# aerius-labs/paillier-halo2

Hardware: AMD Instinct MI355X
Metric: Paillier-encrypt proofs/s (2048-bit n, k=17); MSM achieved HBM GB/s vs peak (higher is better)
Workload: dtype u32 limbs (29-bit reduced radix, 254-bit modular integers), u64 limbs (4096-bit integers)

## Files before the change

include/pz.h:

```cpp
#ifndef PZ_H
#define PZ_H

#include <stddef.h>
#include <stdint.h>

#ifdef __cplusplus
extern "C" {
#endif

typedef struct pz_ctx pz_ctx;
typedef struct pz_bases pz_bases;

enum pz_status {
    PZ_OK = 0,
    PZ_ERR_INVALID = -1,
    PZ_ERR_HIP = -2,
    PZ_ERR_NO_DEVICE = -3,
    PZ_ERR_OOM = -4,
    PZ_ERR_ZERO_MODULUS = -5,
    PZ_ERR_RANGE = -6,
    PZ_ERR_UNSUPPORTED = -7,
    PZ_ERR_CAPACITY = -8,
    PZ_ERR_MESSAGE_RANGE = -9,
    PZ_ERR_ASYNC = -10
    ,
    PZ_ERR_INTERNAL = -11
};

int pz_init(int n_devices, const int* device_ids, pz_ctx** out);
int pz_free(pz_ctx* ctx);
const char* pz_strerror(int status);
const char* pz_last_hip_error(const pz_ctx* ctx);
int pz_set_stream(pz_ctx* ctx, void* hip_stream);
int pz_sync(pz_ctx* ctx);
#define PZ_ABI_VERSION 7
int pz_abi_version(void);

int pz_dev_alloc(pz_ctx* ctx, size_t bytes, void** d_out);
int pz_dev_cache_limit(pz_ctx* ctx, size_t max_bytes);
int pz_dev_arena(pz_ctx* ctx, size_t bytes);
int pz_dev_arena_info(pz_ctx* ctx, uint64_t out[6]);
int pz_dev_mem_info(pz_ctx* ctx, size_t* free_bytes, size_t* total_bytes);
int pz_dev_free(pz_ctx* ctx, void* d);
int pz_upload(pz_ctx* ctx, void* d_dst, const void* src, size_t bytes);
int pz_download(pz_ctx* ctx, void* dst, const void* d_src, size_t bytes);
int pz_dev_memset(pz_ctx* ctx, void* d_dst, int byte_value, size_t bytes);
int pz_dev_copy(pz_ctx* ctx, void* d_dst, const void* d_src, size_t bytes);
int pz_dev_copy_2d(pz_ctx* ctx, void* d_dst, size_t dst_pitch, const void* d_src, size_t src_pitch, size_t width, size_t rows);
int pz_ctx_wait(pz_ctx* waiter, pz_ctx* producer);

int pz_srs_load_g1(pz_ctx* ctx, uint32_t k, const uint64_t* bases_affine, int lagrange, pz_bases** out);
int pz_bases_load_g1(pz_ctx* ctx, const uint64_t* bases_affine, size_t n_points, int on_device,
                     uint32_t window_bits, pz_bases** out);
int pz_bases_free(pz_ctx* ctx, pz_bases* bases);
int pz_bases_info(const pz_bases* bases, size_t* n_points, uint32_t* window_bits, uint32_t* n_windows);

int pz_msm_g1(pz_ctx* ctx, const pz_bases* bases, const uint64_t* scalars, size_t n, uint64_t out_jac[12]);
int pz_msm_g1_batch(pz_ctx* ctx, const pz_bases* bases, const uint64_t* const* scalar_cols, size_t n_cols,
                    size_t n, uint64_t* out_jac );
int pz_msm_g1_dev(pz_ctx* ctx, const pz_bases* bases, const uint64_t* d_scalars, size_t n_cols, size_t n,
                  size_t col_stride, uint32_t win_lo, uint32_t win_hi, uint64_t* d_out_jac);
int pz_g1_sum(pz_ctx* ctx, const uint64_t* jac , size_t n, uint64_t out_jac[12]);
int pz_g1_sum_dev(pz_ctx* ctx, const uint64_t* d_jac, size_t n, uint64_t* d_out_jac);
int pz_msm_g1_multi(pz_ctx* const* ctxs, const pz_bases* const* bases, const uint64_t* const* d_scalars, const size_t* n_per_ctx,
                    size_t n_ctx, int split_points, uint64_t out_jac[12]);
int pz_g1_normalize(pz_ctx* ctx, const uint64_t* jac , size_t n, uint64_t* aff );
int pz_g1_fixed_base_mul(pz_ctx* ctx, const uint64_t* scalars, size_t n, uint64_t* out_affine );
int pz_g1_fixed_base_mul_dev(pz_ctx* ctx, const uint64_t* d_scalars, size_t n, uint64_t* d_out_affine);

int pz_g1_commit_mask_dev(pz_ctx* ctx, const pz_bases* bases, const uint8_t* d_mask, size_t n_cols, size_t n, size_t mask_stride,
                          uint64_t* d_out_jac);

int pz_ntt_fr(pz_ctx* ctx, uint64_t* a , const uint64_t omega[4], uint32_t log_n);
int pz_ntt_fr_batch(pz_ctx* ctx, uint64_t* const* cols, size_t n_cols, const uint64_t omega[4], uint32_t log_n);
int pz_ntt_fr_dev(pz_ctx* ctx, uint64_t* d_a, size_t n_cols, size_t col_stride, const uint64_t omega[4],
                  uint32_t log_n, const uint64_t* pre_coset_g, const uint64_t* post_scale);
int pz_ntt_fr_to_dev(pz_ctx* ctx, const uint64_t* d_in, size_t in_stride, uint64_t* d_out, size_t out_stride, size_t n_cols,
                     const uint64_t omega[4], uint32_t log_n, const uint64_t* pre_coset_g, const uint64_t* post_scale);

int pz_ntt_fr_extend_dev(pz_ctx* ctx, const uint64_t* d_coeff, size_t n_cols, size_t in_stride, uint64_t* d_ext,
                         size_t out_stride, uint32_t log_n, uint32_t log_e, const uint64_t omega_n[4],
                         const uint64_t* coset_gens, const uint64_t* scale);
int pz_ntt_fr_coeff_extend_dev(pz_ctx* ctx, uint64_t* d_values, size_t n_cols, size_t col_stride, uint64_t* d_ext,
                               size_t out_stride, uint32_t log_n, uint32_t log_e, const uint64_t omega_n[4],
                               const uint64_t omega_n_inv[4], const uint64_t n_inv[4], const uint64_t* coset_gens);
int pz_fr_convert_dev(pz_ctx* ctx, uint64_t* d_a, size_t n, int to_mont);
int pz_fr_from_mask_dev(pz_ctx* ctx, const uint8_t* d_mask, size_t n, uint64_t* d_out);

int pz_mul_mod(pz_ctx* ctx, uint32_t limbs, const uint64_t* a, const uint64_t* b, const uint64_t* modulus,
               uint64_t* q, uint64_t* r);
int pz_paillier_trace(pz_ctx* ctx, uint32_t limbs_n2, const uint64_t* n2, const uint64_t* base, const uint64_t* exp,
                      uint32_t exp_limbs, uint64_t* steps_out, size_t* n_steps, uint64_t* result);
int pz_paillier_encrypt(pz_ctx* ctx, uint32_t limbs_n, size_t batch, const uint64_t* n, const uint64_t* g,
                        const uint64_t* m, const uint64_t* r, uint64_t* steps_out, size_t steps_cap,
                        uint32_t* n_steps_g, uint32_t* n_steps_r, uint64_t* c_out);
int pz_paillier_encrypt_dev(pz_ctx* ctx, uint32_t limbs_n, size_t batch, const uint64_t* n, const uint64_t* g,
                            const uint64_t* m, const uint64_t* r, uint64_t* d_steps_out, size_t steps_cap,
                            uint32_t* n_steps_g, uint32_t* n_steps_r, uint64_t* c_out);

int pz_paillier_encrypt_uniform(pz_ctx* ctx, uint32_t limbs_n, size_t batch, uint32_t m_bits, const uint64_t* n, const uint64_t* g,
                                const uint64_t* m, const uint64_t* r, uint64_t* steps_out, size_t steps_cap, uint32_t* n_steps_g,
                                uint32_t* n_steps_r, uint64_t* c_out);
int pz_paillier_encrypt_uniform_dev(pz_ctx* ctx, uint32_t limbs_n, size_t batch, uint32_t m_bits, const uint64_t* n,
                                    const uint64_t* g, const uint64_t* m, const uint64_t* r, uint64_t* d_steps_out, size_t steps_cap,
                                    uint32_t* n_steps_g, uint32_t* n_steps_r, uint64_t* c_out);

int pz_paillier_tally(pz_ctx* ctx, uint32_t limbs_n, size_t count, const uint64_t* n, const uint64_t* cts, uint64_t* steps_out,
                      size_t steps_cap, uint64_t* c_out);
int pz_paillier_tally_dev(pz_ctx* ctx, uint32_t limbs_n, size_t count, const uint64_t* n, const uint64_t* cts, uint64_t* d_steps_out,
                          size_t steps_cap, uint64_t* c_out);

int pz_witness_cells_per_step(uint32_t limbs, uint32_t limb_bits, uint32_t lookup_bits, size_t* advice_cells,
                              size_t* lookup_cells);
int pz_witness_expand_dev(pz_ctx* ctx, uint32_t limbs, uint32_t limb_bits, uint32_t lookup_bits,
                          const uint64_t* d_steps, size_t n_steps, const uint64_t* d_modulus, uint64_t* d_advice,
                          uint64_t* d_lookup);

int pz_circuit_cells(int kind, uint32_t limbs_n, uint32_t limb_bits, uint32_t lookup_bits, size_t n_steps_g,
                     size_t n_steps_r, size_t* advice_cells, size_t* lookup_cells);
int pz_circuit_expand_dev(pz_ctx* ctx, int kind, uint32_t limbs_n, uint32_t limb_bits, uint32_t lookup_bits,
                          const uint64_t* inputs, const uint64_t* d_steps, size_t n_steps_g, size_t n_steps_r,
                          const uint64_t* d_modulus, uint64_t* d_advice, uint64_t* d_lookup, size_t rows, size_t col_stride);

int pz_circuit_break_points(const uint8_t* gate_mask, size_t n_cells, size_t max_rows, uint64_t* starts_out, size_t capacity,
// ... 121 lines not shown
                           const uint64_t* d_l_active, const uint64_t beta[4], const uint64_t gamma[4], const uint64_t y[4],
                           uint64_t* d_h);
int pz_quotient_permutation_split_dev(pz_ctx* ctx, const uint64_t* d_cols_ext, size_t col_stride, const uint64_t* d_sigma_ext,
                                      size_t sigma_stride, const uint64_t* d_z_ext, size_t z_stride, uint32_t n_sets_total,
                                      uint32_t set_lo, uint32_t n_sets, uint32_t chunk_len, uint32_t m_cols, int head, uint32_t log_ext,
                                      uint32_t rot_step, uint32_t last_rotation, const uint64_t* d_l0, const uint64_t* d_l_last,
                                      const uint64_t beta[4], const uint64_t gamma[4], const uint64_t delta[4],
                                      const uint64_t coset_g[4], const uint64_t omega_ext[4], const uint64_t y[4], uint64_t* d_h_low,
                                      uint64_t* d_h_d);
int pz_quotient_lookup_split_dev(pz_ctx* ctx, const uint64_t* d_input_ext, size_t input_stride, const uint64_t* d_table_ext,
                                 const uint64_t* d_perm_input_ext, size_t perm_input_stride, const uint64_t* d_perm_table_ext,
                                 size_t perm_table_stride, const uint64_t* d_z_ext, size_t z_stride, uint32_t n_lookups,
                                 uint32_t log_ext, uint32_t rot_step, const uint64_t* d_l0, const uint64_t* d_l_last,
                                 const uint64_t* d_l_active, const uint64_t beta[4], const uint64_t gamma[4], const uint64_t y[4],
                                 uint64_t* d_h_low, uint64_t* d_h_d);
int pz_quotient_d_rows_dev(pz_ctx* ctx, const uint64_t* d_cols, size_t col_stride, const uint64_t* d_sigma, size_t sigma_stride,
                           const uint64_t* d_z, size_t z_stride, uint32_t m, uint32_t chunk_len, const uint64_t* d_input,
                           size_t input_stride, const uint64_t* d_table, const uint64_t* d_perm_input, size_t perm_input_stride,
                           const uint64_t* d_perm_table, size_t perm_table_stride, const uint64_t* d_zl, size_t zl_stride,
                           uint32_t n_lookups, uint32_t log_n, size_t row_lo, const uint64_t omega[4], const uint64_t beta[4],
                           const uint64_t gamma[4], const uint64_t delta[4], const uint64_t y[4], uint64_t* d_out);
int pz_fr_mul_row_dev(pz_ctx* ctx, const uint64_t* d_a, size_t n_cols, size_t col_stride, size_t n, const uint64_t* d_row,
                      uint64_t* d_out, size_t out_stride);
int pz_quotient_finish_dev(pz_ctx* ctx, uint64_t* d_h, uint32_t log_n, uint32_t log_e, const uint64_t coset_g[4],
                           const uint64_t omega_ext[4]);
int pz_fr_distribute_powers_dev(pz_ctx* ctx, uint64_t* d_a, size_t n_cols, size_t col_stride, size_t n,
                                const uint64_t g[4], const uint64_t c[4]);
int pz_fr_lincomb_dev(pz_ctx* ctx, const uint64_t* d_polys, size_t n_cols, size_t col_stride, size_t n,
                      const uint64_t v[4], uint64_t* d_out, int accumulate);
int pz_poly_div_linear_dev(pz_ctx* ctx, const uint64_t* d_coeffs, size_t n_cols, size_t col_stride, size_t n,
                           const uint64_t x[4], uint64_t* d_q, size_t q_stride);

typedef struct pz_shplonk pz_shplonk;
int pz_shplonk_begin_dev(pz_ctx* ctx, size_t n, uint32_t n_sets, const uint32_t* set_n_polys, const uint64_t* const* d_polys,
                         const uint32_t* set_n_points, const uint32_t* point_idx, uint32_t n_points_total, const uint64_t* points,
                         const uint64_t* evals, const uint64_t y[4], const uint64_t v[4], uint64_t* d_h, pz_shplonk** state);
int pz_shplonk_finish_dev(pz_ctx* ctx, pz_shplonk* state, const uint64_t u[4], const uint64_t* d_h, uint64_t* d_h2);
int pz_shplonk_free(pz_ctx* ctx, pz_shplonk* state);

typedef struct pz_structure pz_structure;
int pz_circuit_structure_dev(pz_ctx* ctx, int kind, uint32_t limbs_n, uint32_t limb_bits, uint32_t lookup_bits, uint32_t k,
                             const uint64_t* exp_g, const uint64_t* exp_r, size_t minimum_rows, uint32_t blinding_factors,
                             pz_structure** out);
int pz_circuit_structure_tally_dev(pz_ctx* ctx, uint32_t limbs_n, uint32_t limb_bits, uint32_t lookup_bits, uint32_t k, size_t count,
                                   size_t minimum_rows, uint32_t blinding_factors, pz_structure** out);
int pz_structure_info(const pz_structure* st, size_t* n_adv, size_t* n_adv_filled, size_t* n_lk, size_t* max_rows, size_t* n_constants,
                      size_t* n_cells, size_t* n_lookups, size_t* n_steps_g, size_t* n_steps_r);
int pz_structure_arrays(const pz_structure* st, const uint8_t** d_selectors, const uint32_t** d_map_col, const uint32_t** d_map_row,
                        const uint64_t** d_col_starts, const uint64_t** constants, const uint64_t** col_starts_host);
int pz_structure_free(pz_structure* st);

typedef struct pz_pk pz_pk;
typedef struct pz_proof pz_proof;
#define PZ_BLINDING_SEEDED_TEST_STREAM (~(size_t)0)
#define PZ_PK_EXT_ALL (~(size_t)0)
int pz_pk_create(pz_ctx* ctx, const pz_bases* bases_lagrange, const pz_bases* bases_monomial, uint32_t k, uint32_t lookup_bits,
                 uint32_t blinding_factors, size_t max_rows, size_t n_adv, size_t n_lk, const uint8_t* selectors,
                 const uint64_t* constants, size_t n_constants, const uint32_t* map_col, const uint32_t* map_row, size_t tile,
                 size_t ext_resident_cols, pz_pk** out);
int pz_pk_create_dev(pz_ctx* ctx, const pz_bases* bases_lagrange, const pz_bases* bases_monomial, uint32_t k, uint32_t lookup_bits,
                     uint32_t blinding_factors, size_t max_rows, size_t n_adv, size_t n_lk, const uint8_t* d_selectors,
                     const uint64_t* constants, size_t n_constants, const uint32_t* d_map_col, const uint32_t* d_map_row, size_t tile,
                     size_t ext_resident_cols, pz_pk** out);
int pz_pk_info(const pz_pk* pk, size_t* n_fixed, size_t* n_perm_cols, size_t* n_sets, size_t* blinding_words, size_t* evals_words);
int pz_pk_commitments(const pz_pk* pk, uint64_t* fixed_affine, uint64_t* sigma_affine);
int pz_pk_free(pz_pk* pk);
int pz_proof_begin(pz_pk* pk, uint64_t* d_cols, uint64_t seed, const uint64_t* blinding, size_t n_blinding, pz_proof** out,
                   uint64_t* advice_affine);
int pz_proof_lookups(pz_proof* proof, const uint64_t theta[4], uint64_t* perm_inputs_affine, uint64_t* perm_tables_affine);
int pz_proof_products(pz_proof* proof, const uint64_t beta[4], const uint64_t gamma[4], uint64_t* perm_z_affine,
                      uint64_t* lookup_z_affine, uint64_t* random_affine);
int pz_proof_quotient(pz_proof* proof, const uint64_t y[4], uint64_t* h_affine);
int pz_proof_evaluate(pz_proof* proof, const uint64_t x[4], uint64_t* evals);
int pz_proof_open_begin(pz_proof* proof, const uint64_t y[4], const uint64_t v[4], uint64_t* w1_affine);
int pz_proof_open_finish(pz_proof* proof, const uint64_t u[4], uint64_t* w2_affine, int* quotient_degree_ok);
int pz_proof_free(pz_proof* proof);

int pz_circuit_public_cells(int kind, uint32_t limbs_n, uint32_t limb_bits, uint32_t lookup_bits, size_t n_steps_g, size_t n_steps_r,
                            uint64_t* cells_out, size_t capacity, size_t* n_public);
int pz_structure_expose(pz_structure* st);
int pz_structure_public(const pz_structure* st, size_t* n_instance, size_t* n_public, const uint32_t** d_cell_col, const uint32_t** d_cell_row);
int pz_public_gather_dev(pz_ctx* ctx, const uint64_t* d_cols, size_t col_stride, const uint32_t* d_cell_col, const uint32_t* d_cell_row,
                         size_t n_public, uint64_t* out_words);
int pz_instance_eval_dev(pz_ctx* ctx, uint32_t k, const uint64_t omega[4], const uint64_t n_inv[4], const uint64_t* d_instances,
                         size_t n_public, size_t n_proofs, const uint64_t* d_x, uint64_t* d_out, int32_t* d_flags);
int pz_pk_create_pub(pz_ctx* ctx, const pz_bases* bases_lagrange, const pz_bases* bases_monomial, uint32_t k, uint32_t lookup_bits,
                     uint32_t blinding_factors, size_t max_rows, size_t n_adv, size_t n_lk, size_t n_instance, size_t n_public,
                     const uint8_t* selectors, const uint64_t* constants, size_t n_constants, const uint32_t* map_col, const uint32_t* map_row,
                     size_t tile, size_t ext_resident_cols, pz_pk** out);
int pz_pk_create_pub_dev(pz_ctx* ctx, const pz_bases* bases_lagrange, const pz_bases* bases_monomial, uint32_t k, uint32_t lookup_bits,
                         uint32_t blinding_factors, size_t max_rows, size_t n_adv, size_t n_lk, size_t n_instance, size_t n_public,
                         const uint8_t* d_selectors, const uint64_t* constants, size_t n_constants, const uint32_t* d_map_col,
                         const uint32_t* d_map_row, size_t tile, size_t ext_resident_cols, pz_pk** out);
int pz_vk_keygen_pub_dev(pz_ctx* ctx, const pz_bases* bases_lagrange, uint32_t k, uint32_t lookup_bits, size_t n_adv, size_t n_lk,
                         size_t n_instance, size_t n_public, const uint8_t* d_selectors, const uint64_t* constants, size_t n_constants,
                         const uint32_t* d_map_col, const uint32_t* d_map_row, size_t tile, uint64_t* fixed_affine, uint64_t* sigma_affine);
int pz_vk_keygen_pub(pz_ctx* ctx, const pz_bases* bases_lagrange, uint32_t k, uint32_t lookup_bits, size_t n_adv, size_t n_lk,
                     size_t n_instance, size_t n_public, const uint8_t* selectors, const uint64_t* constants, size_t n_constants,
                     const uint32_t* map_col, const uint32_t* map_row, size_t tile, uint64_t* fixed_affine, uint64_t* sigma_affine);
int pz_vk_create_pub(pz_ctx* ctx, uint32_t k, uint32_t blinding_factors, size_t n_adv, size_t n_lk, size_t n_instance, size_t n_public,
                     const uint64_t* fixed_affine, const uint64_t* sigma_affine, const uint64_t g0_affine[8], const uint64_t g2[16],
                     const uint64_t s_g2[16], pz_vk** out);
int pz_proof_begin_pub(pz_pk* pk, uint64_t* d_cols, uint64_t seed, const uint64_t* blinding, size_t n_blinding, const uint64_t* instances,
                       size_t n_public, pz_proof** out, uint64_t* advice_affine);
int pz_verify_batch_pub(pz_vk* vk, const uint64_t* instances, size_t n_public, const uint64_t* proofs, size_t n_proofs, const uint8_t* seeds,
                        const size_t* seed_offsets, int32_t* verdicts, uint64_t* h_evals, uint64_t* ab_affine, int* all_ok);
// ... 19 lines not shown
```

paillier_halo2_amd/_lib.py:

```python
from __future__ import annotations

import ctypes as C
import os
import subprocess

_HERE = os.path.dirname(os.path.abspath(__file__))
CSRC = os.path.join(_HERE, "csrc")
SO_PATH = os.path.join(CSRC, "libpz_hip.so")
PROBE_SO_PATH = os.path.join(CSRC, "libpz_probe.so")

U64P = C.POINTER(C.c_uint64)
U32P = C.POINTER(C.c_uint32)
VP = C.c_void_p

SIGNATURES = {
    "pz_init": (C.c_int, [C.c_int, C.POINTER(C.c_int), C.POINTER(VP)]),
    "pz_free": (C.c_int, [VP]),
    "pz_strerror": (C.c_char_p, [C.c_int]),
    "pz_last_hip_error": (C.c_char_p, [VP]),
    "pz_set_stream": (C.c_int, [VP, VP]),
    "pz_sync": (C.c_int, [VP]),
    "pz_abi_version": (C.c_int, []),
    "pz_dev_alloc": (C.c_int, [VP, C.c_size_t, C.POINTER(VP)]),
    "pz_dev_cache_limit": (C.c_int, [VP, C.c_size_t]),
    "pz_dev_arena": (C.c_int, [VP, C.c_size_t]),
    "pz_dev_arena_info": (C.c_int, [VP, C.POINTER(C.c_uint64)]),
    "pz_dev_mem_info": (C.c_int, [VP, C.POINTER(C.c_size_t), C.POINTER(C.c_size_t)]),
    "pz_dev_free": (C.c_int, [VP, VP]),
    "pz_upload": (C.c_int, [VP, VP, VP, C.c_size_t]),
    "pz_download": (C.c_int, [VP, VP, VP, C.c_size_t]),
    "pz_dev_memset": (C.c_int, [VP, VP, C.c_int, C.c_size_t]),
    "pz_dev_copy": (C.c_int, [VP, VP, VP, C.c_size_t]),
    "pz_dev_copy_2d": (C.c_int, [VP, VP, C.c_size_t, VP, C.c_size_t, C.c_size_t, C.c_size_t]),
    "pz_ctx_wait": (C.c_int, [VP, VP]),
    "pz_srs_load_g1": (C.c_int, [VP, C.c_uint32, VP, C.c_int, C.POINTER(VP)]),
    "pz_bases_load_g1": (C.c_int, [VP, VP, C.c_size_t, C.c_int, C.c_uint32, C.POINTER(VP)]),
    "pz_bases_free": (C.c_int, [VP, VP]),
    "pz_bases_info": (C.c_int, [VP, C.POINTER(C.c_size_t), U32P, U32P]),
    "pz_msm_g1": (C.c_int, [VP, VP, VP, C.c_size_t, VP]),
    "pz_msm_g1_batch": (C.c_int, [VP, VP, C.POINTER(VP), C.c_size_t, C.c_size_t, VP]),
    "pz_msm_g1_dev": (C.c_int, [VP, VP, VP, C.c_size_t, C.c_size_t, C.c_size_t, C.c_uint32, C.c_uint32, VP]),
    "pz_g1_commit_mask_dev": (C.c_int, [VP, VP, VP, C.c_size_t, C.c_size_t, C.c_size_t, VP]),
    "pz_g1_sum": (C.c_int, [VP, VP, C.c_size_t, VP]),
    "pz_g1_sum_dev": (C.c_int, [VP, VP, C.c_size_t, VP]),
    "pz_msm_g1_multi": (C.c_int, [VP, VP, VP, VP, C.c_size_t, C.c_int, VP]),
    "pz_g1_normalize": (C.c_int, [VP, VP, C.c_size_t, VP]),
    "pz_g1_fixed_base_mul": (C.c_int, [VP, VP, C.c_size_t, VP]),
    "pz_g1_fixed_base_mul_dev": (C.c_int, [VP, VP, C.c_size_t, VP]),
    "pz_ntt_fr": (C.c_int, [VP, VP, VP, C.c_uint32]),
    "pz_ntt_fr_batch": (C.c_int, [VP, C.POINTER(VP), C.c_size_t, VP, C.c_uint32]),
    "pz_ntt_fr_dev": (C.c_int, [VP, VP, C.c_size_t, C.c_size_t, VP, C.c_uint32, VP, VP]),
    "pz_ntt_fr_to_dev": (C.c_int, [VP, VP, C.c_size_t, VP, C.c_size_t, C.c_size_t, VP, C.c_uint32, VP, VP]),
    "pz_ntt_fr_extend_dev": (C.c_int, [VP, VP, C.c_size_t, C.c_size_t, VP, C.c_size_t, C.c_uint32, C.c_uint32, VP, VP, VP]),
    "pz_ntt_fr_coeff_extend_dev": (C.c_int, [VP, VP, C.c_size_t, C.c_size_t, VP, C.c_size_t, C.c_uint32, C.c_uint32, VP, VP, VP,
                                             VP]),
    "pz_fr_convert_dev": (C.c_int, [VP, VP, C.c_size_t, C.c_int]),
    "pz_fr_from_mask_dev": (C.c_int, [VP, VP, C.c_size_t, VP]),
    "pz_mul_mod": (C.c_int, [VP, C.c_uint32, VP, VP, VP, VP, VP]),
    "pz_paillier_trace": (C.c_int, [VP, C.c_uint32, VP, VP, VP, C.c_uint32, VP, C.POINTER(C.c_size_t), VP]),
    "pz_paillier_encrypt": (C.c_int, [VP, C.c_uint32, C.c_size_t, VP, VP, VP, VP, VP, C.c_size_t, VP, VP, VP]),
    "pz_paillier_encrypt_dev": (C.c_int, [VP, C.c_uint32, C.c_size_t, VP, VP, VP, VP, VP, C.c_size_t, VP, VP, VP]),
    "pz_paillier_tally": (C.c_int, [VP, C.c_uint32, C.c_size_t, VP, VP, VP, C.c_size_t, VP]),
    "pz_paillier_tally_dev": (C.c_int, [VP, C.c_uint32, C.c_size_t, VP, VP, VP, C.c_size_t, VP]),
    "pz_paillier_encrypt_uniform": (C.c_int, [VP, C.c_uint32, C.c_size_t, C.c_uint32, VP, VP, VP, VP, VP, C.c_size_t, VP, VP, VP]),
    "pz_paillier_encrypt_uniform_dev": (C.c_int, [VP, C.c_uint32, C.c_size_t, C.c_uint32, VP, VP, VP, VP, VP, C.c_size_t, VP, VP, VP]),
    "pz_witness_cells_per_step": (C.c_int, [C.c_uint32, C.c_uint32, C.c_uint32, C.POINTER(C.c_size_t),
                                            C.POINTER(C.c_size_t)]),
    "pz_witness_expand": (C.c_int, [VP, C.c_uint32, C.c_uint32, C.c_uint32, VP, C.c_size_t, VP, VP, VP]),
    "pz_witness_expand_dev": (C.c_int, [VP, C.c_uint32, C.c_uint32, C.c_uint32, VP, C.c_size_t, VP, VP, VP]),
    "pz_refresh_aux": (C.c_int, [C.c_uint32, C.c_uint32, C.c_uint32, VP, C.c_uint32, U32P]),
    "pz_op_cells": (C.c_int, [C.c_int, C.c_uint32, C.c_uint32, C.c_uint32, C.POINTER(C.c_size_t), C.POINTER(C.c_size_t)]),
    "pz_circuit_cells": (C.c_int, [C.c_int, C.c_uint32, C.c_uint32, C.c_uint32, C.c_size_t, C.c_size_t, C.POINTER(C.c_size_t),
                                   C.POINTER(C.c_size_t)]),
    "pz_circuit_expand_dev": (C.c_int, [VP, C.c_int, C.c_uint32, C.c_uint32, C.c_uint32, VP, VP, C.c_size_t, C.c_size_t, VP, VP, VP,
                                        C.c_size_t, C.c_size_t]),
    "pz_circuit_break_points": (C.c_int, [VP, C.c_size_t, C.c_size_t, VP, C.c_size_t, C.POINTER(C.c_size_t)]),
    "pz_circuit_expand_cols_dev": (C.c_int, [VP, C.c_int, C.c_uint32, C.c_uint32, C.c_uint32, VP, VP, C.c_size_t, C.c_size_t, VP, VP, VP,
                                             VP, C.c_size_t, C.c_size_t, C.c_size_t, C.c_size_t]),
    "pz_srs_setup_g1_dev": (C.c_int, [VP, C.c_uint32, VP, VP, VP, VP]),
    "pz_srs_lagrange_from_monomial_dev": (C.c_int, [VP, C.c_uint32, VP, VP, VP, VP]),
    "pz_permutation_sigma_dev": (C.c_int, [VP, VP, VP, C.c_size_t, C.c_uint32, VP, VP, VP, C.c_size_t]),
    "pz_permutation_sigma_part_dev": (C.c_int, [VP, VP, VP, C.c_size_t, C.c_size_t, C.c_size_t, C.c_uint32, VP, VP, VP, C.c_size_t]),
    "pz_keygen_columns_dev": (C.c_int, [VP, VP, VP, C.c_size_t, C.c_size_t, C.c_uint32, C.c_uint32, VP, VP, VP, VP, VP, VP, C.c_size_t]),
    "pz_poly_eval_dev": (C.c_int, [VP, VP, C.c_size_t, C.c_size_t, C.c_size_t, VP, VP]),
    "pz_poly_eval_multi_dev": (C.c_int, [VP, VP, C.c_size_t, C.c_size_t, C.c_size_t, VP, C.c_uint32, VP]),
    "pz_g1_check_dev": (C.c_int, [VP, VP, C.c_size_t, C.POINTER(C.c_uint64)]),
    "pz_g2_generator": (C.c_int, [VP]),
    "pz_g2_mul_dev": (C.c_int, [VP, VP, VP, C.c_size_t, VP]),
    "pz_pairing_dev": (C.c_int, [VP, VP, VP, C.c_size_t, VP]),
    "pz_pairing_check_dev": (C.c_int, [VP, VP, VP, C.c_size_t, C.c_uint32, VP]),
    "pz_vk_create": (C.c_int, [VP, C.c_uint32, C.c_uint32, C.c_size_t, C.c_size_t, VP, VP, VP, VP, VP, C.POINTER(VP)]),
    "pz_vk_info": (C.c_int, [VP, C.POINTER(C.c_size_t), C.POINTER(C.c_size_t)]),
    "pz_verify_batch": (C.c_int, [VP, VP, C.c_size_t, VP, VP, VP, VP, VP, C.POINTER(C.c_int)]),
    "pz_vk_free": (C.c_int, [VP]),
    "pz_vk_keygen_dev": (C.c_int, [VP, VP, C.c_uint32, C.c_uint32, C.c_size_t, C.c_size_t, VP, VP, C.c_size_t, VP, VP, C.c_size_t, VP, VP]),
# ... 171 lines not shown
```

paillier_halo2_amd/csrc/pz_internal.h:

```cpp
#pragma once
#include <hip/hip_runtime.h>
#include <stdint.h>
#include <stdio.h>
#include <string.h>

#include <map>
#include <mutex>
#include <vector>

#include "../../include/pz.h"

enum { PZ_T_MSM_ACC = 0, PZ_T_NTT = 1, PZ_T_TRACE = 2, PZ_T_EXPAND = 3, PZ_T_MSM_ALL = 4, PZ_T_MSM_SORT = 5, PZ_T_MSM_TREE = 6, PZ_T_COUNT = 7 };

struct pz_pow_table {
    uint64_t base[4];
    uint64_t init[4];
    size_t n;
    size_t cap;
    void* d;
    void* d_raw = nullptr;
    bool raw_valid = false;
    uint64_t stamp;
};

// ... 7 lines not shown
    size_t cap = 0;
};

enum { WS_HIST = 0, WS_OFFS, WS_CURSOR, WS_ITEMS, WS_ENTRIES, WS_PARTIALS, WS_NODES_A, WS_NODES_B, WS_NTT_TMP,
       WS_IO_A, WS_IO_B, WS_IO_C, WS_BIG_A, WS_BIG_B, WS_BIG_C, WS_MISC, WS_TOTALS, WS_ORDER, WS_SH_C, WS_SH_SMALL, WS_ROWC, WS_SEL, WS_K3, WS_MULTI, WS_PAIR, WS_COUNT };

struct pz_event_pair {
    hipEvent_t a, b;
};

#define PZ_IO_EVENTS 10
struct pz_arena;
struct pz_ctx {
    int device = 0;
    hipStream_t own_stream = nullptr;
    hipStream_t stream = nullptr;
    char hip_err[256] = {0};
    pz_wsbuf ws[WS_COUNT];
    std::vector<pz_pow_table> pow_tables;
    uint64_t pow_clock = 0;
    std::vector<pz_ext_table> ext_tables;
    bool timing = false;
    std::vector<pz_event_pair> ev[PZ_T_COUNT];
    size_t ev_used[PZ_T_COUNT] = {0};
    double ev_ms[PZ_T_COUNT] = {0};
    uint64_t ev_n[PZ_T_COUNT] = {0};
    int cu_count = 256;
    size_t mem_avail = 0;
    unsigned mem_avail_age = 0;
    hipStream_t io_h2d = nullptr, io_d2h = nullptr;
    hipEvent_t io_ev[PZ_IO_EVENTS] = {};
    void* stage_h[4] = {nullptr, nullptr, nullptr, nullptr};
    size_t stage_cap[4] = {0, 0, 0, 0};
    hipEvent_t stage_ev[4] = {nullptr, nullptr, nullptr, nullptr};
    unsigned stage_next = 0;
    volatile unsigned* async_err_h = nullptr;
    volatile unsigned* async_err_d = nullptr;
    size_t dev_cache_limit = 0, dev_cache_bytes = 0;
    std::vector<std::pair<void*, size_t>> dev_cache;
    std::map<void*, size_t> dev_live;
    struct pz_arena* arena = nullptr;
    std::recursive_mutex mu;
};

struct pz_bases {
    size_t n = 0;
    uint32_t c = 0;
    uint32_t nwin = 0;
    void* d_table = nullptr;
    int lagrange = 0;
    int device = 0;
};

static inline int pz_hip_fail(pz_ctx* ctx, hipError_t e, const char* what) {
    if (ctx) snprintf(ctx->hip_err, sizeof ctx->hip_err, "%s: %s", what, hipGetErrorString(e));
    return e == hipErrorOutOfMemory ? PZ_ERR_OOM : PZ_ERR_HIP;
}
#define HIPCHK(ctx, x)                                              \
    do {                                                            \
        hipError_t e_ = (x);                                        \
        if (e_ != hipSuccess) return pz_hip_fail((ctx), e_, #x);    \
    } while (0)
#define PZCHK(x)                    \
    do {                            \
        int rc_ = (x);              \
        if (rc_ != PZ_OK) return rc_; \
    } while (0)

#define PZ_ENTER(ctx)                                           \
    std::lock_guard<std::recursive_mutex> pz_lock_((ctx)->mu);  \
    HIPCHK((ctx), hipSetDevice((ctx)->device))

int pz_ws_get(pz_ctx* ctx, int slot, size_t bytes, void** out);
hipError_t pz_hip_malloc(pz_ctx* ctx, void** d, size_t bytes);
hipError_t pz_hip_free(void* d);
size_t pz_mem_free_bytes(pz_ctx* ctx);
void pz_dev_cache_trim(pz_ctx* ctx, size_t keep_bytes);
int pz_get_pow_table(pz_ctx* ctx, const uint64_t base[4], size_t n, void** d_out, const uint64_t* init = nullptr);
int pz_get_pow_table_raw(pz_ctx* ctx, const uint64_t base[4], size_t n, void** d_raw_out, const uint64_t* init = nullptr);
int pz_raw29_convert(pz_ctx* ctx, const void* d_src_fr, void* d_dst_u32, size_t count);

struct pz_timer {
    pz_ctx* ctx;
    int cls;
    bool on;
    size_t idx;
    pz_timer(pz_ctx* c, int cls_);
    ~pz_timer();
};

int pz_async_err_init(pz_ctx* ctx);
int pz_check_async(pz_ctx* ctx);
const uint64_t* pz_fr_one261();
int pz_io_init(pz_ctx* ctx);
int pz_upload_small_async(pz_ctx* ctx, void* d_dst, const void* src, size_t bytes);

int pz_permutation_sigma_tile(pz_ctx* ctx, const uint32_t* d_mc, const uint32_t* d_mr, size_t m_total, size_t n_cols, uint32_t k,
                              const uint64_t omega[4], const uint64_t delta[4], uint64_t* d_sigma, size_t sigma_stride);

struct pz_dev_bufs {
    pz_ctx* c;
    std::vector<void*> bufs;
    explicit pz_dev_bufs(pz_ctx* c_) : c(c_) {}
    int get(size_t bytes, void** out) {
        *out = nullptr;
        const int rc = pz_dev_alloc(c, bytes ? bytes : 1, out);
// ... 59 lines not shown
```

paillier_halo2_amd/csrc/pz_msm.hip:

```cpp
#include "ec.cuh"
#include "ec29.cuh"
#include "ec29_quad.cuh"
#include <math.h>
#include <stdlib.h>

#include "pz_internal.h"

#define MSM_CHUNK_MIN 16u
#define MSM_CHUNK_MAX 256u
#define MSM_HEAVY 24u
#define MSM_MEDIUM 1024u
#define MSM_SLICE_MAX_COLS 8u

struct MsmP {
    size_t n;
    size_t n_table;
    unsigned c;
    unsigned nwin;
    unsigned win_lo, win_hi;
    unsigned B;
    size_t cap;
    size_t max_items;
    unsigned chunk;
    unsigned spt;
};

struct ScatterSel {
    const unsigned long long* total;
    unsigned long long thr;
    volatile unsigned* err;
};
__device__ __noinline__ void scatter_bad(const ScatterSel& s) { *s.err = 1u; }
__device__ __forceinline__ bool scatter_dense(const ScatterSel& s) { return *s.total >= s.thr; }

__device__ __forceinline__ u32 sel8(const u32 s[8], unsigned i) {
    u32 r = s[0];
#pragma unroll
    for (int k = 1; k < 8; ++k) r = (i == (unsigned)k) ? s[k] : r;
    return r;
}

__device__ __forceinline__ bool scalar_prepare(const Fr& mont, u32 s[8]) {
    Fr k = fp_from_mont(mont);
    Fr t;
    u64 br = 0;
#pragma unroll
    for (int i = 0; i < 8; ++i) {
        u64 d = (u64)FieldParams<FrTag>::P(i) - k.v[i] - br;
        t.v[i] = (u32)d;
        br = (d >> 32) & 1;
    }
    bool lt = false, decided = false;
#pragma unroll
    for (int i = 7; i >= 0; --i) {
        if (!decided && t.v[i] != k.v[i]) {
            lt = t.v[i] < k.v[i];
            decided = true;
        }
    }
#pragma unroll
    for (int i = 0; i < 8; ++i) s[i] = lt ? t.v[i] : k.v[i];
    return lt;
}

__device__ __forceinline__ int next_digit(const u32 s[8], unsigned w, unsigned c, unsigned& carry) {
    unsigned off = w * c;
    unsigned wi = off >> 5, sh = off & 31;
    u32 lo = wi < 8 ? sel8(s, wi) : 0;
    u32 hi = wi + 1 < 8 ? sel8(s, wi + 1) : 0;
    u64 both = ((u64)hi << 32) | lo;
    unsigned raw = (unsigned)(both >> sh) & ((1u << c) - 1);
    unsigned d = raw + carry;
    if (d > (1u << (c - 1))) {
        carry = 1;
        return (int)d - (int)(1u << c);
    }
    carry = 0;
    return (int)d;
}

__global__ __launch_bounds__(128) void k_build_table(const G1Aff64* __restrict__ bases, G1Aff64* __restrict__ table,
                                                     size_t n, unsigned c, unsigned nwin) {
    size_t i = (size_t)blockIdx.x * blockDim.x + threadIdx.x;
    if (i >= n) return;
    G1A29 p = a29_load64(bases + i);
    if (!a29_is_inf(p)) {
        p.x = f29_to_261(p.x);
        p.y = f29_to_261(p.y);
        p = a29_canon(p);
    }
    a29_store64(table + i, p);
    G1X29 x = x29_from_affine(p);
    for (unsigned w = 1; w < nwin; ++w) {
        for (unsigned k = 0; k < c; ++k) x = x29_dbl(x);
        const G1A29 a = a29_canon(x29_to_affine(x));
        a29_store64(table + (size_t)w * n + i, a);
        x = x29_from_affine(a);
    }
}

#define SORT_THREADS 1024u
#ifndef SORT_PER_THREAD
#define SORT_PER_THREAD 8u
#endif
#define SORT_SLICE (SORT_THREADS * SORT_PER_THREAD)
#define SORT_MAXB 32768u

#ifndef PZ_SORT_XCD
#define PZ_SORT_XCD 1
#endif
__device__ __forceinline__ bool sort_block_coords(unsigned n_slices, size_t n_cols, unsigned& slice, size_t& col) {
    if (PZ_SORT_XCD && n_cols >= 8) {
        const unsigned w = blockIdx.x >> 3;
        slice = w % n_slices;
        col = (size_t)(w / n_slices) * 8 + (blockIdx.x & 7u);
    } else {
        slice = blockIdx.x % n_slices;
        col = blockIdx.x / n_slices;
    }
    return col < n_cols;
}
static unsigned sort_grid(unsigned n_slices, size_t n_cols) {
    if (PZ_SORT_XCD && n_cols >= 8) return n_slices * (unsigned)((n_cols + 7) / 8 * 8);
    return n_slices * (unsigned)n_cols;
}

__global__ __launch_bounds__(SORT_THREADS) void k_msm_hist(const Fr* __restrict__ scalars, size_t col_stride, MsmP p,
                                                           u32* __restrict__ slice_hist, unsigned n_slices, size_t n_cols) {
    __shared__ u32 h[SORT_MAXB];
    size_t col;
    unsigned slice;
    if (!sort_block_coords(n_slices, n_cols, slice, col)) return;
    for (unsigned b = threadIdx.x; b < p.B; b += SORT_THREADS) h[b] = 0;
    __syncthreads();
    const size_t base = (size_t)slice * SORT_THREADS * p.spt;
    for (unsigned t = 0; t < p.spt; ++t) {
        const size_t i = base + (size_t)t * SORT_THREADS + threadIdx.x;
        if (i >= p.n) break;
        u32 s[8];
        (void)scalar_prepare(fp_load<FrTag>(scalars + col * col_stride + i), s);
        u32 any = 0;
#pragma unroll
        for (int k = 0; k < 8; ++k) any |= s[k];
        if (!any) continue;
        unsigned carry = 0;
        if (p.c == 16) {
#pragma unroll
            for (unsigned w = 0; w < 16; ++w) {
                if (w < p.win_hi) {
                    const unsigned d0 = ((s[w >> 1] >> (16 * (w & 1))) & 0xffffu) + carry;
                    carry = d0 > 0x8000u ? 1u : 0u;
                    const unsigned mag = carry ? 0x10000u - d0 : d0;
                    if (w >= p.win_lo && mag != 0) atomicAdd(&h[mag - 1], 1u);
                }
            }
        } else {
            for (unsigned w = 0; w < p.win_hi; ++w) {
                int d = next_digit(s, w, p.c, carry);
                if (w >= p.win_lo && d != 0) atomicAdd(&h[(d < 0 ? -d : d) - 1], 1u);
            }
        }
    }
    __syncthreads();
    u32* out = slice_hist + (col * n_slices + slice) * (size_t)p.B;
    for (unsigned b = threadIdx.x; b < p.B; b += SORT_THREADS) out[b] = h[b];
}

__global__ __launch_bounds__(256) void k_msm_totals(u32* __restrict__ slice_hist, unsigned n_slices, MsmP p,
                                                    u32* __restrict__ totals) {
    const size_t col = blockIdx.y;
    const unsigned b = blockIdx.x * blockDim.x + threadIdx.x;
    if (b >= p.B) return;
    u32* sh = slice_hist + col * n_slices * (size_t)p.B + b;
    u32 run = 0;
    unsigned sl = 0;
    for (; sl + 8 <= n_slices; sl += 8) {
        u32 v[8];
#pragma unroll
        for (unsigned k = 0; k < 8; ++k) v[k] = sh[(size_t)(sl + k) * p.B];
#pragma unroll
        for (unsigned k = 0; k < 8; ++k) {
            sh[(size_t)(sl + k) * p.B] = run;
            run += v[k];
        }
    }
    for (; sl < n_slices; ++sl) {
        const u32 v = sh[(size_t)sl * p.B];
        sh[(size_t)sl * p.B] = run;
        run += v;
    }
    totals[col * p.B + b] = run;
// ... 73 lines not shown
            run += s_bin[m2];
            s_bin[m2] = 0;
        }
        fold_cnt[col] = run;
        run = 0;
        for (int sz = (int)p.chunk; sz >= 1; --sz) {
            s_obase[sz] = run;
            run += s_obin[sz];
            s_obin[sz] = 0;
        }
    }
    __syncthreads();
    c = s_cnt[threadIdx.x];
    m = s_itm[threadIdx.x];
#pragma unroll
    for (unsigned k = 0; k < 32; ++k) {
        const unsigned b = lo + k;
        if (k < per && b < p.B) {
            const u32 v = hv[k];
            o[b] = c;
            it[b] = m;
            c += v;
            const u32 ch = (v + p.chunk - 1) / p.chunk;
            m += ch;
            if (ch > 1 && ch <= MSM_HEAVY) fold_order[col * p.B + s_base[ch] + atomicAdd(&s_bin[ch], 1u)] = b;
            if (ch) {
                const u32 q = v / ch, rem = v % ch;
                const u32 ph = rem ? s_obase[q + 1] + atomicAdd(&s_obin[q + 1], rem) : 0u;
                const u32 pl = s_obase[q] + atomicAdd(&s_obin[q], ch - rem);
                {
                    const u32 item0 = m - ch;
                    u32* ord = item_order + col * p.max_items;
                    u32* obk = item_bucket + col * p.max_items;
                    for (u32 j = 0; j < ch; ++j) {
                        const u32 pos = j < rem ? ph + j : pl + j - rem;
                        ord[pos] = item0 + j;
                        obk[pos] = b;
                    }
                }
            }
        }
    }
}

#define SORT_FINE_LOG 7u
#define SORT_FINE (1u << SORT_FINE_LOG)
#define SORT_COARSE_MAX (SORT_MAXB >> SORT_FINE_LOG)
#define COARSE_THREADS 256u
#define COARSE_ROUND (COARSE_THREADS * 16u)
static_assert(COARSE_ROUND <= 65536u && SORT_COARSE_MAX <= 256u && SORT_COARSE_MAX == COARSE_THREADS, "k_msm_scatter_coarse packing");
__global__ __launch_bounds__(COARSE_THREADS) void k_msm_scatter_coarse(const Fr* __restrict__ scalars, size_t col_stride, MsmP p,
                                                                       const u32* __restrict__ slice_hist, unsigned n_slices,
                                                                       const u32* __restrict__ offs, u32* __restrict__ staged,
                                                                       size_t n_cols, ScatterSel sel) {
    if (!scatter_dense(sel)) return;
    __shared__ u32 cb[SORT_COARSE_MAX];
    __shared__ u32 cnt[SORT_COARSE_MAX];
    __shared__ u32 lbase[SORT_COARSE_MAX];
    __shared__ u32 gb[SORT_COARSE_MAX];
    __shared__ u32 stage[COARSE_ROUND];
    __shared__ unsigned char sbin[COARSE_ROUND];
    __shared__ u32 s_total;
    size_t col;
    unsigned slice;
    if (!sort_block_coords(n_slices, n_cols, slice, col)) return;
    const u32* in = slice_hist + (col * n_slices + slice) * (size_t)p.B;
    const u32* o = offs + col * (p.B + 1);
    const unsigned n_coarse = p.B >> SORT_FINE_LOG;
    if (threadIdx.x < SORT_COARSE_MAX) {
        cb[threadIdx.x] = threadIdx.x < n_coarse ? o[threadIdx.x << SORT_FINE_LOG] : 0u;
        cnt[threadIdx.x] = 0;
    }
    __syncthreads();
    for (unsigned b0 = (threadIdx.x & ~63u); b0 < p.B; b0 += 4 * COARSE_THREADS) {
        u32 v[4];
#pragma unroll
        for (unsigned k = 0; k < 4; ++k) {
            const unsigned b = b0 + k * COARSE_THREADS + (threadIdx.x & 63u);
            v[k] = b < p.B ? in[b] : 0u;
        }
#pragma unroll
        for (unsigned k = 0; k < 4; ++k) {
            u32 t = v[k];
#pragma unroll
            for (int off = 32; off > 0; off >>= 1) t += __shfl_xor(t, off, 64);
            const unsigned b = b0 + k * COARSE_THREADS;
            if ((threadIdx.x & 63u) == 0 && b < p.B && t) atomicAdd(&cb[b >> SORT_FINE_LOG], t);
        }
    }
    __syncthreads();
    u32* e = staged + col * p.cap;
    const size_t base = (size_t)slice * SORT_THREADS * p.spt;
    const unsigned rounds = SORT_THREADS * p.spt / COARSE_THREADS;
    Fr nxt = fp_zero<FrTag>();
    if (base + threadIdx.x < p.n) nxt = fp_load<FrTag>(scalars + col * col_stride + base + threadIdx.x);
    for (unsigned rd = 0; rd < rounds; ++rd) {
        const size_t i = base + (size_t)rd * COARSE_THREADS + threadIdx.x;
        if (base + (size_t)rd * COARSE_THREADS >= p.n) break;
        const Fr cur_scalar = nxt;
        u32 ev[16], rb[16];
#pragma unroll
        for (unsigned w = 0; w < 16; ++w) rb[w] = 0xffffffffu;
        if (i < p.n) {
            u32 s[8];
            const bool neg = scalar_prepare(cur_scalar, s);
            unsigned carry = 0;
#pragma unroll
            for (unsigned w = 0; w < 16; ++w) {
                if (w < p.win_hi) {
                    const unsigned d0 = ((s[w >> 1] >> (16 * (w & 1))) & 0xffffu) + carry;
                    carry = d0 > 0x8000u ? 1u : 0u;
                    const unsigned mag = carry ? 0x10000u - d0 : d0;
                    if (w >= p.win_lo && mag != 0) {
                        const unsigned bkt = mag - 1, grp = bkt >> SORT_FINE_LOG;
                        const bool sgn = neg != (carry != 0);
                        ev[w] = (u32)((size_t)w * p.n_table + i) | (sgn ? 0x01000000u : 0u) | ((bkt & (SORT_FINE - 1)) << 25);
                        rb[w] = atomicAdd(&cnt[grp], 1u) | (grp << 16);
                    }
                }
            }
        }
        __syncthreads();
        if (threadIdx.x < 64) {
            const unsigned c0 = cnt[4 * threadIdx.x], c1 = cnt[4 * threadIdx.x + 1], c2 = cnt[4 * threadIdx.x + 2], c3 = cnt[4 * threadIdx.x + 3];
            const unsigned sum = c0 + c1 + c2 + c3;
            unsigned incl = sum;
#pragma unroll
            for (int off = 1; off < 64; off <<= 1) {
                const unsigned t = __shfl_up(incl, off, 64);
                if ((int)threadIdx.x >= off) incl += t;
            }
            const unsigned excl = incl - sum;
            lbase[4 * threadIdx.x] = excl;
            lbase[4 * threadIdx.x + 1] = excl + c0;
            lbase[4 * threadIdx.x + 2] = excl + c0 + c1;
            lbase[4 * threadIdx.x + 3] = excl + c0 + c1 + c2;
            if (threadIdx.x == 63) s_total = incl;
        }
        __syncthreads();
        {
            const unsigned g = cb[threadIdx.x], c = cnt[threadIdx.x];
            gb[threadIdx.x] = g - lbase[threadIdx.x];
            cb[threadIdx.x] = g + c;
            cnt[threadIdx.x] = 0;
        }
#pragma unroll
        for (unsigned w = 0; w < 16; ++w) {
            if (rb[w] != 0xffffffffu) {
                const unsigned grp = rb[w] >> 16, slot = lbase[grp] + (rb[w] & 0xffffu);
                stage[slot] = ev[w];
                sbin[slot] = (unsigned char)grp;
            }
        }
        __syncthreads();
        {
            const size_t in_ = i + COARSE_THREADS;
            if (rd + 1 < rounds && in_ < p.n) nxt = fp_load<FrTag>(scalars + col * col_stride + in_);
        }
        const unsigned total = s_total;
        for (unsigned sl = threadIdx.x; sl < total; sl += COARSE_THREADS) {
            const u32 pos = gb[sbin[sl]] + sl;
            if (pos < p.cap) e[pos] = stage[sl];
            else scatter_bad(sel);
        }
    }
}

#define FINE_LDS_ENTRIES 12288u
#define FINE_THREADS 512u
__global__ __launch_bounds__(FINE_THREADS) void k_msm_scatter_fine(MsmP p, const u32* __restrict__ offs, const u32* __restrict__ staged,
                                                          u32* __restrict__ entries, ScatterSel sel) {
    if (!scatter_dense(sel)) return;
    __shared__ u32 cur[SORT_FINE + 1];
    __shared__ u32 buf[FINE_LDS_ENTRIES];
    const size_t col = blockIdx.y;
    const u32* o = offs + col * (p.B + 1) + ((size_t)blockIdx.x << SORT_FINE_LOG);
    if (threadIdx.x <= SORT_FINE) cur[threadIdx.x] = o[threadIdx.x];
    __syncthreads();
    const u32 lo = cur[0], hi = cur[SORT_FINE];
    __syncthreads();
    const u32* src = staged + col * p.cap;
    u32* dst = entries + col * p.cap;
    const bool in_lds = hi - lo <= FINE_LDS_ENTRIES;
    for (u32 j0 = lo + threadIdx.x; j0 < hi; j0 += 8 * FINE_THREADS) {
        u32 v[8];
#pragma unroll
        for (unsigned k = 0; k < 8; ++k) {
            const u32 j = j0 + k * FINE_THREADS;
            v[k] = j < hi ? src[j] : 0xffffffffu;
        }
#pragma unroll
        for (unsigned k = 0; k < 8; ++k) {
            if (j0 + k * FINE_THREADS < hi) {
                const u32 pos = atomicAdd(&cur[v[k] >> 25], 1u);
                const u32 e = (v[k] & 0x00ffffffu) | ((v[k] & 0x01000000u) << 7);
                if (pos >= hi) scatter_bad(sel);
                else if (in_lds) buf[pos - lo] = e;
                else dst[pos] = e;
            }
        }
    }
    if (!in_lds) return;
    __syncthreads();
    for (u32 j = threadIdx.x; j < hi - lo; j += FINE_THREADS) dst[lo + j] = buf[j];
}

#define FEW_BINS (MSM_CHUNK_MAX + 1u)
__device__ __forceinline__ u32 block_sum_256(u32 v, u32* s_tmp) {
#pragma unroll
    for (int off = 32; off > 0; off >>= 1) v += __shfl_xor(v, off, 64);
// ... 114 lines not shown
    if (lane == 63) { s_wc[wv] = ic; s_wm[wv] = im; }
    __syncthreads();
    u32 bc = 0, bm = 0;
    for (unsigned k = 0; k < wv; ++k) { bc += s_wc[k]; bm += s_wm[k]; }
    const u32 o_b = pc + bc + ic - v, it_b = pm + bm + im - ch;
    u32* o = offs + col * (p.B + 1);
    u32* it = items + col * (p.B + 1);
    if (b < p.B) {
        o[b] = o_b;
        it[b] = it_b;
        if (b == p.B - 1) {
            o[p.B] = o_b + v;
            it[p.B] = it_b + ch;
            atomicAdd(digits_total, (unsigned long long)(o_b + v));
        }
    }
    u32* ord = item_order + col * p.max_items;
    u32* obk = item_bucket + col * p.max_items;
    u32 ph = 0, pl = 0, rem = 0;
    if (ch) {
        const u32 q = v / ch;
        rem = v % ch;
        if (rem) ph = s_pos[q + 1] + atomicAdd(&s_rank[q + 1], rem);
        pl = s_pos[q] + atomicAdd(&s_rank[q], ch - rem);
        if (ch > ITEMS_SOLO) {
            s_big[atomicAdd(&s_nbig, 1u)] = threadIdx.x;
        } else {
            for (u32 j = 0; j < ch; ++j) {
                const u32 pos = j < rem ? ph + j : pl + j - rem;
                ord[pos] = it_b + j;
                obk[pos] = b;
            }
        }
    }
    __shared__ u32 s_par[256][5];
    if (ch > ITEMS_SOLO) {
        s_par[threadIdx.x][0] = ch; s_par[threadIdx.x][1] = rem; s_par[threadIdx.x][2] = ph; s_par[threadIdx.x][3] = pl; s_par[threadIdx.x][4] = it_b;
    }
    __syncthreads();
    for (unsigned k = 0; k < s_nbig; ++k) {
        const unsigned tt = s_big[k];
        const u32 ch2 = s_par[tt][0], rem2 = s_par[tt][1], ph2 = s_par[tt][2], pl2 = s_par[tt][3], it2 = s_par[tt][4];
        for (u32 j = threadIdx.x; j < ch2; j += blockDim.x) {
            const u32 pos = j < rem2 ? ph2 + j : pl2 + j - rem2;
            ord[pos] = it2 + j;
            obk[pos] = blk * blockDim.x + tt;
        }
    }
}

__global__ __launch_bounds__(SORT_THREADS) void k_msm_scatter(const Fr* __restrict__ scalars, size_t col_stride, MsmP p,
                                                              const u32* __restrict__ slice_hist, unsigned n_slices,
                                                              const u32* __restrict__ offs, u32* __restrict__ entries, size_t n_cols,
                                                              ScatterSel sel) {
    if (scatter_dense(sel)) return;
    __shared__ u32 h[SORT_MAXB];
    size_t col;
    unsigned slice;
    if (!sort_block_coords(n_slices, n_cols, slice, col)) return;
    const u32* in = slice_hist + (col * n_slices + slice) * (size_t)p.B;
    const u32* o = offs + col * (p.B + 1);
    for (unsigned b0 = threadIdx.x; b0 < p.B; b0 += 8 * SORT_THREADS) {
        u32 va[8], vb[8];
#pragma unroll
        for (unsigned k = 0; k < 8; ++k) {
            const unsigned b = b0 + k * SORT_THREADS, bc = b < p.B ? b : p.B - 1;
            va[k] = o[bc];
            vb[k] = in[bc];
        }
#pragma unroll
        for (unsigned k = 0; k < 8; ++k) {
            const unsigned b = b0 + k * SORT_THREADS;
            if (b < p.B) h[b] = va[k] + vb[k];
        }
    }
    __syncthreads();
    u32* e = entries + col * p.cap;
    const size_t base = (size_t)slice * SORT_THREADS * p.spt;
    for (unsigned t = 0; t < p.spt; ++t) {
        const size_t i = base + (size_t)t * SORT_THREADS + threadIdx.x;
        if (i >= p.n) break;
        u32 s[8];
        const bool neg = scalar_prepare(fp_load<FrTag>(scalars + col * col_stride + i), s);
        u32 any = 0;
#pragma unroll
        for (int k = 0; k < 8; ++k) any |= s[k];
        if (!any) continue;
        unsigned carry = 0;
        if (p.c == 16) {
#pragma unroll
            for (unsigned w = 0; w < 16; ++w) {
                if (w < p.win_hi) {
                    const unsigned d0 = ((s[w >> 1] >> (16 * (w & 1))) & 0xffffu) + carry;
                    carry = d0 > 0x8000u ? 1u : 0u;
                    const unsigned mag = carry ? 0x10000u - d0 : d0;
                    if (w >= p.win_lo && mag != 0) {
                        const u32 pos = atomicAdd(&h[mag - 1], 1u);
                        const bool sgn = neg != (carry != 0);
                        if (pos < p.cap) e[pos] = (u32)((size_t)w * p.n_table + i) | (sgn ? 0x80000000u : 0u);
                        else scatter_bad(sel);
                    }
                }
            }
        } else {
            for (unsigned w = 0; w < p.win_hi; ++w) {
                int d = next_digit(s, w, p.c, carry);
                if (w >= p.win_lo && d != 0) {
                    const unsigned b = (d < 0 ? -d : d) - 1;
                    const u32 pos = atomicAdd(&h[b], 1u);
                    const bool sgn = neg != (d < 0);
                    if (pos < p.cap) e[pos] = (u32)((size_t)w * p.n_table + i) | (sgn ? 0x80000000u : 0u);
                    else scatter_bad(sel);
                }
            }
        }
    }
}

__global__ __launch_bounds__(256) void k_msm_accumulate(const G1Aff64* __restrict__ table, MsmP p,
                                                        const u32* __restrict__ offs, const u32* __restrict__ items,
                                                        const u32* __restrict__ item_order,
                                                        const u32* __restrict__ item_bucket,
                                                        const u32* __restrict__ entries, G1X29Raw* __restrict__ partials) {
    const size_t col = blockIdx.x;
    const u32* it = items + col * (p.B + 1);
    const u32 total = it[p.B];
    const u32 rank = blockIdx.y * blockDim.x + threadIdx.x;
    if (rank >= total) return;
    const u32 item = item_order[col * p.max_items + rank];
    const unsigned b = item_bucket[col * p.max_items + rank];
    const u32* o = offs + col * (p.B + 1);
    const u32 cnt = o[b + 1] - o[b], nch = it[b + 1] - it[b], j = item - it[b];
    const u32 q = cnt / nch, rem = cnt % nch;
    const u32 start = o[b] + j * q + (j < rem ? j : rem);
// ... 455 lines not shown
    int rc = pz_bases_load_g1(ctx, bases_affine, (size_t)1 << k, 0, 0, out);
    if (rc == PZ_OK) (*out)->lagrange = lagrange;
    return rc;
}

extern "C" int pz_bases_free(pz_ctx* ctx, pz_bases* b) {
    if (!b) return PZ_OK;
    if (ctx) {
        std::lock_guard<std::recursive_mutex> lk(ctx->mu);
        (void)hipSetDevice(ctx->device);
        (void)hipStreamSynchronize(ctx->stream);
    }
    if (b->d_table) (void)pz_hip_free(b->d_table);
    delete b;
    return PZ_OK;
}

extern "C" int pz_bases_info(const pz_bases* b, size_t* n_points, uint32_t* window_bits, uint32_t* n_windows) {
    if (!b) return PZ_ERR_INVALID;
    if (n_points) *n_points = b->n;
    if (window_bits) *window_bits = b->c;
    if (n_windows) *n_windows = b->nwin;
    return PZ_OK;
}

static unsigned msm_chunk_for(size_t n_cols, size_t digits_per_col, unsigned window_bits) {
    static int env = -1;
    if (env < 0) {
        const char* e = getenv("PZ_MSM_CHUNK");
        env = e ? atoi(e) : 0;
    }
    if (env >= (int)MSM_CHUNK_MIN && env <= (int)MSM_CHUNK_MAX) return (unsigned)env;
    if (n_cols <= MSM_SLICE_MAX_COLS) {
        const double per_bucket = (double)digits_per_col / (double)((size_t)1 << (window_bits - 1));
        double ch = 0.79 * pow(per_bucket, 0.63);
        unsigned c32 = ch < 24.0 ? MSM_CHUNK_MIN : 32u * (unsigned)((ch + 16.0) / 32.0);
        if (c32 > MSM_CHUNK_MAX) c32 = MSM_CHUNK_MAX;
        return c32;
    }
    const size_t want = (n_cols * digits_per_col) >> 18;
    unsigned chunk = MSM_CHUNK_MIN;
    while (chunk < MSM_CHUNK_MAX && chunk * 2 <= want) chunk *= 2;
    return chunk;
}

static unsigned msm_spt_for(size_t n_cols, size_t n) {
    const size_t min_wg = n_cols <= MSM_SLICE_MAX_COLS ? 128 : 512;
    unsigned spt = SORT_PER_THREAD;
    while (spt > 1 && n_cols * pz_div_up(n, (size_t)SORT_THREADS * spt) < min_wg) spt >>= 1;
    return spt;
}

static int msm_group(pz_ctx* ctx, const pz_bases* bases, const Fr* d_scalars, size_t nc, size_t n, size_t cs,
                     unsigned win_lo, unsigned win_hi, unsigned chunk, G1Jac* d_out) {
    MsmP p;
    p.n = n;
    p.n_table = bases->n;
    p.c = bases->c;
    p.nwin = bases->nwin;
    p.win_lo = win_lo;
    p.win_hi = win_hi;
    p.B = 1u << (bases->c - 1);
    p.cap = n * (size_t)(win_hi - win_lo);
    p.chunk = chunk;
    if (p.B + n * (size_t)(win_hi - win_lo) / chunk > 65535u * 256u) return PZ_ERR_CAPACITY;
    p.max_items = p.B + p.cap / chunk;
    void *hist, *offs, *heavy, *items, *entries, *partials, *na, *nb, *totals, *fold, *iord;
    p.spt = msm_spt_for(nc, n);
    const unsigned n_slices = pz_div_up(n, (size_t)SORT_THREADS * p.spt);
    PZCHK(pz_ws_get(ctx, WS_HIST, nc * (size_t)n_slices * p.B * 4, &hist));
    PZCHK(pz_ws_get(ctx, WS_CURSOR, nc * (size_t)(p.B + 1) * 4, &heavy));
    const bool split_items = nc <= MSM_SLICE_MAX_COLS;
    const unsigned nblk_few = pz_div_up(p.B, 256);
    PZCHK(pz_ws_get(ctx, WS_TOTALS, nc * ((size_t)p.B + (split_items ? (size_t)nblk_few * (2 + FEW_BINS) : 0)) * 4, &totals));
    u32* blk_cnt = (u32*)totals + nc * (size_t)p.B;
    u32* blk_itm = blk_cnt + nc * (size_t)nblk_few;
    u32* blk_bins = blk_itm + nc * (size_t)nblk_few;
    u32* heavy_cnt = (u32*)heavy + nc * (size_t)p.B;
    PZCHK(pz_ws_get(ctx, WS_MISC, nc * (size_t)(p.B + 1) * 4, &fold));
    u32* fold_cnt = (u32*)fold + nc * (size_t)p.B;
    PZCHK(pz_ws_get(ctx, WS_ORDER, nc * p.max_items * 8, &iord));
    u32* item_order = (u32*)iord;
    u32* item_bucket = (u32*)iord + nc * p.max_items;
    PZCHK(pz_ws_get(ctx, WS_OFFS, nc * (p.B + 1) * 4, &offs));
    PZCHK(pz_ws_get(ctx, WS_ITEMS, nc * (p.B + 1) * 4, &items));
    PZCHK(pz_ws_get(ctx, WS_ENTRIES, nc * p.cap * 4 + 16, &entries));
    static int scatter_mode = -1;
    if (scatter_mode < 0) {
        const char* e = getenv("PZ_MSM_SCATTER");
        scatter_mode = (e && !strcmp(e, "one")) ? 1 : (e && !strcmp(e, "two")) ? 2 : 0;
    }
    const bool two_pass = scatter_mode != 1 && p.c == 16 && (size_t)p.nwin * p.n_table <= ((size_t)1 << 24) &&
                          (nc > MSM_SLICE_MAX_COLS || scatter_mode == 2);
    {
        const size_t part_bytes = nc * p.max_items * sizeof(G1X29Raw), stage_bytes = two_pass ? nc * p.cap * 4 + 16 : 0;
        PZCHK(pz_ws_get(ctx, WS_PARTIALS, part_bytes > stage_bytes ? part_bytes : stage_bytes, &partials));
    }
    const unsigned m1 = p.B >= 16 ? 16 : p.B;
    unsigned n_nodes = p.B / m1;
    PZCHK(pz_ws_get(ctx, WS_NODES_A, nc * (size_t)n_nodes * sizeof(MsmNode), &na));
    PZCHK(pz_ws_get(ctx, WS_NODES_B, nc * (size_t)(n_nodes / 2 + 1) * sizeof(MsmNode), &nb));
    hipStream_t st = ctx->stream;
    pz_timer tall(ctx, PZ_T_MSM_ALL);
    dim3 gs(sort_grid(n_slices, nc));
    void* dsel;
    PZCHK(pz_ws_get(ctx, WS_SEL, 8, &dsel));
    HIPCHK(ctx, hipMemsetAsync(dsel, 0, 8, st));
    PZCHK(pz_async_err_init(ctx));
    {
        pz_timer tsort(ctx, PZ_T_MSM_SORT);
        hipLaunchKernelGGL(k_msm_hist, gs, dim3(SORT_THREADS), 0, st, d_scalars, cs, p, (u32*)hist, n_slices, nc);
        if (split_items) {
            hipLaunchKernelGGL(k_msm_totals_few, dim3(nblk_few, (unsigned)nc), dim3(256), 0, st, (u32*)hist, n_slices, p, (u32*)totals,
                               blk_cnt, blk_itm, blk_bins);
            hipLaunchKernelGGL(k_msm_items_few, dim3(nblk_few, (unsigned)nc), dim3(256), 0, st, p, (const u32*)totals, (const u32*)blk_cnt,
                               (const u32*)blk_itm, (const u32*)blk_bins, (u32*)offs, (u32*)items, item_order, item_bucket,
                               (unsigned long long*)dsel);
        } else {
            hipLaunchKernelGGL(k_msm_totals, dim3(pz_div_up(p.B, 256), (unsigned)nc), dim3(256), 0, st, (u32*)hist, n_slices, p,
                               (u32*)totals);
            hipLaunchKernelGGL(k_msm_scan, dim3((unsigned)nc), dim3(SCAN_THREADS), 0, st, (const u32*)totals, p, (u32*)offs, (u32*)items,
                               (u32*)heavy, heavy_cnt, (u32*)fold, fold_cnt, item_order, item_bucket, (unsigned long long*)dsel);
        }
        ScatterSel sel;
        sel.total = (const unsigned long long*)dsel;
        sel.thr = !two_pass ? ~0ull : scatter_mode == 2 ? 0ull : (unsigned long long)(0.4 * (double)nc * (double)p.cap);
        sel.err = ctx->async_err_d;
        if (two_pass) {
            hipLaunchKernelGGL(k_msm_scatter_coarse, gs, dim3(COARSE_THREADS), 0, st, d_scalars, cs, p, (const u32*)hist, n_slices,
                               (const u32*)offs, (u32*)partials, nc, sel);
            hipLaunchKernelGGL(k_msm_scatter_fine, dim3(p.B >> SORT_FINE_LOG, (unsigned)nc), dim3(FINE_THREADS), 0, st, p, (const u32*)offs,
                               (const u32*)partials, (u32*)entries, sel);
        }
        if (scatter_mode != 2 || !two_pass)
            hipLaunchKernelGGL(k_msm_scatter, gs, dim3(SORT_THREADS), 0, st, d_scalars, cs, p, (const u32*)hist, n_slices,
                               (const u32*)offs, (u32*)entries, nc, sel);
    }
    {
        pz_timer tacc(ctx, PZ_T_MSM_ACC);
        hipLaunchKernelGGL(k_msm_accumulate, dim3((unsigned)nc, pz_div_up(p.max_items, 256)), dim3(256), 0, st,
                           (const G1Aff64*)bases->d_table, p, (const u32*)offs, (const u32*)items,
                           (const u32*)item_order, (const u32*)item_bucket, (const u32*)entries, (G1X29Raw*)partials);
    }
    pz_timer ttree(ctx, PZ_T_MSM_TREE);
    if (split_items) {
        const unsigned gx4 = pz_div_up(p.B, 64), gx32 = p.B / 8 < 2048u ? (p.B / 8 ? p.B / 8 : 1u) : 2048u;
        hipLaunchKernelGGL(k_msm_fold_few, dim3(gx4, (unsigned)nc), dim3(256), 0, st, p, (const u32*)items, (G1X29Raw*)partials, 2u, 1u, MSM_FEW_SMALL);
        hipLaunchKernelGGL(k_msm_fold_few, dim3(gx32, (unsigned)nc), dim3(256), 0, st, p, (const u32*)items, (G1X29Raw*)partials, 5u, MSM_FEW_SMALL,
                           MSM_MEDIUM);
        hipLaunchKernelGGL(k_msm_heavy_few, dim3(p.B / 256 < 64u ? (p.B / 256 ? p.B / 256 : 1u) : 64u, (unsigned)nc), dim3(256), 0, st, p,
                           (const u32*)items, (G1X29Raw*)partials);
    } else {
    hipLaunchKernelGGL(k_msm_bucket_sum, dim3((unsigned)nc, pz_div_up(p.B, 256)), dim3(256), 0, st, p, (const u32*)items,
                       (const u32*)fold, (const u32*)fold_cnt, (G1X29Raw*)partials);
    unsigned hx = (unsigned)(8192 / nc);
    if (hx < 4) hx = 4;
    if (hx > p.B) hx = p.B;
    hipLaunchKernelGGL(k_msm_heavy_sum, dim3(hx, (unsigned)nc), dim3(256), 0, st, p, (const u32*)items, (const u32*)heavy,
                       (const u32*)heavy_cnt, (G1X29Raw*)partials);
    hipLaunchKernelGGL(k_msm_medium_sum, dim3(hx, (unsigned)nc), dim3(256), 0, st, p, (const u32*)items, (const u32*)heavy,
                       (const u32*)heavy_cnt, (G1X29Raw*)partials);
    }
    if (nc <= MSM_SLICE_MAX_COLS) {
        const unsigned nblk = (p.B >> 8) + 1;
        void *sp, *sl;
        PZCHK(pz_ws_get(ctx, WS_NODES_A, nc * (size_t)SLICE_SLOTS * nblk * sizeof(G1X29Raw), &sp));
        PZCHK(pz_ws_get(ctx, WS_NODES_B, nc * 16 * sizeof(G1X29Raw), &sl));
        hipLaunchKernelGGL(k_msm_slice_partial, dim3(nblk, SLICE_SLOTS, (unsigned)nc), dim3(256), 0, st, p, (const u32*)items,
                           (const G1X29Raw*)partials, nblk, (G1X29Raw*)sp);
        hipLaunchKernelGGL(k_msm_slice_reduce, dim3(p.c, (unsigned)nc), dim3(256), 0, st, p, nblk, (const G1X29Raw*)sp, (G1X29Raw*)sl);
        hipLaunchKernelGGL(k_msm_slice_horner, dim3((unsigned)nc), dim3(64), 0, st, p, (const G1X29Raw*)sl, d_out);
        HIPCHK(ctx, hipGetLastError());
        return PZ_OK;
    }
    hipLaunchKernelGGL(k_msm_reduce_l1, dim3(pz_div_up(n_nodes, 128), (unsigned)nc), dim3(128), 0, st, p, m1,
                       (const u32*)items, (const G1X29Raw*)partials, (MsmNode*)na);
    const unsigned m1_used = m1;
    MsmNode* cur = (MsmNode*)na;
    MsmNode* nxt = (MsmNode*)nb;
    unsigned log_w = 0;
    for (unsigned t = m1_used; t > 1; t >>= 1) ++log_w;
    while (n_nodes > 1) {
        unsigned m = n_nodes >= 16 ? 16 : n_nodes;
        hipLaunchKernelGGL(k_msm_combine_quad, dim3(pz_div_up((size_t)(n_nodes / m) * 4, 256), (unsigned)nc), dim3(256), 0, st, n_nodes, m,
                           log_w, (const MsmNode*)cur, nxt);
        n_nodes /= m;
        for (unsigned t = m; t > 1; t >>= 1) ++log_w;
        MsmNode* tmp = cur;
        cur = nxt;
        nxt = tmp;
    }
    hipLaunchKernelGGL(k_msm_emit, dim3(pz_div_up(nc, 64)), dim3(64), 0, st, (const MsmNode*)cur, nc, d_out);
    HIPCHK(ctx, hipGetLastError());
    return PZ_OK;
}

extern "C" int pz_msm_g1_dev(pz_ctx* ctx, const pz_bases* bases, const uint64_t* d_scalars, size_t n_cols, size_t n,
                             size_t col_stride, uint32_t win_lo, uint32_t win_hi, uint64_t* d_out_jac) {
    if (!ctx || !bases || (n_cols && (!d_scalars || !d_out_jac))) return PZ_ERR_INVALID;
    if (n > bases->n || win_lo > win_hi || win_hi > bases->nwin) return PZ_ERR_INVALID;
    if (col_stride % 4 || (n_cols > 1 && col_stride < 4 * n)) return PZ_ERR_INVALID;
    if (n_cols == 0) return PZ_OK;
    PZ_ENTER(ctx);
    if (n == 0 || win_lo == win_hi) {
        size_t nn = n_cols;
        void* z;
        PZCHK(pz_ws_get(ctx, WS_NODES_A, nn * sizeof(MsmNode), &z));
        HIPCHK(ctx, hipMemsetAsync(z, 0, nn * sizeof(MsmNode), ctx->stream));
        hipLaunchKernelGGL(k_msm_emit, dim3(pz_div_up(nn, 64)), dim3(64), 0, ctx->stream, (const MsmNode*)z, nn,
                           (G1Jac*)d_out_jac);
        HIPCHK(ctx, hipGetLastError());
        return PZ_OK;
    }
    const size_t cs = col_stride / 4;
    const size_t digits = n * (size_t)(win_hi - win_lo);
    const unsigned chunk = msm_chunk_for(n_cols, digits, bases->c);
    const size_t part_col = (digits / chunk) * sizeof(G1X29Raw);
    const size_t per_col = digits * 4 + (part_col > digits * 4 ? part_col : digits * 4) + (digits / chunk) * 8 +
                           (size_t)(1u << (bases->c - 1)) * (180 + 4 * (size_t)pz_div_up(n, (size_t)SORT_THREADS * msm_spt_for(1, n)));
    size_t ws_budget = pz_msm_ws_gib() << 30;
    {
        if (ctx->mem_avail == 0 || ++ctx->mem_avail_age >= 64) {
            const size_t free_b = pz_mem_free_bytes(ctx);
            if (free_b) {
                size_t held = 0;
                for (int i = 0; i < WS_COUNT; ++i) held += ctx->ws[i].cap;
                ctx->mem_avail = (free_b + held) / 2;
                ctx->mem_avail_age = 0;
            }
        }
        if (ctx->mem_avail && ws_budget > ctx->mem_avail) ws_budget = ctx->mem_avail;
    }
    size_t group = ws_budget / per_col;
    if (group == 0) group = 1;
    if (group > n_cols) group = n_cols;
    if (group > 4096) group = 4096;
    for (size_t c0 = 0; c0 < n_cols;) {
        const size_t nc = n_cols - c0 < group ? n_cols - c0 : group;
        const int rc = msm_group(ctx, bases, (const Fr*)d_scalars + c0 * cs, nc, n, cs, win_lo, win_hi, chunk, (G1Jac*)d_out_jac + c0);
        if (rc == PZ_ERR_OOM && group > 1) {
            ctx->mem_avail = 0;
            (void)hipGetLastError();
            group = (group + 1) / 2;
            continue;
        }
        PZCHK(rc);
        c0 += nc;
    }
    return PZ_OK;
}

extern "C" int pz_msm_g1_batch(pz_ctx* ctx, const pz_bases* bases, const uint64_t* const* scalar_cols, size_t n_cols,
                               size_t n, uint64_t* out_jac) {
    if (!ctx || !bases || (n_cols && (!scalar_cols || !out_jac))) return PZ_ERR_INVALID;
    if (n > bases->n) return PZ_ERR_INVALID;
    if (n_cols == 0) return PZ_OK;
    PZ_ENTER(ctx);
    const size_t bytes = n * 32;
    for (size_t j = 0; j < n_cols; ++j)
        if (!scalar_cols[j] && n) return PZ_ERR_INVALID;
    const size_t g_min = bytes ? (((size_t)1 << 27) / bytes ? ((size_t)1 << 27) / bytes : 1) : n_cols;
    size_t g_max = bytes ? (((size_t)1 << 30) / bytes ? ((size_t)1 << 30) / bytes : 1) : n_cols;
    if (g_max > n_cols) g_max = n_cols;
    void *d_s, *d_o;
    PZCHK(pz_ws_get(ctx, WS_IO_B, 2 * g_max * bytes + 32, &d_s));
    PZCHK(pz_ws_get(ctx, WS_IO_C, n_cols * 96, &d_o));
    PZCHK(pz_io_init(ctx));
    hipEvent_t* ev_in = ctx->io_ev;
    hipEvent_t* ev_done = ctx->io_ev + 2;
    int rc = PZ_OK;
    size_t g = 0, group = g_min < g_max ? g_min : g_max;
    for (size_t c0 = 0; c0 < n_cols && rc == PZ_OK; ++g) {
        const size_t nc = n_cols - c0 < group ? n_cols - c0 : group;
        const unsigned b = (unsigned)(g & 1);
        char* buf = (char*)d_s + b * g_max * bytes;
        hipError_t e = hipSuccess;
        if (g >= 2) e = hipStreamWaitEvent(ctx->io_h2d, ev_done[b], 0);
        for (size_t j = 0; j < nc && e == hipSuccess && bytes; ++j)
            e = hipMemcpyAsync(buf + j * bytes, scalar_cols[c0 + j], bytes, hipMemcpyHostToDevice, ctx->io_h2d);
        if (e == hipSuccess) e = hipEventRecord(ev_in[b], ctx->io_h2d);
        if (e == hipSuccess) e = hipStreamWaitEvent(ctx->stream, ev_in[b], 0);
        if (e != hipSuccess) { rc = pz_hip_fail(ctx, e, "pz_msm_g1_batch: upload"); break; }
        rc = pz_msm_g1_dev(ctx, bases, (const uint64_t*)buf, nc, n, 4 * n, 0, bases->nwin, (uint64_t*)d_o + c0 * 12);
        if (rc == PZ_OK && (e = hipEventRecord(ev_done[b], ctx->stream)) != hipSuccess) rc = pz_hip_fail(ctx, e, "pz_msm_g1_batch: event");
        c0 += nc;
        group = group * 2 < g_max ? group * 2 : g_max;
    }
    if (rc == PZ_OK) {
        hipError_t e = hipMemcpyAsync(out_jac, d_o, n_cols * 96, hipMemcpyDeviceToHost, ctx->stream);
        if (e != hipSuccess) rc = pz_hip_fail(ctx, e, "pz_msm_g1_batch: download");
    }
    hipError_t e1 = hipStreamSynchronize(ctx->io_h2d), e2 = hipStreamSynchronize(ctx->stream);
    if (rc == PZ_OK && (e1 != hipSuccess || e2 != hipSuccess)) rc = pz_hip_fail(ctx, e1 != hipSuccess ? e1 : e2, "pz_msm_g1_batch: synchronize");
    if (rc == PZ_OK) rc = pz_check_async(ctx);
    return rc;
}

extern "C" int pz_msm_g1(pz_ctx* ctx, const pz_bases* bases, const uint64_t* scalars, size_t n, uint64_t out_jac[12]) {
    if (n && !scalars) return PZ_ERR_INVALID;
    const uint64_t* cols[1] = {scalars};
    return pz_msm_g1_batch(ctx, bases, cols, 1, n, out_jac);
// ... 222 lines not shown
```

paillier_halo2_amd/csrc/pz_prover.cpp:

```cpp
#define PZP_THROW
#include "../host/create_proof.hpp"

#include <atomic>
#include <memory>
#include <mutex>
#include <new>

struct pz_pk {
    pzp::Ctx mem;
    pzp::ProvingKey* key = nullptr;
    pzp::Workspace ws;
    std::atomic<bool> busy{false};
    mutable std::mutex digest_mu;
    mutable bool have_digest = false;
    mutable uint8_t digest[pzh::KEY_DIGEST_BYTES] = {};
};
struct pz_proof {
    pz_pk* pk;
    pzp::Session* se;
    bool failed = false;
};

namespace {
bool fr_canonical(const uint64_t c[4]) {
    for (int i = 3; i >= 0; --i)
        if (c[i] != pzh::FR_MOD[i]) return c[i] < pzh::FR_MOD[i];
    return false;
}
pzh::Fr fr_of(const uint64_t c[4]) {
    pzh::Fr r;
    memcpy(r.v, c, 32);
    return r;
}
template <class F> int guarded_raw(F&& f) {
    try {
        f();
        return PZ_OK;
    } catch (const pzp::PzpError& e) {
        return e.rc;
    } catch (const std::bad_alloc&) {
        return PZ_ERR_OOM;
    } catch (...) {
        return PZ_ERR_INTERNAL;
    }
}
template <class F> int phase(pz_proof* pr, F&& f) {
    if (pr->failed) return PZ_ERR_INVALID;
    const int rc = guarded_raw(f);
    if (rc != PZ_OK) pr->failed = true;
    return rc;
}
size_t evals_words(const pzp::ProvingKey& pk) {
    const size_t A = pk.st.n_adv, Lk = pk.st.n_lk, m = pk.st.m(), S = pk.n_sets;
    return 4 * (4 * A + (Lk + 1) + pk.F + m + 3 * S + 2 * Lk + 2 * Lk + Lk + 1 + 1);
}
}

namespace {
int pk_create(pz_ctx* ctx, const pz_bases* bases_lagrange, const pz_bases* bases_monomial, uint32_t k, uint32_t lookup_bits,
              uint32_t blinding_factors, size_t max_rows, size_t n_adv, size_t n_lk, const uint8_t* selectors, const uint64_t* constants,
              size_t n_constants, const uint32_t* map_col, const uint32_t* map_row, size_t tile, size_t ext_resident_cols, bool on_device,
              size_t n_instance, size_t n_public, pz_pk** out) {
    if (!ctx || !bases_lagrange || !bases_monomial || !selectors || !map_col || !map_row || !out || (n_constants && !constants)) return PZ_ERR_INVALID;
    if (k < 4 || k > 24 || !n_adv || !n_lk || lookup_bits >= k || tile == 0 || tile % pzp::CHUNK) return PZ_ERR_INVALID;
    const size_t n = (size_t)1 << k;
    if (max_rows + blinding_factors + 1 > n || n_constants > max_rows) return PZ_ERR_INVALID;
    if (n_instance > 1 || (n_instance ? n_public == 0 || n_public > max_rows : n_public != 0)) return PZ_ERR_INVALID;
    if ((n_adv + n_lk + 1 + n_instance) > ((size_t)1 << 32) / n) return PZ_ERR_UNSUPPORTED;
    size_t np_l = 0, np_m = 0;
    if (pz_bases_info(bases_lagrange, &np_l, nullptr, nullptr) != PZ_OK || pz_bases_info(bases_monomial, &np_m, nullptr, nullptr) != PZ_OK) return PZ_ERR_INVALID;
    if (np_l < n || np_m < n) return PZ_ERR_INVALID;
    *out = nullptr;
    pz_pk* pk = new (std::nothrow) pz_pk;
    if (!pk) return PZ_ERR_OOM;
    pk->mem.c = ctx;
    pk->mem.round_cols = true;
    const int rc = guarded_raw([&] {
        pzp::Structure st;
        st.k = k; st.lookup_bits = lookup_bits; st.blinding_factors = blinding_factors; st.max_rows = max_rows; st.n_adv = n_adv; st.n_lk = n_lk;
        st.n_instance = n_instance; st.n_public = n_public;
        const size_t m = st.m();
        st.constants.assign(constants, constants + 4 * n_constants);
        if (on_device) {
            st.d_selectors = selectors; st.d_map_col = map_col; st.d_map_row = map_row;
        } else {
            st.selectors.assign(selectors, selectors + n_adv * n);
            st.map_col.assign(map_col, map_col + m * n);
            st.map_row.assign(map_row, map_row + m * n);
        }
        pk->key = pzp::keygen(pk->mem, std::move(st), bases_lagrange, bases_monomial, ext_resident_cols);
        pk->key->st.d_selectors = nullptr; pk->key->st.d_map_col = pk->key->st.d_map_row = nullptr;
        pk->ws = pzp::make_workspace(pk->mem, *pk->key, tile);
        PZP_CK(pz_sync(ctx));
    });
    if (rc != PZ_OK) {
        (void)pz_sync(ctx);
        pk->mem.release();
        delete pk->key;
        delete pk;
        return rc;
    }
    *out = pk;
    return PZ_OK;
}
}

extern "C" int pz_pk_create(pz_ctx* ctx, const pz_bases* bases_lagrange, const pz_bases* bases_monomial, uint32_t k, uint32_t lookup_bits,
                            uint32_t blinding_factors, size_t max_rows, size_t n_adv, size_t n_lk, const uint8_t* selectors,
                            const uint64_t* constants, size_t n_constants, const uint32_t* map_col, const uint32_t* map_row, size_t tile,
                            size_t ext_resident_cols, pz_pk** out) {
    return pk_create(ctx, bases_lagrange, bases_monomial, k, lookup_bits, blinding_factors, max_rows, n_adv, n_lk, selectors, constants, n_constants,
                     map_col, map_row, tile, ext_resident_cols, false, 0, 0, out);
}
extern "C" int pz_pk_create_dev(pz_ctx* ctx, const pz_bases* bases_lagrange, const pz_bases* bases_monomial, uint32_t k, uint32_t lookup_bits,
                                uint32_t blinding_factors, size_t max_rows, size_t n_adv, size_t n_lk, const uint8_t* d_selectors,
                                const uint64_t* constants, size_t n_constants, const uint32_t* d_map_col, const uint32_t* d_map_row, size_t tile,
                                size_t ext_resident_cols, pz_pk** out) {
    return pk_create(ctx, bases_lagrange, bases_monomial, k, lookup_bits, blinding_factors, max_rows, n_adv, n_lk, d_selectors, constants,
                     n_constants, d_map_col, d_map_row, tile, ext_resident_cols, true, 0, 0, out);
}
extern "C" int pz_pk_create_pub(pz_ctx* ctx, const pz_bases* bases_lagrange, const pz_bases* bases_monomial, uint32_t k, uint32_t lookup_bits,
                                uint32_t blinding_factors, size_t max_rows, size_t n_adv, size_t n_lk, size_t n_instance, size_t n_public,
                                const uint8_t* selectors, const uint64_t* constants, size_t n_constants, const uint32_t* map_col,
                                const uint32_t* map_row, size_t tile, size_t ext_resident_cols, pz_pk** out) {
    return pk_create(ctx, bases_lagrange, bases_monomial, k, lookup_bits, blinding_factors, max_rows, n_adv, n_lk, selectors, constants, n_constants,
                     map_col, map_row, tile, ext_resident_cols, false, n_instance, n_public, out);
}
extern "C" int pz_pk_create_pub_dev(pz_ctx* ctx, const pz_bases* bases_lagrange, const pz_bases* bases_monomial, uint32_t k, uint32_t lookup_bits,
                                    uint32_t blinding_factors, size_t max_rows, size_t n_adv, size_t n_lk, size_t n_instance, size_t n_public,
                                    const uint8_t* d_selectors, const uint64_t* constants, size_t n_constants, const uint32_t* d_map_col,
                                    const uint32_t* d_map_row, size_t tile, size_t ext_resident_cols, pz_pk** out) {
    return pk_create(ctx, bases_lagrange, bases_monomial, k, lookup_bits, blinding_factors, max_rows, n_adv, n_lk, d_selectors, constants,
                     n_constants, d_map_col, d_map_row, tile, ext_resident_cols, true, n_instance, n_public, out);
}

extern "C" int pz_pk_info(const pz_pk* pk, size_t* n_fixed, size_t* n_perm_cols, size_t* n_sets, size_t* blinding_words, size_t* evals_words_out) {
    if (!pk || !pk->key) return PZ_ERR_INVALID;
    if (n_fixed) *n_fixed = pk->key->F;
    if (n_perm_cols) *n_perm_cols = pk->key->st.m();
    if (n_sets) *n_sets = pk->key->n_sets;
    if (blinding_words) *blinding_words = pzp::blinding_words(*pk->key);
    if (evals_words_out) *evals_words_out = evals_words(*pk->key);
    return PZ_OK;
}

extern "C" int pz_pk_commitments(const pz_pk* pk, uint64_t* fixed_affine, uint64_t* sigma_affine) {
    if (!pk || !pk->key || !fixed_affine || !sigma_affine) return PZ_ERR_INVALID;
    memcpy(fixed_affine, pk->key->fixed_commit.data(), pk->key->fixed_commit.size() * 8);
    memcpy(sigma_affine, pk->key->sigma_commit.data(), pk->key->sigma_commit.size() * 8);
    return PZ_OK;
}

extern "C" int pz_pk_digest(const pz_pk* pk, uint8_t out[64]) {
    if (!pk || !pk->key || !out) return PZ_ERR_INVALID;
    std::lock_guard<std::mutex> g(pk->digest_mu);
    if (!pk->have_digest) {
        pzp::key_digest(*pk->key, pk->digest);
        pk->have_digest = true;
    }
    memcpy(out, pk->digest, pzh::KEY_DIGEST_BYTES);
    return PZ_OK;
}

extern "C" int pz_pk_free(pz_pk* pk) {
    if (!pk) return PZ_OK;
    if (pk->busy.load()) return PZ_ERR_INVALID;
    if (pk->mem.c) (void)pz_sync(pk->mem.c);
    pk->mem.release();
    delete pk->key;
    delete pk;
    return PZ_OK;
}

namespace {
int proof_begin(pz_pk* pk, uint64_t* d_cols, uint64_t seed, const uint64_t* blinding, size_t n_blinding, const uint64_t* instances, size_t n_public,
                pz_proof** out, uint64_t* advice_affine) {
    if (!pk || !pk->key || !d_cols || !out || !advice_affine) return PZ_ERR_INVALID;
    if (blinding ? n_blinding < pzp::blinding_words(*pk->key) : n_blinding != PZ_BLINDING_SEEDED_TEST_STREAM) return PZ_ERR_INVALID;
    if (n_public != pk->key->st.n_public || (n_public && !instances)) return PZ_ERR_INVALID;
    for (size_t i = 0; i < n_public; ++i)
        if (pzh::ge_mod(instances + 4 * i)) return PZ_ERR_INVALID;
    *out = nullptr;
    bool idle = false;
    if (!pk->busy.compare_exchange_strong(idle, true)) return PZ_ERR_INVALID;
    pz_proof* pr = new (std::nothrow) pz_proof{pk, nullptr};
    if (!pr) {
// ... 79 lines not shown
```

paillier_halo2_amd/engine.py:

```python
from __future__ import annotations

import ctypes as C
from typing import Optional, Sequence, Tuple

import numpy as np

from . import _lib
from ._lib import PzError, VP


def _np(a, shape_last: Optional[int] = None) -> np.ndarray:
    arr = np.ascontiguousarray(a, dtype=np.uint64)
    if shape_last is not None and (arr.ndim == 0 or arr.shape[-1] != shape_last):
        arr = arr.reshape(-1, shape_last)
    return arr


def _ptr(a: np.ndarray) -> VP:
    return VP(a.ctypes.data)


class Bases:

    def __init__(self, engine: "Engine", handle: VP):
        self.engine = engine
        self.handle = handle
        n = C.c_size_t()
        c = C.c_uint32()
        w = C.c_uint32()
        engine._chk(_lib.lib().pz_bases_info(handle, C.byref(n), C.byref(c), C.byref(w)), "pz_bases_info")
        self.n_points = n.value
        self.window_bits = c.value
        self.n_windows = w.value

    def free(self):
        if self.handle is not None:
            _lib.lib().pz_bases_free(self.engine.ctx, self.handle)
            self.handle = None


class VkHandle:

    def __init__(self, engine: "Engine", handle: VP):
        self.engine = engine
        self.handle = handle
        cw, ew = C.c_size_t(), C.c_size_t()
        engine._chk(_lib.lib().pz_vk_info(handle, C.byref(cw), C.byref(ew)), "pz_vk_info")
        self.commitment_words, self.evals_words = cw.value, ew.value

    @property
    def proof_words(self) -> int:
        return self.commitment_words + self.evals_words

    @property
    def wire_bytes(self) -> int:
        n = C.c_size_t()
        self.engine._chk(_lib.lib().pz_proof_wire_bytes(self.handle, C.byref(n)), "pz_proof_wire_bytes")
        return n.value

    def digest(self) -> bytes:
        out = (C.c_uint8 * 64)()
        self.engine._chk(_lib.lib().pz_vk_digest(self.handle, out), "pz_vk_digest")
        return bytes(out)

    def bind(self, on: bool = True):
        self.engine._chk(_lib.lib().pz_vk_bind(self.handle, 1 if on else 0), "pz_vk_bind")

    @property
    def bound(self) -> bool:
        on = C.c_int()
        self.engine._chk(_lib.lib().pz_vk_is_bound(self.handle, C.byref(on)), "pz_vk_is_bound")
        return bool(on.value)

    def free(self):
        if self.handle is not None:
            _lib.lib().pz_vk_free(self.handle)
            self.handle = None

    def __del__(self):
        try:
            self.free()
        except Exception:
            pass


class _BorrowedBases(Bases):

    def __init__(self, engine: "Engine", handle: VP, owner):
        super().__init__(engine, handle)
        self.owner = owner

    def free(self):
        self.handle = None
# ... 95 lines not shown
        if stream is None:
            stream = torch.cuda.Stream(device=self.device)
        assert stream.cuda_stream != 0
        torch.cuda.set_stream(stream)
        self.set_stream(stream.cuda_stream)
        self._torch_stream = stream
        return stream

    def sync(self):
        self._chk(self.L.pz_sync(self.ctx), "pz_sync")

    def load_bases(self, bases_affine, window_bits: int = 0) -> Bases:
        b = _np(bases_affine, 8)
        h = VP()
        self._chk(self.L.pz_bases_load_g1(self.ctx, _ptr(b), b.shape[0], 0, window_bits, C.byref(h)),
                  "pz_bases_load_g1")
        return Bases(self, h)

    def load_bases_dev(self, d_ptr: int, n_points: int, window_bits: int = 0) -> Bases:
        h = VP()
        self._chk(self.L.pz_bases_load_g1(self.ctx, VP(d_ptr), n_points, 1, window_bits, C.byref(h)),
                  "pz_bases_load_g1(dev)")
        return Bases(self, h)

    def srs_load_g1(self, k: int, bases_affine, lagrange: bool = False) -> Bases:
        b = _np(bases_affine, 8)
        assert b.shape[0] == 1 << k
        h = VP()
        self._chk(self.L.pz_srs_load_g1(self.ctx, k, _ptr(b), int(lagrange), C.byref(h)), "pz_srs_load_g1")
        return Bases(self, h)

    def msm(self, bases: Bases, scalars) -> np.ndarray:
        s = _np(scalars, 4)
        out = np.zeros(12, dtype=np.uint64)
        self._chk(self.L.pz_msm_g1(self.ctx, bases.handle, _ptr(s) if s.size else VP(), s.shape[0] if s.size else 0,
                                   _ptr(out)), "pz_msm_g1")
        return out

    def msm_batch(self, bases: Bases, cols: Sequence[np.ndarray]) -> np.ndarray:
        cols = [_np(c, 4) for c in cols]
        n = cols[0].shape[0] if cols else 0
        assert all(c.shape[0] == n for c in cols)
        arr = (VP * len(cols))(*[_ptr(c) for c in cols])
        out = np.zeros((len(cols), 12), dtype=np.uint64)
        self._chk(self.L.pz_msm_g1_batch(self.ctx, bases.handle, arr, len(cols), n, _ptr(out)), "pz_msm_g1_batch")
        return out

    def msm_dev(self, bases: Bases, d_scalars: int, n_cols: int, n: int, col_stride_u64: int, d_out: int,
                win_lo: int = 0, win_hi: Optional[int] = None):
        if win_hi is None:
            win_hi = bases.n_windows
        self._chk(self.L.pz_msm_g1_dev(self.ctx, bases.handle, VP(d_scalars), n_cols, n, col_stride_u64, win_lo,
                                       win_hi, VP(d_out)), "pz_msm_g1_dev")

    @staticmethod
    def msm_multi(engines: Sequence["Engine"], bases: Sequence[Bases], d_scalars: Sequence[int], n_per_ctx: Sequence[int],
                  split_points: bool) -> np.ndarray:
        k = len(engines)
        assert len(bases) == len(d_scalars) == len(n_per_ctx) == k and k > 0
        ctxs = (VP * k)(*[e.ctx for e in engines])
        bs = (VP * k)(*[(b.handle if b is not None else VP()) for b in bases])
        sc = (VP * k)(*[VP(p) for p in d_scalars])
        ns = (C.c_size_t * k)(*n_per_ctx)
        out = np.zeros(12, dtype=np.uint64)
        engines[0]._chk(engines[0].L.pz_msm_g1_multi(ctxs, bs, sc, ns, k, int(split_points), _ptr(out)), "pz_msm_g1_multi")
        return out

    def g1_sum(self, jac) -> np.ndarray:
        j = _np(jac, 12)
        out = np.zeros(12, dtype=np.uint64)
        self._chk(self.L.pz_g1_sum(self.ctx, _ptr(j), j.shape[0], _ptr(out)), "pz_g1_sum")
        return out

    def g1_sum_dev(self, d_jac: int, n: int, d_out: int):
        self._chk(self.L.pz_g1_sum_dev(self.ctx, VP(d_jac), n, VP(d_out)), "pz_g1_sum_dev")

    def g1_normalize(self, jac) -> np.ndarray:
        j = _np(jac, 12)
        out = np.zeros((j.shape[0], 8), dtype=np.uint64)
        self._chk(self.L.pz_g1_normalize(self.ctx, _ptr(j), j.shape[0], _ptr(out)), "pz_g1_normalize")
        return out

    def g1_fixed_base_mul(self, scalars) -> np.ndarray:
        s = _np(scalars, 4)
        out = np.zeros((s.shape[0], 8), dtype=np.uint64)
        self._chk(self.L.pz_g1_fixed_base_mul(self.ctx, _ptr(s), s.shape[0], _ptr(out)), "pz_g1_fixed_base_mul")
        return out

    def g1_fixed_base_mul_dev(self, d_scalars: int, n: int, d_out: int):
        self._chk(self.L.pz_g1_fixed_base_mul_dev(self.ctx, VP(d_scalars), n, VP(d_out)), "pz_g1_fixed_base_mul_dev")

    def ntt(self, a, omega, log_n: int) -> np.ndarray:
        x = _np(a, 4).copy()
        assert x.shape[0] == 1 << log_n
        w = _np(omega).reshape(4)
        self._chk(self.L.pz_ntt_fr(self.ctx, _ptr(x), _ptr(w), log_n), "pz_ntt_fr")
        return x

    def ntt_batch(self, cols: Sequence[np.ndarray], omega, log_n: int):
        cols = [_np(c, 4).copy() for c in cols]
        arr = (VP * len(cols))(*[_ptr(c) for c in cols])
        w = _np(omega).reshape(4)
        self._chk(self.L.pz_ntt_fr_batch(self.ctx, arr, len(cols), _ptr(w), log_n), "pz_ntt_fr_batch")
        return cols

    def ntt_batch_inplace(self, cols: Sequence[np.ndarray], omega, log_n: int):
# ... 649 lines not shown
```

paillier_halo2_amd/host/create_proof.hpp:

```cpp
#pragma once
#include <cstdint>
#include <cstdio>
#include <cstdlib>
#include <cstring>
#include <functional>
#include <memory>
#include <string>
#include <vector>

#include "../../include/pz.h"
#include "fr_host.hpp"
#include "key_digest.hpp"
#include "transcript.hpp"

namespace pzp {
using pzh::Fr;

struct PzpError {
    int rc;
};
#ifdef PZP_THROW
#define PZP_FAIL(rc_, what_) throw ::pzp::PzpError{rc_}
#else
#define PZP_FAIL(rc_, what_)                                                                               \
// ... 48 lines not shown
        n_inv = pzh::inv(pzh::from_u64(n));
        omega4 = pzh::omega(k + 2);
        coset_g = pzh::zeta();
        auto mk = [&](unsigned log_e, const Fr& cg, const Fr& om) {
            Part p;
            p.log_e = log_e;
            p.size = n << log_e;
            p.coset_g = cg;
            p.omega = om;
            p.omega_inv = pzh::inv(om);
            p.size_inv = pzh::inv(pzh::from_u64(p.size));
            Fr x = cg;
            for (unsigned r = 0; r < (1u << log_e); ++r) {
                p.gens.insert(p.gens.end(), x.v, x.v + 4);
                x = pzh::mul(x, om);
            }
            return p;
        };
        parts.push_back(mk(1, coset_g, pzh::mul(omega4, omega4)));
        parts.push_back(mk(0, pzh::mul(coset_g, omega4), omega));
    }
};

class Ctx {
  public:
    pz_ctx* c = nullptr;
    std::vector<void*> owned;
    bool round_cols = false;
    size_t cols(size_t x) const { return round_cols ? (x + 63) / 64 * 64 : x; }
    uint64_t* alloc(size_t words) {
        void* d = nullptr;
        PZP_CK(pz_dev_alloc(c, words * 8, &d));
        owned.push_back(d);
        PZP_CK(pz_dev_memset(c, d, 0, words * 8));
        return (uint64_t*)d;
    }
    void release() {
        for (void* d : owned) pz_dev_free(c, d);
        owned.clear();
    }
};

struct ProvingKey {
    Structure st;
    Domain dom;
    size_t n_sets = 0, F = 0;
    const pz_bases *bl = nullptr, *bm = nullptr;
    uint64_t *fixed_coeff = nullptr, *sigma_coeff = nullptr, *sigma_lagrange = nullptr, *const_lagrange = nullptr, *table_lagrange = nullptr;
    uint64_t *fixed_ext[2] = {nullptr, nullptr}, *sigma_ext[2] = {nullptr, nullptr}, *l_ext[2] = {nullptr, nullptr};
    uint64_t* table_ext[2] = {nullptr, nullptr};
    size_t res_fixed = 0, res_sigma = 0;
    bool streamed = false;
    std::vector<uint64_t> fixed_commit, sigma_commit;
    explicit ProvingKey(Structure&& s) : st(std::move(s)), dom(st.k, st.blinding_factors) {}
};

inline void key_digest(const ProvingKey& pk, uint8_t out[pzh::KEY_DIGEST_BYTES]) {
    pzh::key_digest(pk.st.k, pk.st.blinding_factors, pk.st.n_adv, pk.st.n_lk, pk.st.n_instance, pk.st.n_public, pk.fixed_commit.data(),
                    pk.sigma_commit.data(), out);
}

inline void upload_mont(Ctx& cx, uint64_t* d, const std::vector<Fr>& v) {
    PZP_CK(pz_upload(cx.c, d, v.data(), v.size() * 32));
}

static const size_t EXT_ALL = ~(size_t)0;

struct Scratch {
    pz_ctx* c;
    std::vector<void*> bufs;
    explicit Scratch(pz_ctx* c_) : c(c_) {}
    void* get(size_t bytes) {
        void* d = nullptr;
        PZP_CK(pz_dev_alloc(c, bytes, &d));
        bufs.push_back(d);
        return d;
    }
    ~Scratch() {
        for (void* d : bufs) pz_dev_free(c, d);
    }
};

inline ProvingKey* keygen(Ctx& cx, Structure&& st_in, const pz_bases* bl, const pz_bases* bm, size_t ext_resident_cols = EXT_ALL) {
    std::unique_ptr<ProvingKey> pk(new ProvingKey(std::move(st_in)));
    const Structure& st = pk->st;
    Domain& d = pk->dom;
    const size_t n = d.n, A = st.n_adv, m = st.m(), F = A + 2;
    pk->bl = bl; pk->bm = bm; pk->F = F;
    pk->n_sets = (m + CHUNK - 1) / CHUNK;
    pk->streamed = ext_resident_cols < m;
    pk->res_sigma = pk->streamed ? ext_resident_cols : m;
    pk->res_fixed = pk->res_sigma < A ? pk->res_sigma : A;
    uint64_t* fixed = cx.alloc(cx.cols(F) * n * 4);
    {
        Scratch tmp(cx.c);
        const uint8_t* d_sel = st.d_selectors;
        if (!d_sel) {
            void* up = tmp.get(A * n);
            PZP_CK(pz_upload(cx.c, up, st.selectors.data(), A * n));
            d_sel = (const uint8_t*)up;
        }
        PZP_CK(pz_fr_from_mask_dev(cx.c, d_sel, A * n, fixed));
        PZP_CK(pz_sync(cx.c));
    }
    {
        std::vector<Fr> col(n);
        const Fr zero = {{0, 0, 0, 0}};
        for (size_t i = 0; i < n; ++i) col[i] = i < st.constants.size() / 4 ? pzh::from_raw(&st.constants[4 * i]) : zero;
        upload_mont(cx, fixed + A * n * 4, col);
        for (size_t i = 0; i < n; ++i) col[i] = i < ((size_t)1 << st.lookup_bits) ? pzh::from_u64(i) : zero;
        upload_mont(cx, fixed + (A + 1) * n * 4, col);
    }
    pk->const_lagrange = cx.alloc(n * 4);
    pk->table_lagrange = cx.alloc(n * 4);
    PZP_CK(pz_dev_copy(cx.c, pk->const_lagrange, fixed + A * n * 4, n * 32));
    PZP_CK(pz_dev_copy(cx.c, pk->table_lagrange, fixed + (A + 1) * n * 4, n * 32));
    uint64_t* sigma = cx.alloc(cx.cols(m) * n * 4);
    {
        Scratch tmp(cx.c);
        const uint32_t *dmc = st.d_map_col, *dmr = st.d_map_row;
        if (!dmc || !dmr) {
            void *mc = tmp.get(m * n * 4), *mr = tmp.get(m * n * 4);
            PZP_CK(pz_upload(cx.c, mc, st.map_col.data(), m * n * 4));
            PZP_CK(pz_upload(cx.c, mr, st.map_row.data(), m * n * 4));
            dmc = (const uint32_t*)mc;
            dmr = (const uint32_t*)mr;
        }
        const Fr delta = pzh::delta();
        PZP_CK(pz_permutation_sigma_dev(cx.c, dmc, dmr, m, st.k, d.omega.v, delta.v, sigma, 4 * n));
        PZP_CK(pz_sync(cx.c));
    }
    {
        Structure& s_ = pk->st;
        std::vector<uint8_t>().swap(s_.selectors);
        std::vector<uint32_t>().swap(s_.map_col);
        std::vector<uint32_t>().swap(s_.map_row);
    }
    pk->sigma_lagrange = cx.alloc(cx.cols(m) * n * 4);
    PZP_CK(pz_dev_copy(cx.c, pk->sigma_lagrange, sigma, m * n * 32));
    uint64_t* com_f = cx.alloc(cx.cols(F) * 12);
    uint64_t* com_s = cx.alloc(cx.cols(m) * 12);
    for (int pi = 0; pi < 2; ++pi) {
        pk->fixed_ext[pi] = cx.alloc((pk->res_fixed ? cx.cols(pk->res_fixed) : 1) * d.parts[pi].size * 4);
        pk->sigma_ext[pi] = cx.alloc((pk->res_sigma ? cx.cols(pk->res_sigma) : 1) * d.parts[pi].size * 4);
        pk->l_ext[pi] = cx.alloc(3 * d.parts[pi].size * 4);
        pk->table_ext[pi] = cx.alloc(d.parts[pi].size * 4);
    }
    struct Job { uint64_t* cols; size_t cnt; uint64_t* com; uint64_t** ext; size_t res; };
    Job jobs[2] = {{fixed, F, com_f, pk->fixed_ext, pk->res_fixed}, {sigma, m, com_s, pk->sigma_ext, pk->res_sigma}};
    for (auto& jb : jobs) {
        for (size_t c0 = 0; c0 < jb.cnt; c0 += 256) {
            const size_t cnt = jb.cnt - c0 < 256 ? jb.cnt - c0 : 256;
            const size_t r_here = jb.res <= c0 ? 0 : (jb.res - c0 < cnt ? jb.res - c0 : cnt);
            const size_t lo[2] = {c0, c0 + r_here}, bc[2] = {r_here, cnt - r_here};
            for (int keep = 1; keep >= 0; --keep) {
                const size_t b0 = lo[1 - keep], bn = bc[1 - keep];
                if (!bn) continue;
                const Part& A_ = d.parts[0];
                PZP_CK(pz_keygen_columns_dev(cx.c, bl, jb.cols + b0 * n * 4, bn, 4 * n, st.k, A_.log_e, d.omega.v, d.omega_inv.v, d.n_inv.v,
                                             A_.gens.data(), jb.com + b0 * 12, keep ? jb.ext[0] + b0 * A_.size * 4 : nullptr, 4 * A_.size));
                if (!keep) continue;
                const Part& B_ = d.parts[1];
                PZP_CK(pz_ntt_fr_extend_dev(cx.c, jb.cols + b0 * n * 4, bn, 4 * n, jb.ext[1] + b0 * B_.size * 4, 4 * B_.size, st.k, B_.log_e, d.omega.v,
                                            B_.gens.data(), nullptr));
            }
        }
    }
    pk->fixed_coeff = fixed;
    pk->sigma_coeff = sigma;
    for (int pi = 0; pi < 2; ++pi)
        PZP_CK(pz_ntt_fr_extend_dev(cx.c, fixed + (A + 1) * n * 4, 1, 4 * n, pk->table_ext[pi], 4 * d.parts[pi].size, st.k, d.parts[pi].log_e,
                                    d.omega.v, d.parts[pi].gens.data(), nullptr));
    {
        uint64_t* lrows = cx.alloc(3 * n * 4);
        std::vector<Fr> col(n);
        const Fr zero = {{0, 0, 0, 0}};
        for (int w = 0; w < 3; ++w) {
            for (size_t i = 0; i < n; ++i) col[i] = (w == 0 ? i == 0 : w == 1 ? i == d.usable : i < d.usable) ? pzh::FR_ONE : zero;
            upload_mont(cx, lrows + (size_t)w * n * 4, col);
        }
        PZP_CK(pz_ntt_fr_dev(cx.c, lrows, 3, 4 * n, d.omega_inv.v, st.k, nullptr, d.n_inv.v));
        for (int pi = 0; pi < 2; ++pi)
            PZP_CK(pz_ntt_fr_extend_dev(cx.c, lrows, 3, 4 * n, pk->l_ext[pi], 4 * d.parts[pi].size, st.k, d.parts[pi].log_e, d.omega.v,
// ... 109 lines not shown
struct Fam {
    const char* name;
    const uint64_t* polys;
    size_t count;
    std::vector<int> idx;
};

struct Session {
    Ctx& cx;
    ProvingKey& pk;
    Workspace& w;
    uint64_t* d_cols;
    Rng rng;
    Fr beta, gamma, y, x, xs[6];
    uint64_t* pieces = nullptr;
    std::vector<Fam> fams;
    std::vector<std::vector<uint64_t>> ev;
    pz_shplonk* state = nullptr;
    int phase = 0;
    std::vector<uint64_t> instances;

    Session(Ctx& cx_, ProvingKey& pk_, Workspace& w_, uint64_t* d_cols_, Rng rng_) : cx(cx_), pk(pk_), w(w_), d_cols(d_cols_), rng(rng_) {}
    ~Session() {
        if (state) pz_shplonk_free(cx.c, state);
    }
    void expect(int p) {
        if (phase != p) PZP_FAIL(PZ_ERR_INVALID, "proof phases out of order");
        phase = -1;
    }
    void done(int p) { phase = p + 1; }
    void commit(const pz_bases* b, const uint64_t* t, size_t count, uint64_t* out) {
        uint32_t nw = 0, cb = 0;
        size_t np = 0;
        PZP_CK(pz_bases_info(b, &np, &cb, &nw));
        PZP_CK(pz_msm_g1_dev(cx.c, b, t, count, pk.dom.n, 4 * pk.dom.n, 0, nw, out));
    }
    void affine(const uint64_t* d_jac, size_t count, uint64_t* out) {
        std::vector<uint64_t> jac(12 * count);
        PZP_CK(pz_download(cx.c, jac.data(), d_jac, count * 96));
        PZP_CK(pz_g1_normalize(cx.c, jac.data(), count, out));
    }

    void advice(uint64_t* out_affine, const std::function<void()>& after_launch = nullptr) {
        expect(0);
        const Domain& d = pk.dom;
        const size_t n = d.n, W = pk.st.n_adv + pk.st.n_lk;
        blind_rows(cx, w, rng, d_cols, W, n, d.usable);
        PZP_CK(pz_dev_copy(cx.c, d_cols + W * n * 4, pk.const_lagrange, n * 32));
        if (pk.st.n_instance) {
            if (instances.size() != 4 * pk.st.n_public) PZP_FAIL(PZ_ERR_INVALID, "instances do not match the key's n_public");
            PZP_CK(pz_dev_memset(cx.c, d_cols + (W + 1) * n * 4, 0, n * 32));
            PZP_CK(pz_upload(cx.c, d_cols + (W + 1) * n * 4, instances.data(), instances.size() * 8));
        }
        commit(pk.bl, d_cols, W, w.out12);
        if (after_launch) after_launch();
        affine(w.out12, W, out_affine);
        done(0);
    }
    void lookups(uint64_t* out_inputs, uint64_t* out_tables) {
        expect(1);
        const Domain& d = pk.dom;
        const size_t n = d.n, Lk = pk.st.n_lk;
        uint64_t* lk_in = d_cols + pk.st.n_adv * n * 4;
        PZP_CK(pz_lookup_permute_dev(cx.c, lk_in, Lk, 4 * n, pk.table_lagrange, d.usable, pk.st.lookup_bits, w.Ap, w.Sp, 4 * n));
        blind_rows(cx, w, rng, w.Ap, Lk, n, d.usable);
        blind_rows(cx, w, rng, w.Sp, Lk, n, d.usable);
        commit(pk.bl, w.Ap, Lk, w.out12);
        commit(pk.bl, w.Sp, Lk, w.out12 + Lk * 12);
        affine(w.out12, Lk, out_inputs);
        affine(w.out12 + Lk * 12, Lk, out_tables);
        done(1);
    }
    void products(const Fr& beta_, const Fr& gamma_, uint64_t* out_z, uint64_t* out_zl, uint64_t* out_random) {
        expect(2);
        beta = beta_; gamma = gamma_;
        const Domain& d = pk.dom;
        const size_t n = d.n, u = d.usable, Lk = pk.st.n_lk, S = pk.n_sets;
        const Fr delta = pzh::delta();
        uint64_t* lk_in = d_cols + pk.st.n_adv * n * 4;
        PZP_CK(pz_permutation_product_sets_dev(cx.c, d_cols, 4 * n, pk.sigma_lagrange, 4 * n, pk.st.m(), CHUNK, d.k, u, d.omega.v, beta.v, gamma.v,
                                               delta.v, w.Z, 4 * n));
        blind_rows(cx, w, rng, w.Z, S, n, u + 1);
        PZP_CK(pz_lookup_product_dev(cx.c, lk_in, 4 * n, pk.table_lagrange, w.Ap, 4 * n, w.Sp, 4 * n, Lk, n, beta.v, gamma.v, pzh::FR_ONE.v, w.Zl,
                                     4 * n));
        blind_rows(cx, w, rng, w.Zl, Lk, n, u + 1);
        blind_rows(cx, w, rng, w.rnd, 1, n, 0);
        commit(pk.bl, w.Z, S, w.out12);
        commit(pk.bl, w.Zl, Lk, w.out12 + S * 12);
        commit(pk.bm, w.rnd, 1, w.out12 + (S + Lk) * 12);
        affine(w.out12, S, out_z);
        affine(w.out12 + S * 12, Lk, out_zl);
        affine(w.out12 + (S + Lk) * 12, 1, out_random);
        done(2);
    }
    void quotient(const Fr& y_, uint64_t* out_h) {
        expect(3);
        y = y_;
        const Structure& st = pk.st;
        const Domain& d = pk.dom;
        const size_t n = d.n, A = st.n_adv, Lk = st.n_lk, m = st.m(), S = pk.n_sets, tile = w.tile;
        const unsigned k = d.k, bf = d.bf;
        const Fr delta = pzh::delta();
        auto to_coeff = [&](uint64_t* t, size_t cnt) {
            for (size_t c0 = 0; c0 < cnt; c0 += tile)
                PZP_CK(pz_ntt_fr_dev(cx.c, t + c0 * n * 4, cnt - c0 < tile ? cnt - c0 : tile, 4 * n, d.omega_inv.v, k, nullptr, d.n_inv.v));
        };
        PZP_CK(pz_quotient_d_rows_dev(cx.c, d_cols, 4 * n, pk.sigma_lagrange, 4 * n, w.Z, 4 * n, (uint32_t)m, CHUNK, d_cols + A * n * 4, 4 * n,
// ... 248 lines not shown
```

paillier_halo2_amd/prover.py:

```python
from __future__ import annotations

from dataclasses import dataclass, field
from typing import Dict, List, Optional, Sequence, Tuple

import numpy as np

from . import consts
from .engine import Bases, Engine

FR = consts.FR_R
M = consts.fr_mont_limbs

LOG_E = 2
CHUNK = 2
ZETA = pow(consts.FR_GENERATOR, (FR - 1) // 3, FR)
DELTA = pow(consts.FR_GENERATOR, 1 << consts.FR_S, FR)


@dataclass
class CircuitStructure:
    k: int
    lookup_bits: int
    max_rows: int
    blinding_factors: int
    selectors: np.ndarray
    n_lk: int
    constants: Sequence[int]
    map_col: np.ndarray
    map_row: np.ndarray
    table: Optional[Sequence[int]] = None
    minimum_rows: Optional[int] = None
    n_adv_used: Optional[int] = None
    n_instance: int = 0
    public_cells: Optional[Sequence[Tuple[int, int]]] = None

    @property
    def n_adv(self) -> int:
        return int(self.selectors.shape[0])

    @property
    def n_public(self) -> int:
        return len(self.public_cells) if self.n_instance and self.public_cells is not None else 0

    @property
    def m(self) -> int:
        return self.n_adv + self.n_lk + 1 + self.n_instance


def _torch():
    import torch

    return torch


# ... 18 lines not shown
    t = torch.from_numpy(raw.view(np.int64)).cuda()
    eng.fr_convert_dev(t.data_ptr(), n, True)
    return t


_R3 = FR >> 192


def _random_fr(gen, *shape):
    torch = _torch()
    K = 8
    c = torch.randint(-(1 << 63), (1 << 63) - 1, (*shape, K, 4), dtype=torch.int64, device="cuda", generator=gen)
    c[..., 3] &= 0x3FFFFFFFFFFFFFFF
    ok = c[..., 3] < _R3
    first = ok.to(torch.int8).argmax(dim=-1, keepdim=True)
    t = torch.gather(c, -2, first.unsqueeze(-1).expand(*shape, 1, 4)).squeeze(-2)
    none = ~ok.any(dim=-1)
    t[..., 3] = torch.where(none, t[..., 3] & 0x0FFFFFFFFFFFFFFF, t[..., 3])
    return t


@dataclass
class Domain:
    k: int
    bf: int
    cosets: int = 3

    def __post_init__(self):
        self.n = 1 << self.k
        self.N = self.n << LOG_E
        self.E = 1 << LOG_E
        self.usable = self.n - (self.bf + 1)
        self.omega = consts.fr_omega(self.k)
        self.omega_inv = pow(self.omega, -1, FR)
        self.n_inv = pow(self.n, -1, FR)
        self.omega_ext = consts.fr_omega(self.k + LOG_E)
        self.omega_ext_inv = pow(self.omega_ext, -1, FR)
        self.N_inv = pow(self.N, -1, FR)
        self.coset_g = ZETA
        self.gens = np.stack([M(self.coset_g * pow(self.omega_ext, r, FR) % FR) for r in range(self.E)])
        self.parts = self._parts(self.cosets)

    def _parts(self, cosets: int):
        w4, g = self.omega_ext, self.coset_g
        mk = lambda log_e, cg, om: dict(log_e=log_e, E=1 << log_e, size=self.n << log_e, coset_g=cg, omega=om, omega_inv=pow(om, -1, FR),
                                        size_inv=pow(self.n << log_e, -1, FR),
                                        gens=np.stack([M(cg * pow(om, r, FR) % FR) for r in range(1 << log_e)]))
        if cosets == 4:
            return [mk(2, g, w4)]
        assert cosets == 3
        return [mk(1, g, w4 * w4 % FR), mk(0, g * w4 % FR, pow(w4, 4, FR))]


class ProvingKey:

    def __init__(self, eng: Engine, st: CircuitStructure, bases_lagrange: Bases, bases_monomial: Bases, cosets: int = 3,
                 ext_resident_cols: Optional[int] = None):
        torch = _torch()
        self.eng, self.st = eng, st
        self.dom = d = Domain(st.k, st.blinding_factors, cosets)
        self.bases_lagrange, self.bases_monomial = bases_lagrange, bases_monomial
        n, N, A, m = d.n, d.N, st.n_adv, st.m
        assert st.max_rows <= d.usable and tuple(st.map_col.shape) == (m, n) and tuple(st.selectors.shape) == (A, n)
        self.n_sets = -(-m // CHUNK)
        one = torch.from_numpy(M(1).view(np.int64)).cuda()
        zero4 = torch.zeros_like(one)
        GB = 256
        F = A + 2
        fixed = _zeros_cap(F, n, 4)
        for a0 in range(0, A, GB):
            sel = st.selectors[a0:a0 + GB]
            sel = sel.cuda() if isinstance(sel, torch.Tensor) else torch.from_numpy(np.ascontiguousarray(sel)).cuda()
            fixed[a0:a0 + sel.shape[0]] = torch.where(sel.bool().unsqueeze(-1), one, zero4)
            del sel
        consts_col = list(st.constants) + [0] * (n - len(st.constants))
        fixed[A] = _ints_to_dev_mont(eng, consts_col)
        table = list(st.table) if st.table is not None else [i if i < (1 << st.lookup_bits) else 0 for i in range(n)]
        fixed[A + 1] = _ints_to_dev_mont(eng, table)
        self.const_lagrange = fixed[A].clone()
        self.table_lagrange = fixed[A + 1].clone()
        sigma = _zeros_cap(m, n, 4)
        as_dev = lambda a: a.to(torch.int32).cuda().contiguous() if isinstance(a, torch.Tensor) else torch.from_numpy(a.view(np.int32)).cuda()
        d_mc, d_mr = as_dev(st.map_col), as_dev(st.map_row)
        eng.permutation_sigma_dev(d_mc.data_ptr(), d_mr.data_ptr(), m, st.k, M(d.omega), M(DELTA), sigma.data_ptr(), 4 * n)
        eng.sync()
        del d_mc, d_mr
        self.sigma_lagrange = _zeros_cap(m, n, 4).copy_(sigma)
        self.fixed_commit = _zeros(F, 12)
        self.sigma_commit = _zeros(m, 12)
        P0 = d.parts[0]
        self.streamed = ext_resident_cols is not None and ext_resident_cols < m
        R = m if not self.streamed else max(0, int(ext_resident_cols))
        self.ext_resident = (min(R, A), R)
        Rf, Rs = self.ext_resident
        if not self.streamed:
            Rf = F
        self.fixed_ext = [_zeros_cap(Rf, pt["size"], 4) for pt in d.parts]
        self.sigma_ext = [_zeros_cap(Rs, pt["size"], 4) for pt in d.parts]
        for t_, cnt_all, com, ext, Rx in ((fixed, F, self.fixed_commit, self.fixed_ext, Rf), (sigma, m, self.sigma_commit, self.sigma_ext, Rs)):
            for c0 in range(0, cnt_all, GB):
                cnt = min(GB, cnt_all - c0)
                r_here = max(0, min(cnt, Rx - c0))
                for b0, bc, keep in ((c0, r_here, True), (c0 + r_here, cnt - r_here, False)):
                    if not bc:
                        continue
                    eng.keygen_columns_dev(bases_lagrange, t_[b0].data_ptr(), bc, 4 * n, st.k, P0["log_e"], M(d.omega), M(d.omega_inv), M(d.n_inv),
                                           P0["gens"], com[b0].data_ptr(), ext[0][b0].data_ptr() if keep else None, 4 * P0["size"])
                    for pi in range(1, len(d.parts) if keep else 0):
                        pt = d.parts[pi]
                        eng.ntt_extend_dev(t_[b0].data_ptr(), bc, 4 * n, ext[pi][b0].data_ptr(), 4 * pt["size"], st.k, pt["log_e"], M(d.omega),
                                           pt["gens"], None)
        self.fixed_coeff = fixed
        self.sigma_coeff = sigma
        self.table_ext = [_zeros(1, pt["size"], 4) for pt in d.parts]
        for pi, pt in enumerate(d.parts):
            eng.ntt_extend_dev(fixed[A + 1].data_ptr(), 1, 4 * n, self.table_ext[pi].data_ptr(), 4 * pt["size"], st.k, pt["log_e"], M(d.omega), pt["gens"], None)
        u = d.usable
        lrows = _zeros(3, n, 4)
        lrows[0, 0] = one
        lrows[1, u] = one
        lrows[2, :u] = one
        eng.ntt_dev(lrows.data_ptr(), 3, 4 * n, M(d.omega_inv), st.k, None, M(d.n_inv))
        self.l_ext = [_zeros(3, pt["size"], 4) for pt in d.parts]
        for pi, pt in enumerate(d.parts):
            eng.ntt_extend_dev(lrows.data_ptr(), 3, 4 * n, self.l_ext[pi].data_ptr(), 4 * pt["size"], st.k, pt["log_e"], M(d.omega), pt["gens"], None)
        eng.sync()

    def vk_commitments(self) -> Dict[str, np.ndarray]:
        e = self.eng
        e.sync()
        jac = lambda t: e.g1_normalize(t.cpu().numpy().view(np.uint64))
        return {"fixed": jac(self.fixed_commit), "sigma": jac(self.sigma_commit)}

    def digest(self) -> bytes:
        if getattr(self, "_digest", None) is None:
            vk, st = self.vk_commitments(), self.st
            self._digest = key_digest(st.k, st.blinding_factors, st.n_adv, st.n_lk, vk["fixed"], vk["sigma"], getattr(st, "n_instance", 0),
                                      getattr(st, "n_public", 0))
        return self._digest


KEY_DIGEST_PERSONAL = b"PZ-Key-Digest-v1"


def key_digest(k: int, bf: int, n_adv: int, n_lk: int, fixed, sigma, n_instance: int = 0, n_public: int = 0) -> bytes:
    import hashlib
    import struct

    f = np.ascontiguousarray(fixed, dtype="<u8").reshape(-1)
    s = np.ascontiguousarray(sigma, dtype="<u8").reshape(-1)
    if f.size != 8 * (n_adv + 2) or s.size != 8 * (n_adv + n_lk + 1 + n_instance):
        raise ValueError("fixed must hold n_adv + 2 points and sigma n_adv + n_lk + 1 (+ 1 with an instance column)")
    if not n_instance and n_public:
        raise ValueError("public values need the instance column")
    h = hashlib.blake2b(struct.pack("<6Q", k, bf, n_adv, n_lk, n_instance, n_public), digest_size=64, person=KEY_DIGEST_PERSONAL)
    h.update(f.tobytes())
    h.update(s.tobytes())
    return h.digest()


def keygen(eng: Engine, st: CircuitStructure, bases_lagrange: Bases, bases_monomial: Bases, cosets: int = 3,
           ext_resident_cols: Optional[int] = None) -> ProvingKey:
    return ProvingKey(eng, st, bases_lagrange, bases_monomial, cosets, ext_resident_cols)


@dataclass
class Challenges:
    theta: int
    beta: int
    gamma: int
    y: int
    x: int
    sh_y: int
    sh_v: int
    sh_u: int
    transcript_seed: Optional[bytes] = None


class Transcript:

    def __init__(self, ch: Challenges):
        self.ch = ch

    def absorb_points(self, eng: Engine, *jac_tensors):
        return [eng.g1_normalize(t.cpu().numpy().view(np.uint64)) for t in jac_tensors]

    def absorb_affine(self, *host_arrays):
        pass

    def absorb_scalars(self, *host_arrays):
        pass

    def squeeze(self, name: str) -> int:
        return getattr(self.ch, name)


class HashTranscript(Transcript):

    PERSONAL = b"Halo2-Transcript"

    def __init__(self, seed: bytes = b"pz", key_digest: Optional[bytes] = None):
        import hashlib

        self.seed = bytes(seed)
        self.key_digest = None if key_digest is None else bytes(key_digest)
        if self.key_digest is not None and len(self.key_digest) != 64:
            raise ValueError("a key digest is 64 bytes")
        self.h = hashlib.blake2b((self.key_digest or b"") + self.seed, digest_size=64, person=self.PERSONAL)
        self.drawn: Dict[str, int] = {}

    def _items(self, tag: int, a: np.ndarray, words: int):
        a = np.ascontiguousarray(a, dtype=np.uint64).reshape(-1, words)
        buf = np.empty((a.shape[0], 1 + 8 * words), dtype=np.uint8)
        buf[:, 0] = tag
        buf[:, 1:] = a.view(np.uint8).reshape(a.shape[0], 8 * words)
        self.h.update(buf.tobytes())
# ... 100 lines not shown

        seed = int.from_bytes(os.urandom(8), "little") >> 1
    gen.manual_seed(seed)
    pr = Proof()
    bl, bm = pk.bases_lagrange, pk.bases_monomial
    t_last = [time.perf_counter()]

    def phase(name):
        if "on_phase" in hooks:
            hooks["on_phase"](name)
        if timings is not None:
            eng.sync()
            now = time.perf_counter()
            timings[name] = timings.get(name, 0.0) + (now - t_last[0]) * 1e3
            t_last[0] = now

    eng2, split_cols = hooks.get("commit_engine"), int(hooks.get("commit_split", 512))

    def commit(bases, t, count, stride_u64):
        out = _zeros(count, 12)
        if eng2 is None or count < 2 * split_cols:
            eng.msm_dev(bases, t.data_ptr(), count, n, stride_u64, out.data_ptr())
            return out
        eng2.wait_for(eng)
        for i, c0 in enumerate(range(0, count, split_cols)):
            (eng if i % 2 == 0 else eng2).msm_dev(bases, t[c0].data_ptr(), min(split_cols, count - c0), n, stride_u64, out[c0].data_ptr())
        eng.wait_for(eng2)
        return out

    def to_coeff(t, cnt):
        for c0 in range(0, cnt, tile):
            eng.ntt_dev(t[c0].data_ptr(), min(tile, cnt - c0), 4 * n, M(d.omega_inv), k, None, M(d.n_inv))

    def extend(src, cnt, dst, pt):
        eng.ntt_extend_dev(src.data_ptr(), cnt, 4 * n, dst.data_ptr(), 4 * pt["size"], k, pt["log_e"], M(d.omega), pt["gens"], None)

    if st.n_instance and not st.n_public:
        raise ValueError("a structure with the instance column names its public cells (at least one)")
    n_pub = st.n_public if st.n_instance else 0
    if (len(instances) if instances is not None else 0) != n_pub:
        raise ValueError("this key's statement has %d public values" % n_pub)
    if n_pub:
        if any(not 0 <= int(v) < FR for v in instances):
            raise ValueError("a public value must be a field element")
        inst_m = np.stack([M(int(v)) for v in instances]).astype(np.uint64)
        tr.absorb_scalars(inst_m.reshape(n_pub, 1, 4))
    cols[:W, u:] = _random_fr(gen, W, n - u)
    cols[W] = pk.const_lagrange
    if st.n_instance:
        cols[W + 1] = 0
        cols[W + 1, :n_pub] = torch.from_numpy(inst_m.view(np.int64)).to(cols.device)
    if "advice" in hooks:
        hooks["advice"](cols)
    c_adv = commit(bl, cols, W, 4 * n)
    if "after_advice_launch" in hooks:
        hooks["after_advice_launch"]()
    (a_adv,) = tr.absorb_points(eng, c_adv)
    tr.squeeze("theta")
    phase("advice_commit")
    Ap, Sp, Zl, Z = ws.Ap, ws.Sp, ws.Zl, ws.Z
    lk_in = cols[A:W]
    eng.lookup_permute_dev(lk_in.data_ptr(), Lk, 4 * n, pk.table_lagrange.data_ptr(), u, st.lookup_bits, Ap.data_ptr(), Sp.data_ptr(), 4 * n)
    if "permuted" in hooks:
        hooks["permuted"](Ap, Sp)
    Ap[:, u:] = _random_fr(gen, Lk, n - u)
    Sp[:, u:] = _random_fr(gen, Lk, n - u)
    c_ap, c_sp = commit(bl, Ap, Lk, 4 * n), commit(bl, Sp, Lk, 4 * n)
    a_ap, a_sp = tr.absorb_points(eng, c_ap, c_sp)
    beta_i, gamma_i = tr.squeeze("beta"), tr.squeeze("gamma")
    beta, gamma = M(beta_i), M(gamma_i)
    phase("lookup_permute_commit")
    eng.permutation_product_sets_dev(cols.data_ptr(), 4 * n, pk.sigma_lagrange.data_ptr(), 4 * n, m, CHUNK, k, u, M(d.omega), beta, gamma,
                                     M(DELTA), Z.data_ptr(), 4 * n)
    Z[:, u + 1:] = _random_fr(gen, S, n - u - 1)
    eng.lookup_product_dev(lk_in.data_ptr(), 4 * n, pk.table_lagrange.data_ptr(), Ap.data_ptr(), 4 * n, Sp.data_ptr(), 4 * n, Lk, n, beta,
                           gamma, M(1), Zl.data_ptr(), 4 * n)
    Zl[:, u + 1:] = _random_fr(gen, Lk, n - u - 1)
    if "products" in hooks:
        hooks["products"](Z, Zl)
    c_z, c_zl = commit(bl, Z, S, 4 * n), commit(bl, Zl, Lk, 4 * n)
    rnd = ws.rnd
    rnd.copy_(_random_fr(gen, 1, n))
    c_rnd = commit(bm, rnd, 1, 4 * n)
    a_z, a_zl, a_rnd = tr.absorb_points(eng, c_z, c_zl, c_rnd)
    y_i = tr.squeeze("y")
    y = M(y_i)
    phase("products_commit")
    if len(d.parts) == 2:
        dvec = ws.dvec
        eng.quotient_d_rows_dev(cols.data_ptr(), 4 * n, pk.sigma_lagrange.data_ptr(), 4 * n, Z.data_ptr(), 4 * n, m, CHUNK, lk_in.data_ptr(), 4 * n,
                                pk.table_lagrange.data_ptr(), Ap.data_ptr(), 4 * n, Sp.data_ptr(), 4 * n, Zl.data_ptr(), 4 * n, Lk, k, u, M(d.omega),
                                beta, gamma, M(DELTA), y, dvec.data_ptr())
    for t, cnt in ((cols, m), (Ap, Lk), (Sp, Lk), (Z, S), (Zl, Lk)):
        to_coeff(t, cnt)
    n_perm_lines = 2 + (S - 1) + S
    lt = ws.lk_ext[0][0].shape[0]
    Rf, Rs = pk.ext_resident
    h = ws.h
    pieces = h.view(d.E, n, 4)

    def key_tile(pi, coeff, resident, R_, which, c0, cnt):
        if not pk.streamed or c0 + cnt <= R_:
            return resident[pi][c0].data_ptr()
        buf = ws.key_ext[pi][which]
        extend(coeff[c0:c0 + cnt], cnt, buf, d.parts[pi])
        return buf.data_ptr()

# ... 175 lines not shown
```

paillier_halo2_amd/prover_native.py:

```python
from __future__ import annotations

import ctypes as C
from typing import Dict, Optional

import numpy as np

from . import consts
from ._lib import VP
from .engine import Bases, Engine
from .prover import CHUNK, Challenges, CircuitStructure, Proof, Transcript

M = consts.fr_mont_limbs


def _host(a):
    return a.cpu().numpy() if hasattr(a, "cpu") else a


def _p(a: np.ndarray):
    return VP(a.ctypes.data)


class NativeKey:

    def __init__(self, eng: Engine, st: CircuitStructure, bases_lagrange: Bases, bases_monomial: Bases, tile: int = 64,
                 ext_resident_cols: Optional[int] = None):
        self.eng, self.st = eng, st
        n = 1 << st.k
        consts_w = np.zeros((len(st.constants), 4), dtype=np.uint64)
        for i, v in enumerate(st.constants):
            consts_w[i] = consts.int_to_limbs(int(v) % consts.FR_R, 4)
        h = VP()
        R = (1 << 64) - 1 if ext_resident_cols is None else int(ext_resident_cols)
        on_dev = hasattr(st.selectors, "is_cuda") and st.selectors.is_cuda
        if on_dev:
            import torch

            sel = st.selectors.to(torch.uint8).contiguous()
            mc, mr = st.map_col.to(torch.int32).contiguous(), st.map_row.to(torch.int32).contiguous()
            assert tuple(sel.shape) == (st.n_adv, n) and tuple(mc.shape) == (st.m, n) == tuple(mr.shape)
            eng._chk(eng.L.pz_pk_create_pub_dev(eng.ctx, bases_lagrange.handle, bases_monomial.handle, st.k, st.lookup_bits, st.blinding_factors,
                                                st.max_rows, st.n_adv, st.n_lk, st.n_instance, st.n_public, VP(sel.data_ptr()), _p(consts_w),
                                                len(st.constants), VP(mc.data_ptr()), VP(mr.data_ptr()), tile, R, C.byref(h)), "pz_pk_create_pub_dev")
        else:
            sel = np.ascontiguousarray(_host(st.selectors), dtype=np.uint8)
            mc = np.ascontiguousarray(_host(st.map_col)).view(np.uint32)
            mr = np.ascontiguousarray(_host(st.map_row)).view(np.uint32)
            assert sel.shape == (st.n_adv, n) and mc.shape == (st.m, n) == mr.shape
            eng._chk(eng.L.pz_pk_create_pub(eng.ctx, bases_lagrange.handle, bases_monomial.handle, st.k, st.lookup_bits, st.blinding_factors,
                                            st.max_rows, st.n_adv, st.n_lk, st.n_instance, st.n_public, _p(sel), _p(consts_w), len(st.constants),
                                            _p(mc), _p(mr), tile, R, C.byref(h)), "pz_pk_create_pub")
        self.handle = h
        out = [C.c_size_t() for _ in range(5)]
        eng._chk(eng.L.pz_pk_info(h, *[C.byref(x) for x in out]), "pz_pk_info")
        self.n_fixed, self.m, self.n_sets, self.blinding_words, self.evals_words = (int(x.value) for x in out)
        assert self.m == st.m and self.n_sets == -(-st.m // CHUNK)

    @classmethod
    def from_device(cls, eng: Engine, ns: "NativeStructure", bases_lagrange: Bases, bases_monomial: Bases, tile: int = 64,
                    ext_resident_cols: Optional[int] = None) -> "NativeKey":
        self = cls.__new__(cls)
        self.eng = eng
        self.st = CircuitStructure(k=ns.k, lookup_bits=ns.lookup_bits, max_rows=ns.max_rows, blinding_factors=ns.blinding_factors,
                                   selectors=np.zeros((ns.n_adv, 0), dtype=np.uint8), n_lk=ns.n_lk, constants=ns.constants(), map_col=None, map_row=None,
                                   minimum_rows=ns.minimum_rows, n_adv_used=ns.n_adv_used, n_instance=ns.n_instance,
                                   public_cells=ns.public_cells() if ns.n_instance else None)
        h = VP()
        R = (1 << 64) - 1 if ext_resident_cols is None else int(ext_resident_cols)
        eng._chk(eng.L.pz_pk_create_pub_dev(eng.ctx, bases_lagrange.handle, bases_monomial.handle, ns.k, ns.lookup_bits, ns.blinding_factors,
                                            ns.max_rows, ns.n_adv, ns.n_lk, ns.n_instance, ns.n_public, VP(ns.d_selectors), VP(ns._constants),
                                            ns.n_constants, VP(ns.d_map_col), VP(ns.d_map_row), tile, R, C.byref(h)), "pz_pk_create_pub_dev")
        self.handle = h
        out = [C.c_size_t() for _ in range(5)]
        eng._chk(eng.L.pz_pk_info(h, *[C.byref(x) for x in out]), "pz_pk_info")
        self.n_fixed, self.m, self.n_sets, self.blinding_words, self.evals_words = (int(x.value) for x in out)
        return self

    def vk_commitments(self) -> Dict[str, np.ndarray]:
        f, s = np.zeros((self.n_fixed, 8), dtype=np.uint64), np.zeros((self.m, 8), dtype=np.uint64)
        self.eng._chk(self.eng.L.pz_pk_commitments(self.handle, _p(f), _p(s)), "pz_pk_commitments")
        return {"fixed": f, "sigma": s}

    def digest(self) -> bytes:
        out = (C.c_uint8 * 64)()
        self.eng._chk(self.eng.L.pz_pk_digest(self.handle, out), "pz_pk_digest")
        return bytes(out)

    def free(self):
        if self.handle:
            self.eng._chk(self.eng.L.pz_pk_free(self.handle), "pz_pk_free")
            self.handle = None


def _canon_words(vals) -> np.ndarray:
    w = np.zeros((len(vals), 4), dtype=np.uint64)
    for i, v in enumerate(vals):
        w[i] = consts.int_to_limbs(int(v), 4)
    return w


def create_proof(key: NativeKey, d_cols: int, tr, seed: int = 0, blinding: Optional[np.ndarray] = None, instances=None) -> Proof:
    eng, st, L = key.eng, key.st, key.eng.L
    if isinstance(tr, Challenges):
        tr = Transcript(tr)
    A, Lk, m, S = st.n_adv, st.n_lk, st.m, key.n_sets
    z = lambda cnt: np.zeros((cnt, 8), dtype=np.uint64)
    h = VP()
    adv = z(A + Lk)
    bl = np.ascontiguousarray(blinding, dtype=np.uint64) if blinding is not None else None
# ... 131 lines not shown
```

rust/pz-sys/src/lib.rs:

```rust
#![allow(non_camel_case_types)]
use core::ffi::{c_char, c_int, c_void};

#[repr(C)] pub struct pz_ctx     { _p: [u8; 0] }
#[repr(C)] pub struct pz_bases   { _p: [u8; 0] }
#[repr(C)] pub struct pz_shplonk { _p: [u8; 0] }
#[repr(C)] pub struct pz_pk      { _p: [u8; 0] }
#[repr(C)] pub struct pz_structure { _p: [u8; 0] }
#[repr(C)] pub struct pz_proof   { _p: [u8; 0] }
#[repr(C)] pub struct pz_vk      { _p: [u8; 0] }
#[repr(C)] pub struct pz_params  { _p: [u8; 0] }

extern "C" {
    pub fn pz_init(n_devices: c_int, device_ids: *const c_int, out: *mut *mut pz_ctx) -> c_int;
    pub fn pz_free(ctx: *mut pz_ctx) -> c_int;
    pub fn pz_strerror(status: c_int) -> *const c_char;
    pub fn pz_last_hip_error(ctx: *const pz_ctx) -> *const c_char;
    pub fn pz_set_stream(ctx: *mut pz_ctx, hip_stream: *mut c_void) -> c_int;
    pub fn pz_sync(ctx: *mut pz_ctx) -> c_int;
    pub fn pz_abi_version() -> c_int;

    pub fn pz_dev_alloc(ctx: *mut pz_ctx, bytes: usize, d_out: *mut *mut c_void) -> c_int;
    pub fn pz_dev_cache_limit(ctx: *mut pz_ctx, max_bytes: usize) -> c_int;
    pub fn pz_dev_arena(ctx: *mut pz_ctx, bytes: usize) -> c_int;
    pub fn pz_dev_arena_info(ctx: *mut pz_ctx, out: *mut u64) -> c_int;
    pub fn pz_dev_mem_info(ctx: *mut pz_ctx, free_bytes: *mut usize, total_bytes: *mut usize) -> c_int;
    pub fn pz_dev_free(ctx: *mut pz_ctx, d: *mut c_void) -> c_int;
    pub fn pz_upload(ctx: *mut pz_ctx, d_dst: *mut c_void, src: *const c_void, bytes: usize) -> c_int;
    pub fn pz_download(ctx: *mut pz_ctx, dst: *mut c_void, d_src: *const c_void, bytes: usize) -> c_int;
    pub fn pz_dev_memset(ctx: *mut pz_ctx, d_dst: *mut c_void, byte_value: c_int, bytes: usize) -> c_int;
    pub fn pz_dev_copy(ctx: *mut pz_ctx, d_dst: *mut c_void, d_src: *const c_void, bytes: usize) -> c_int;
    pub fn pz_dev_copy_2d(ctx: *mut pz_ctx, d_dst: *mut c_void, dst_pitch: usize, d_src: *const c_void, src_pitch: usize, width: usize,
                          rows: usize) -> c_int;
    pub fn pz_ctx_wait(waiter: *mut pz_ctx, producer: *mut pz_ctx) -> c_int;

    pub fn pz_srs_load_g1(ctx: *mut pz_ctx, k: u32, bases_affine: *const u64, lagrange: c_int,
                          out: *mut *mut pz_bases) -> c_int;
    pub fn pz_bases_load_g1(ctx: *mut pz_ctx, bases_affine: *const u64, n_points: usize, on_device: c_int,
                            window_bits: u32, out: *mut *mut pz_bases) -> c_int;
    pub fn pz_bases_free(ctx: *mut pz_ctx, bases: *mut pz_bases) -> c_int;
    pub fn pz_bases_info(bases: *const pz_bases, n_points: *mut usize, window_bits: *mut u32,
                         n_windows: *mut u32) -> c_int;
    pub fn pz_msm_g1(ctx: *mut pz_ctx, bases: *const pz_bases, scalars: *const u64, n: usize,
                     out_jac: *mut u64 ) -> c_int;
    pub fn pz_msm_g1_batch(ctx: *mut pz_ctx, bases: *const pz_bases, scalar_cols: *const *const u64,
                           n_cols: usize, n: usize, out_jac: *mut u64) -> c_int;
    pub fn pz_msm_g1_dev(ctx: *mut pz_ctx, bases: *const pz_bases, d_scalars: *const u64, n_cols: usize,
                         n: usize, col_stride: usize, win_lo: u32, win_hi: u32, d_out_jac: *mut u64) -> c_int;
    pub fn pz_g1_sum(ctx: *mut pz_ctx, jac: *const u64, n: usize, out_jac: *mut u64) -> c_int;
    pub fn pz_g1_sum_dev(ctx: *mut pz_ctx, d_jac: *const u64, n: usize, d_out_jac: *mut u64) -> c_int;
    pub fn pz_msm_g1_multi(ctxs: *const *mut pz_ctx, bases: *const *const pz_bases, d_scalars: *const *const u64, n_per_ctx: *const usize,
                           n_ctx: usize, split_points: c_int, out_jac: *mut u64) -> c_int;
    pub fn pz_g1_normalize(ctx: *mut pz_ctx, jac: *const u64, n: usize, aff: *mut u64) -> c_int;
    pub fn pz_g1_fixed_base_mul(ctx: *mut pz_ctx, scalars: *const u64, n: usize, out_affine: *mut u64) -> c_int;
    pub fn pz_g1_fixed_base_mul_dev(ctx: *mut pz_ctx, d_scalars: *const u64, n: usize, d_out: *mut u64) -> c_int;

    pub fn pz_ntt_fr(ctx: *mut pz_ctx, a: *mut u64, omega: *const u64 , log_n: u32) -> c_int;
    pub fn pz_ntt_fr_batch(ctx: *mut pz_ctx, cols: *const *mut u64, n_cols: usize, omega: *const u64,
                           log_n: u32) -> c_int;
    pub fn pz_ntt_fr_dev(ctx: *mut pz_ctx, d_a: *mut u64, n_cols: usize, col_stride: usize, omega: *const u64,
                         log_n: u32, pre_coset_g: *const u64, post_scale: *const u64) -> c_int;
    pub fn pz_ntt_fr_to_dev(ctx: *mut pz_ctx, d_in: *const u64, in_stride: usize, d_out: *mut u64, out_stride: usize, n_cols: usize,
                            omega: *const u64, log_n: u32, pre_coset_g: *const u64, post_scale: *const u64) -> c_int;
    pub fn pz_ntt_fr_extend_dev(ctx: *mut pz_ctx, d_coeff: *const u64, n_cols: usize, in_stride: usize, d_ext: *mut u64,
                                out_stride: usize, log_n: u32, log_e: u32, omega_n: *const u64, coset_gens: *const u64,
                                scale: *const u64) -> c_int;
    pub fn pz_ntt_fr_coeff_extend_dev(ctx: *mut pz_ctx, d_values: *mut u64, n_cols: usize, col_stride: usize, d_ext: *mut u64,
                                      out_stride: usize, log_n: u32, log_e: u32, omega_n: *const u64, omega_n_inv: *const u64,
                                      n_inv: *const u64, coset_gens: *const u64) -> c_int;
    pub fn pz_fr_convert_dev(ctx: *mut pz_ctx, d_a: *mut u64, n: usize, to_mont: c_int) -> c_int;
    pub fn pz_fr_from_mask_dev(ctx: *mut pz_ctx, d_mask: *const u8, n: usize, d_out: *mut u64) -> c_int;
    pub fn pz_g1_commit_mask_dev(ctx: *mut pz_ctx, bases: *const pz_bases, d_mask: *const u8, n_cols: usize, n: usize,
                                 mask_stride: usize, d_out_jac: *mut u64) -> c_int;

    pub fn pz_mul_mod(ctx: *mut pz_ctx, limbs: u32, a: *const u64, b: *const u64, modulus: *const u64,
                      q: *mut u64, r: *mut u64) -> c_int;
    pub fn pz_paillier_trace(ctx: *mut pz_ctx, limbs_n2: u32, n2: *const u64, base: *const u64, exp: *const u64,
                             exp_limbs: u32, steps_out: *mut u64, n_steps: *mut usize, result: *mut u64) -> c_int;
    pub fn pz_paillier_encrypt(ctx: *mut pz_ctx, limbs_n: u32, batch: usize, n: *const u64, g: *const u64,
                               m: *const u64, r: *const u64, steps_out: *mut u64, steps_cap: usize,
                               n_steps_g: *mut u32, n_steps_r: *mut u32, c_out: *mut u64) -> c_int;
    pub fn pz_paillier_encrypt_dev(ctx: *mut pz_ctx, limbs_n: u32, batch: usize, n: *const u64, g: *const u64,
                                   m: *const u64, r: *const u64, d_steps_out: *mut u64, steps_cap: usize,
                                   n_steps_g: *mut u32, n_steps_r: *mut u32, c_out: *mut u64) -> c_int;
    pub fn pz_paillier_tally(ctx: *mut pz_ctx, limbs_n: u32, count: usize, n: *const u64, cts: *const u64,
                             steps_out: *mut u64, steps_cap: usize, c_out: *mut u64) -> c_int;
    pub fn pz_paillier_tally_dev(ctx: *mut pz_ctx, limbs_n: u32, count: usize, n: *const u64, cts: *const u64,
                                 d_steps_out: *mut u64, steps_cap: usize, c_out: *mut u64) -> c_int;

    pub fn pz_paillier_encrypt_uniform(ctx: *mut pz_ctx, limbs_n: u32, batch: usize, m_bits: u32, n: *const u64, g: *const u64,
                                       m: *const u64, r: *const u64, steps_out: *mut u64, steps_cap: usize,
                                       n_steps_g: *mut u32, n_steps_r: *mut u32, c_out: *mut u64) -> c_int;
    pub fn pz_paillier_encrypt_uniform_dev(ctx: *mut pz_ctx, limbs_n: u32, batch: usize, m_bits: u32, n: *const u64,
                                           g: *const u64, m: *const u64, r: *const u64, d_steps_out: *mut u64, steps_cap: usize,
                                           n_steps_g: *mut u32, n_steps_r: *mut u32, c_out: *mut u64) -> c_int;

    pub fn pz_srs_lagrange_from_monomial_dev(ctx: *mut pz_ctx, k: u32, omega_inv: *const u64, n_inv: *const u64,
                                             d_g: *const u64, d_g_lagrange: *mut u64) -> c_int;
    pub fn pz_permutation_sigma_dev(ctx: *mut pz_ctx, d_map_col: *const u32, d_map_row: *const u32, m: usize, k: u32,
                                    omega: *const u64, delta: *const u64, d_sigma: *mut u64, sigma_stride: usize) -> c_int;
    pub fn pz_permutation_sigma_part_dev(ctx: *mut pz_ctx, d_map_col: *const u32, d_map_row: *const u32, m_total: usize,
                                         col_lo: usize, n_cols: usize, k: u32, omega: *const u64, delta: *const u64,
                                         d_sigma: *mut u64, sigma_stride: usize) -> c_int;
    pub fn pz_keygen_columns_dev(ctx: *mut pz_ctx, bases_lagrange: *const pz_bases, d_cols: *mut u64, n_cols: usize,
                                 col_stride: usize, k: u32, log_e: u32, omega_n: *const u64, omega_n_inv: *const u64,
                                 n_inv: *const u64, coset_gens: *const u64, d_commit_jac: *mut u64, d_ext: *mut u64,
                                 ext_stride: usize) -> c_int;

    pub fn pz_shplonk_begin_dev(ctx: *mut pz_ctx, n: usize, n_sets: u32, set_n_polys: *const u32, d_polys: *const *const u64,
                                set_n_points: *const u32, point_idx: *const u32, n_points_total: u32, points: *const u64,
                                evals: *const u64, y: *const u64, v: *const u64, d_h: *mut u64,
                                state: *mut *mut pz_shplonk) -> c_int;
    pub fn pz_shplonk_finish_dev(ctx: *mut pz_ctx, state: *mut pz_shplonk, u: *const u64, d_h: *const u64, d_h2: *mut u64) -> c_int;
    pub fn pz_shplonk_free(ctx: *mut pz_ctx, state: *mut pz_shplonk) -> c_int;

    pub fn pz_circuit_structure_dev(ctx: *mut pz_ctx, kind: c_int, limbs_n: u32, limb_bits: u32, lookup_bits: u32, k: u32, exp_g: *const u64,
                                    exp_r: *const u64, minimum_rows: usize, blinding_factors: u32, out: *mut *mut pz_structure) -> c_int;
    pub fn pz_circuit_structure_tally_dev(ctx: *mut pz_ctx, limbs_n: u32, limb_bits: u32, lookup_bits: u32, k: u32, count: usize,
                                          minimum_rows: usize, blinding_factors: u32, out: *mut *mut pz_structure) -> c_int;
    pub fn pz_structure_info(st: *const pz_structure, n_adv: *mut usize, n_adv_filled: *mut usize, n_lk: *mut usize, max_rows: *mut usize,
                             n_constants: *mut usize, n_cells: *mut usize, n_lookups: *mut usize, n_steps_g: *mut usize,
                             n_steps_r: *mut usize) -> c_int;
    pub fn pz_structure_arrays(st: *const pz_structure, d_selectors: *mut *const u8, d_map_col: *mut *const u32, d_map_row: *mut *const u32,
                               d_col_starts: *mut *const u64, constants: *mut *const u64, col_starts_host: *mut *const u64) -> c_int;
    pub fn pz_structure_free(st: *mut pz_structure) -> c_int;
    pub fn pz_pk_create(ctx: *mut pz_ctx, bases_lagrange: *const pz_bases, bases_monomial: *const pz_bases, k: u32, lookup_bits: u32,
// ... 213 lines not shown
```

Before: 1.458.

## Precompute copy-constraint group base sums to shrink advice commitment MSMs

Adds a keygen-time pass that uses pointer jumping over the permutation map to find equivalence classes of copy-constrained cells. For each column it precomputes summed Lagrange bases for groups of cells that must hold equal values. A new grouped MSM then replaces each group with one representative point, so the advice commitment touches fewer bases. This trades extra keygen work and device memory for smaller proof-time MSMs, and relies on copy constraints holding in the witness. The path is on by default via an environment flag and is skipped when advice hooks or a second engine are in use.

```diff
diff --git a/include/pz.h b/include/pz.h
--- a/include/pz.h
+++ b/include/pz.h
@@ -70,6 +70,18 @@
 
 int pz_g1_commit_mask_dev(pz_ctx* ctx, const pz_bases* bases, const uint8_t* d_mask, size_t n_cols, size_t n, size_t mask_stride,
                           uint64_t* d_out_jac);
+
+typedef struct pz_copy_groups pz_copy_groups;
+int pz_copy_groups_create_dev(pz_ctx* ctx, const pz_bases* bases_lagrange, const uint32_t* d_map_col, const uint32_t* d_map_row, size_t m,
+                              uint32_t k, size_t n_cols, uint32_t g_min, size_t min_saved, pz_copy_groups** out);
+int pz_copy_groups_free(pz_ctx* ctx, pz_copy_groups* groups);
+int pz_copy_groups_info(const pz_copy_groups* groups, size_t* n_cols, size_t* n_groups, size_t* n_cells, size_t* bytes);
+int pz_copy_groups_column(pz_ctx* ctx, const pz_copy_groups* groups, size_t col, uint8_t* mask_out, uint32_t* reps_out, size_t reps_cap,
+                          size_t* n_groups);
+int pz_copy_groups_plan(const uint32_t* map_col, const uint32_t* map_row, size_t m, uint32_t k, size_t n_cols, uint32_t g_min,
+                        size_t min_saved, uint8_t* mask_out, uint32_t* reps_out, size_t reps_cap, size_t* col_counts);
+int pz_msm_g1_groups_dev(pz_ctx* ctx, const pz_bases* bases, const pz_copy_groups* groups, size_t first_col, const uint64_t* d_scalars,
+                         size_t n_cols, size_t n, size_t col_stride, uint64_t* d_out_jac);
 
 int pz_ntt_fr(pz_ctx* ctx, uint64_t* a , const uint64_t omega[4], uint32_t log_n);
 int pz_ntt_fr_batch(pz_ctx* ctx, uint64_t* const* cols, size_t n_cols, const uint64_t omega[4], uint32_t log_n);
@@ -297,6 +309,9 @@
 
 typedef struct pz_pk pz_pk;
 typedef struct pz_proof pz_proof;
+
+int pz_pk_copy_groups_default(int enabled, uint32_t g_min, size_t min_saved);
+int pz_pk_copy_groups(const pz_pk* pk, size_t* n_groups, size_t* n_cells, size_t* bytes);
 #define PZ_BLINDING_SEEDED_TEST_STREAM (~(size_t)0)
 #define PZ_PK_EXT_ALL (~(size_t)0)
 int pz_pk_create(pz_ctx* ctx, const pz_bases* bases_lagrange, const pz_bases* bases_monomial, uint32_t k, uint32_t lookup_bits,
diff --git a/paillier_halo2_amd/_lib.py b/paillier_halo2_amd/_lib.py
--- a/paillier_halo2_amd/_lib.py
+++ b/paillier_halo2_amd/_lib.py
@@ -41,6 +41,14 @@
     "pz_msm_g1_batch": (C.c_int, [VP, VP, C.POINTER(VP), C.c_size_t, C.c_size_t, VP]),
     "pz_msm_g1_dev": (C.c_int, [VP, VP, VP, C.c_size_t, C.c_size_t, C.c_size_t, C.c_uint32, C.c_uint32, VP]),
     "pz_g1_commit_mask_dev": (C.c_int, [VP, VP, VP, C.c_size_t, C.c_size_t, C.c_size_t, VP]),
+    "pz_copy_groups_create_dev": (C.c_int, [VP, VP, VP, VP, C.c_size_t, C.c_uint32, C.c_size_t, C.c_uint32, C.c_size_t, C.POINTER(VP)]),
+    "pz_copy_groups_free": (C.c_int, [VP, VP]),
+    "pz_copy_groups_info": (C.c_int, [VP, C.POINTER(C.c_size_t), C.POINTER(C.c_size_t), C.POINTER(C.c_size_t), C.POINTER(C.c_size_t)]),
+    "pz_copy_groups_column": (C.c_int, [VP, VP, C.c_size_t, VP, VP, C.c_size_t, C.POINTER(C.c_size_t)]),
+    "pz_copy_groups_plan": (C.c_int, [VP, VP, C.c_size_t, C.c_uint32, C.c_size_t, C.c_uint32, C.c_size_t, VP, VP, C.c_size_t, VP]),
+    "pz_msm_g1_groups_dev": (C.c_int, [VP, VP, VP, C.c_size_t, VP, C.c_size_t, C.c_size_t, C.c_size_t, VP]),
+    "pz_pk_copy_groups_default": (C.c_int, [C.c_int, C.c_uint32, C.c_size_t]),
+    "pz_pk_copy_groups": (C.c_int, [VP, C.POINTER(C.c_size_t), C.POINTER(C.c_size_t), C.POINTER(C.c_size_t)]),
     "pz_g1_sum": (C.c_int, [VP, VP, C.c_size_t, VP]),
     "pz_g1_sum_dev": (C.c_int, [VP, VP, C.c_size_t, VP]),
     "pz_msm_g1_multi": (C.c_int, [VP, VP, VP, VP, C.c_size_t, C.c_int, VP]),
diff --git a/paillier_halo2_amd/csrc/pz_groups.hip b/paillier_halo2_amd/csrc/pz_groups.hip
--- /dev/null
+++ b/paillier_halo2_amd/csrc/pz_groups.hip
@@ -0,0 +1,389 @@
+#include "ec.cuh"
+#include "ec29.cuh"
+#include <stdlib.h>
+
+#include <algorithm>
+
+#include <hipcub/hipcub.hpp>
+
+#include "pz_internal.h"
+
+#define CG_THREADS 256u
+#define CG_BATCH_COLS 256u
+#define CG_NONE 0xffffffffffffffffull
+
+__global__ __launch_bounds__(CG_THREADS) void k_cg_init(const u32* __restrict__ mc, const u32* __restrict__ mr, size_t m, size_t n,
+                                                        u32* __restrict__ nxt, u32* __restrict__ lab, unsigned* __restrict__ bad) {
+    const size_t i = (size_t)blockIdx.x * blockDim.x + threadIdx.x;
+    if (i >= m * n) return;
+    const u32 c = mc[i], r = mr[i];
+    u32 t = (u32)i;
+    if (c >= m || r >= n) *bad = 1u;
+    else t = (u32)((size_t)c * n + r);
+    nxt[i] = t;
+    lab[i] = (u32)i;
+}
+
+__global__ __launch_bounds__(CG_THREADS) void k_cg_jump(const u32* __restrict__ nxt_a, const u32* __restrict__ lab_a, u32* __restrict__ nxt_b,
+                                                        u32* __restrict__ lab_b, size_t total, unsigned* __restrict__ changed) {
+    const size_t i = (size_t)blockIdx.x * blockDim.x + threadIdx.x;
+    if (i >= total) return;
+    const u32 t = nxt_a[i];
+    const u32 l0 = lab_a[i], l1 = lab_a[t];
+    const u32 l = l1 < l0 ? l1 : l0;
+    nxt_b[i] = nxt_a[t];
+    lab_b[i] = l;
+    if (l != l0) *changed = 1u;
+}
+
+__global__ __launch_bounds__(CG_THREADS) void k_cg_keys(const u32* __restrict__ lab, const u32* __restrict__ mc, const u32* __restrict__ mr,
+                                                        size_t c0, size_t cb, unsigned k, unsigned long long* __restrict__ keys) {
+    const size_t j = (size_t)blockIdx.x * blockDim.x + threadIdx.x;
+    if (j >= (cb << k)) return;
+    const size_t cl = j >> k, row = j & (((size_t)1 << k) - 1), cell = ((c0 + cl) << k) + row;
+    const bool self = mc[cell] == (u32)(c0 + cl) && mr[cell] == (u32)row;
+    keys[j] = self ? CG_NONE : ((unsigned long long)cl << (32 + k)) | ((unsigned long long)lab[cell] << k) | row;
+}
+
+__global__ __launch_bounds__(CG_THREADS) void k_cg_heads(const unsigned long long* __restrict__ keys, size_t N, unsigned k, unsigned g_min,
+                                                         u32* __restrict__ flags) {
+    const size_t j = (size_t)blockIdx.x * blockDim.x + threadIdx.x;
+    if (j >= N) return;
+    const unsigned long long key = keys[j], gk = key >> k;
+    bool head = key != CG_NONE && (j == 0 || (keys[j - 1] >> k) != gk);
+    if (head) {
+        const size_t e = j + g_min - 1;
+        head = e < N && keys[e] != CG_NONE && (keys[e] >> k) == gk;
+    }
+    flags[j] = head ? 1u : 0u;
+}
+
+__global__ __launch_bounds__(CG_THREADS) void k_cg_compact(const unsigned long long* __restrict__ keys, const u32* __restrict__ flags,
+                                                           const u32* __restrict__ gidx, size_t N, unsigned k, u32* __restrict__ headpos,
+                                                           u32* __restrict__ colcnt) {
+    const size_t j = (size_t)blockIdx.x * blockDim.x + threadIdx.x;
+    if (j >= N || !flags[j]) return;
+    headpos[gidx[j]] = (u32)j;
+    atomicAdd(&colcnt[keys[j] >> (32 + k)], 1u);
+}
+
+__global__ __launch_bounds__(64) void k_cg_points(const unsigned long long* __restrict__ keys, size_t N, unsigned k, size_t c0,
+                                                  const u32* __restrict__ headpos, const G1Aff64* __restrict__ table, u32* __restrict__ mask_words,
+                                                  u32* __restrict__ reps, G1Aff64* __restrict__ points, u32* __restrict__ sizes,
+                                                  unsigned long long* __restrict__ colcells) {
+    __shared__ G1X29Raw s_pt[64];
+    const size_t g = blockIdx.x;
+    const size_t j0 = headpos[g];
+    const unsigned long long gk = keys[j0] >> k;
+    const size_t cl = (size_t)(gk >> 32), n = (size_t)1 << k;
+    G1X29 acc = x29_inf();
+    u32 cnt = 0;
+    for (size_t j = j0 + threadIdx.x; j < N; j += 64) {
+        const unsigned long long key = keys[j];
+        if ((key >> k) != gk) break;
+        const size_t row = (size_t)(key & (n - 1));
+        const size_t bit = ((c0 + cl) << k) + row;
+        atomicOr(&mask_words[bit >> 5], 1u << (bit & 31));
+        x29_add_affine(acc, a29_load64(table + row));
+        ++cnt;
+    }
+    x29_store_raw(&s_pt[threadIdx.x], acc);
+    __syncthreads();
+    for (unsigned off = 32; off > 0; off >>= 1) {
+        if (threadIdx.x < off) {
+            G1X29 a = x29_load_raw(&s_pt[threadIdx.x]);
+            const G1X29 o = x29_load_raw(&s_pt[threadIdx.x + off]);
+            x29_add(a, o);
+            x29_store_raw(&s_pt[threadIdx.x], a);
+        }
+        __syncthreads();
+    }
+#pragma unroll
+    for (int off = 32; off > 0; off >>= 1) cnt += __shfl_xor(cnt, off, 64);
+    if (threadIdx.x == 0) {
+        a29_store64(points + g, a29_canon(x29_to_affine(x29_load_raw(&s_pt[0]))));
+        reps[g] = (u32)(keys[j0] & (n - 1));
+        sizes[g] = cnt;
+        atomicAdd(&colcells[cl], (unsigned long long)cnt);
+    }
+}
+
+namespace {
+struct cg_batch {
+    size_t c0 = 0, cb = 0, total = 0;
+    u32* d_reps = nullptr;
+    void* d_points = nullptr;
+    std::vector<u32> colcnt;
+    std::vector<unsigned long long> colcells;
+};
+struct cg_scratch {
+    std::vector<void*> v;
+    hipStream_t st = nullptr;
+    hipError_t get(pz_ctx* ctx, void** d, size_t bytes) {
+        hipError_t e = pz_hip_malloc(ctx, d, bytes ? bytes : 4);
+        if (e == hipSuccess) v.push_back(*d);
+        return e;
+    }
+    void drop(void* d) {
+        for (size_t i = 0; i < v.size(); ++i)
+            if (v[i] == d) {
+                (void)pz_hip_free(d);
+                v.erase(v.begin() + (long)i);
+                return;
+            }
+    }
+    ~cg_scratch() {
+        if (!v.empty()) (void)hipStreamSynchronize(st);
+        for (void* d : v) (void)pz_hip_free(d);
+    }
+};
+}
+
+static void cg_release(pz_copy_groups* g) {
+    if (!g) return;
+    if (g->d_mask) (void)pz_hip_free(g->d_mask);
+    if (g->d_reps) (void)pz_hip_free(g->d_reps);
+    if (g->d_points) (void)pz_hip_free(g->d_points);
+    if (g->d_col_off) (void)pz_hip_free(g->d_col_off);
+    delete g;
+}
+
+extern "C" int pz_copy_groups_create_dev(pz_ctx* ctx, const pz_bases* bases_lagrange, const uint32_t* d_map_col, const uint32_t* d_map_row,
+                                         size_t m, uint32_t k, size_t n_cols, uint32_t g_min, size_t min_saved, pz_copy_groups** out) {
+    if (!ctx || !bases_lagrange || !d_map_col || !d_map_row || !out) return PZ_ERR_INVALID;
+    *out = nullptr;
+    if (k < 3 || k > 26 || g_min < 2 || g_min > 1024 || n_cols == 0 || n_cols > m) return PZ_ERR_INVALID;
+    const size_t n = (size_t)1 << k, total = m * n;
+    if (bases_lagrange->n < n) return PZ_ERR_INVALID;
+    if (total >= ((size_t)1 << 32)) return PZ_ERR_UNSUPPORTED;
+    PZ_ENTER(ctx);
+    if (bases_lagrange->device != ctx->device) return PZ_ERR_INVALID;
+    hipStream_t st = ctx->stream;
+    cg_scratch sc;
+    sc.st = st;
+    u32 *nxt[2], *lab[2];
+    unsigned* d_flag;
+    for (int i = 0; i < 2; ++i) {
+        HIPCHK(ctx, sc.get(ctx, (void**)&nxt[i], total * 4));
+        HIPCHK(ctx, sc.get(ctx, (void**)&lab[i], total * 4));
+    }
+    HIPCHK(ctx, sc.get(ctx, (void**)&d_flag, 8));
+    HIPCHK(ctx, hipMemsetAsync(d_flag, 0, 8, st));
+    const unsigned gt = pz_div_up(total, CG_THREADS);
+    hipLaunchKernelGGL(k_cg_init, dim3(gt), dim3(CG_THREADS), 0, st, d_map_col, d_map_row, m, n, nxt[0], lab[0], d_flag);
+    HIPCHK(ctx, hipGetLastError());
+    unsigned h_flag[2] = {0, 0};
+    HIPCHK(ctx, hipMemcpyAsync(h_flag, d_flag, 8, hipMemcpyDeviceToHost, st));
+    HIPCHK(ctx, hipStreamSynchronize(st));
+    if (h_flag[0]) return PZ_ERR_INVALID;
+    int cur = 0;
+    for (unsigned round = 0; round < 32; ++round) {
+        HIPCHK(ctx, hipMemsetAsync(d_flag + 1, 0, 4, st));
+        hipLaunchKernelGGL(k_cg_jump, dim3(gt), dim3(CG_THREADS), 0, st, (const u32*)nxt[cur], (const u32*)lab[cur], nxt[cur ^ 1], lab[cur ^ 1],
+                           total, d_flag + 1);
+        HIPCHK(ctx, hipGetLastError());
+        HIPCHK(ctx, hipMemcpyAsync(h_flag + 1, d_flag + 1, 4, hipMemcpyDeviceToHost, st));
+        HIPCHK(ctx, hipStreamSynchronize(st));
+        cur ^= 1;
+        if (!h_flag[1]) break;
+    }
+    const u32* d_lab = lab[cur];
+    sc.drop(nxt[0]);
+    sc.drop(nxt[1]);
+    sc.drop(lab[cur ^ 1]);
+    pz_copy_groups* G = new pz_copy_groups();
+    G->device = ctx->device;
+    G->n = n;
+    G->n_cols = n_cols;
+    G->g_min = g_min;
+    G->bases_table = bases_lagrange->d_table;
+    struct guard {
+        pz_copy_groups* g;
+        hipStream_t st;
+        ~guard() {
+            if (g) (void)hipStreamSynchronize(st);
+            cg_release(g);
+        }
+    } gd{G, st};
+    const size_t mask_bytes = (n_cols * (n / 8) + 3) / 4 * 4;
+    HIPCHK(ctx, pz_hip_malloc(ctx, (void**)&G->d_mask, mask_bytes));
+    HIPCHK(ctx, hipMemsetAsync(G->d_mask, 0, mask_bytes, st));
+    size_t CB = CG_BATCH_COLS;
+    while (CB > 1 && (CB << k) > ((size_t)1 << 26)) CB >>= 1;
+    if (CB > n_cols) CB = n_cols;
+    const size_t NB = CB << k;
+    unsigned long long *keys_a, *keys_b, *d_colcells;
+    u32 *flags, *gidx, *headpos, *sizes, *d_colcnt;
+    HIPCHK(ctx, sc.get(ctx, (void**)&keys_a, NB * 8));
+    HIPCHK(ctx, sc.get(ctx, (void**)&keys_b, NB * 8));
+    HIPCHK(ctx, sc.get(ctx, (void**)&flags, NB * 4));
+    HIPCHK(ctx, sc.get(ctx, (void**)&gidx, NB * 4));
+    HIPCHK(ctx, sc.get(ctx, (void**)&headpos, (NB / g_min + 1) * 4));
+    HIPCHK(ctx, sc.get(ctx, (void**)&sizes, (NB / g_min + 1) * 4));
+    HIPCHK(ctx, sc.get(ctx, (void**)&d_colcnt, CB * 4));
+    HIPCHK(ctx, sc.get(ctx, (void**)&d_colcells, CB * 8));
+    size_t tmp_sort = 0, tmp_scan = 0;
+    HIPCHK(ctx, hipcub::DeviceRadixSort::SortKeys(nullptr, tmp_sort, keys_a, keys_b, NB, 0, 64, st));
+    HIPCHK(ctx, hipcub::DeviceScan::ExclusiveSum(nullptr, tmp_scan, flags, gidx, NB, st));
+    const size_t tmp_bytes = std::max(tmp_sort, tmp_scan);
+    void* d_tmp;
+    HIPCHK(ctx, sc.get(ctx, &d_tmp, tmp_bytes));
+    std::vector<cg_batch> batches;
+    for (size_t c0 = 0; c0 < n_cols; c0 += CB) {
+        cg_batch b;
+        b.c0 = c0;
+        b.cb = std::min(CB, n_cols - c0);
+        const size_t N = b.cb << k;
+        const unsigned gn = pz_div_up(N, CG_THREADS);
+        hipLaunchKernelGGL(k_cg_keys, dim3(gn), dim3(CG_THREADS), 0, st, d_lab, d_map_col, d_map_row, c0, b.cb, k, keys_a);
+        size_t tb = tmp_bytes;
+        HIPCHK(ctx, hipcub::DeviceRadixSort::SortKeys(d_tmp, tb, keys_a, keys_b, N, 0, 64, st));
+        hipLaunchKernelGGL(k_cg_heads, dim3(gn), dim3(CG_THREADS), 0, st, (const unsigned long long*)keys_b, N, k, g_min, flags);
+        tb = tmp_bytes;
+        HIPCHK(ctx, hipcub::DeviceScan::ExclusiveSum(d_tmp, tb, flags, gidx, N, st));
+        HIPCHK(ctx, hipGetLastError());
+        u32 last[2];
+        HIPCHK(ctx, hipMemcpyAsync(&last[0], flags + (N - 1), 4, hipMemcpyDeviceToHost, st));
+        HIPCHK(ctx, hipMemcpyAsync(&last[1], gidx + (N - 1), 4, hipMemcpyDeviceToHost, st));
+        HIPCHK(ctx, hipStreamSynchronize(st));
+        b.total = (size_t)last[0] + last[1];
+        b.colcnt.assign(b.cb, 0);
+        b.colcells.assign(b.cb, 0);
+        if (b.total) {
+            if (b.total > N / g_min) return PZ_ERR_INTERNAL;
+            HIPCHK(ctx, sc.get(ctx, (void**)&b.d_reps, b.total * 4));
+            HIPCHK(ctx, sc.get(ctx, &b.d_points, b.total * 64));
+            HIPCHK(ctx, hipMemsetAsync(d_colcnt, 0, CB * 4, st));
+            HIPCHK(ctx, hipMemsetAsync(d_colcells, 0, CB * 8, st));
+            hipLaunchKernelGGL(k_cg_compact, dim3(gn), dim3(CG_THREADS), 0, st, (const unsigned long long*)keys_b, (const u32*)flags,
+                               (const u32*)gidx, N, k, headpos, d_colcnt);
+            hipLaunchKernelGGL(k_cg_points, dim3((unsigned)b.total), dim3(64), 0, st, (const unsigned long long*)keys_b, N, k, c0,
+                               (const u32*)headpos, (const G1Aff64*)bases_lagrange->d_table, (u32*)G->d_mask, b.d_reps, (G1Aff64*)b.d_points,
+                               sizes, d_colcells);
+            HIPCHK(ctx, hipGetLastError());
+            HIPCHK(ctx, hipMemcpyAsync(b.colcnt.data(), d_colcnt, b.cb * 4, hipMemcpyDeviceToHost, st));
+            HIPCHK(ctx, hipMemcpyAsync(b.colcells.data(), d_colcells, b.cb * 8, hipMemcpyDeviceToHost, st));
+            HIPCHK(ctx, hipStreamSynchronize(st));
+        }
+        batches.push_back(std::move(b));
+    }
+    G->col_off.assign(n_cols + 1, 0);
+    for (const cg_batch& b : batches)
+        for (size_t j = 0; j < b.cb; ++j) {
+            const size_t cnt = b.colcnt[j], cells = (size_t)b.colcells[j];
+            const bool keep = cnt && cells >= 2 * cnt + min_saved;
+            G->col_off[b.c0 + j + 1] = keep ? (u32)cnt : 0u;
+            if (keep) G->n_cells += cells;
+            else if (cnt) HIPCHK(ctx, hipMemsetAsync(G->d_mask + (b.c0 + j) * (n / 8), 0, n / 8, st));
+        }
+    for (size_t c = 0; c < n_cols; ++c) G->col_off[c + 1] += G->col_off[c];
+    G->n_groups = G->col_off[n_cols];
+    HIPCHK(ctx, pz_hip_malloc(ctx, (void**)&G->d_col_off, (n_cols + 1) * 4));
+    HIPCHK(ctx, hipMemcpyAsync(G->d_col_off, G->col_off.data(), (n_cols + 1) * 4, hipMemcpyHostToDevice, st));
+    HIPCHK(ctx, pz_hip_malloc(ctx, (void**)&G->d_reps, (G->n_groups + 1) * 4));
+    HIPCHK(ctx, pz_hip_malloc(ctx, &G->d_points, (G->n_groups + 1) * 64));
+    for (const cg_batch& b : batches) {
+        size_t src = 0;
+        for (size_t j = 0; j < b.cb; ++j) {
+            const size_t cnt = b.colcnt[j], dst = G->col_off[b.c0 + j];
+            if (cnt && G->col_off[b.c0 + j + 1] != dst) {
+                HIPCHK(ctx, hipMemcpyAsync(G->d_reps + dst, b.d_reps + src, cnt * 4, hipMemcpyDeviceToDevice, st));
+                HIPCHK(ctx, hipMemcpyAsync((char*)G->d_points + dst * 64, (const char*)b.d_points + src * 64, cnt * 64, hipMemcpyDeviceToDevice, st));
+            }
+            src += cnt;
+        }
+    }
+    HIPCHK(ctx, hipStreamSynchronize(st));
+    G->bytes = mask_bytes + (n_cols + 1) * 4 + (G->n_groups + 1) * 68;
+    gd.g = nullptr;
+    *out = G;
+    return PZ_OK;
+}
+
+extern "C" int pz_copy_groups_free(pz_ctx* ctx, pz_copy_groups* g) {
+    if (!g) return PZ_OK;
+    if (ctx) {
+        std::lock_guard<std::recursive_mutex> lk(ctx->mu);
+        (void)hipSetDevice(ctx->device);
+        (void)hipStreamSynchronize(ctx->stream);
+    }
+    cg_release(g);
+    return PZ_OK;
+}
+
+extern "C" int pz_copy_groups_info(const pz_copy_groups* g, size_t* n_cols, size_t* n_groups, size_t* n_cells, size_t* bytes) {
+    if (!g) return PZ_ERR_INVALID;
+    if (n_cols) *n_cols = g->n_cols;
+    if (n_groups) *n_groups = g->n_groups;
+    if (n_cells) *n_cells = g->n_cells;
+    if (bytes) *bytes = g->bytes;
+    return PZ_OK;
+}
+
+extern "C" int pz_copy_groups_column(pz_ctx* ctx, const pz_copy_groups* g, size_t col, uint8_t* mask_out, uint32_t* reps_out, size_t reps_cap,
+                                     size_t* n_groups) {
+    if (!ctx || !g || col >= g->n_cols) return PZ_ERR_INVALID;
+    PZ_ENTER(ctx);
+    const size_t lo = g->col_off[col], cnt = g->col_off[col + 1] - lo;
+    if (n_groups) *n_groups = cnt;
+    if (reps_out && reps_cap < cnt) return PZ_ERR_CAPACITY;
+    if (mask_out) HIPCHK(ctx, hipMemcpyAsync(mask_out, g->d_mask + col * (g->n / 8), g->n / 8, hipMemcpyDeviceToHost, ctx->stream));
+    if (reps_out && cnt) HIPCHK(ctx, hipMemcpyAsync(reps_out, g->d_reps + lo, cnt * 4, hipMemcpyDeviceToHost, ctx->stream));
+    HIPCHK(ctx, hipStreamSynchronize(ctx->stream));
+    return PZ_OK;
+}
+
+extern "C" int pz_copy_groups_plan(const uint32_t* map_col, const uint32_t* map_row, size_t m, uint32_t k, size_t n_cols, uint32_t g_min,
+                                   size_t min_saved, uint8_t* mask_out, uint32_t* reps_out, size_t reps_cap, size_t* col_counts) {
+    if (!map_col || !map_row || !mask_out || !col_counts || k < 3 || k > 26 || g_min < 2 || g_min > 1024 || n_cols == 0 || n_cols > m)
+        return PZ_ERR_INVALID;
+    const size_t n = (size_t)1 << k, total = m * n;
+    if (total >= ((size_t)1 << 32)) return PZ_ERR_UNSUPPORTED;
+    for (size_t i = 0; i < total; ++i)
+        if (map_col[i] >= m || map_row[i] >= n) return PZ_ERR_INVALID;
+    memset(mask_out, 0, n_cols * (n / 8));
+    std::vector<unsigned char> seen(total, 0);
+    std::vector<std::vector<uint32_t>> reps(n_cols);
+    std::vector<size_t> cells(n_cols, 0);
+    std::vector<uint32_t> cyc;
+    for (size_t s = 0; s < total; ++s) {
+        if (seen[s]) continue;
+        cyc.clear();
+        size_t i = s;
+        while (!seen[i]) {
+            seen[i] = 1;
+            if (i / n < n_cols) cyc.push_back((uint32_t)i);
+            i = (size_t)map_col[i] * n + map_row[i];
+        }
+        if (i == s && map_col[s] * n + map_row[s] == s) continue;
+        std::sort(cyc.begin(), cyc.end());
+        for (size_t a = 0; a < cyc.size();) {
+            size_t b = a;
+            while (b < cyc.size() && cyc[b] / n == cyc[a] / n) ++b;
+            if (b - a >= g_min) {
+                const size_t c = cyc[a] / n;
+                reps[c].push_back((uint32_t)(cyc[a] % n));
+                cells[c] += b - a;
+                for (size_t t = a; t < b; ++t) mask_out[c * (n / 8) + (cyc[t] % n) / 8] |= (uint8_t)(1u << (cyc[t] % 8));
+            }
+            a = b;
+        }
+    }
+    size_t pos = 0;
+    for (size_t c = 0; c < n_cols; ++c) {
+        const bool keep = !reps[c].empty() && cells[c] >= 2 * reps[c].size() + min_saved;
+        if (!keep) {
+            memset(mask_out + c * (n / 8), 0, n / 8);
+            col_counts[c] = 0;
+            continue;
+        }
+        std::sort(reps[c].begin(), reps[c].end());
+        col_counts[c] = reps[c].size();
+        if (reps_out) {
+            if (pos + reps[c].size() > reps_cap) return PZ_ERR_CAPACITY;
+            memcpy(reps_out + pos, reps[c].data(), reps[c].size() * 4);
+        }
+        pos += reps[c].size();
+    }
+    return PZ_OK;
+}
diff --git a/paillier_halo2_amd/csrc/pz_internal.h b/paillier_halo2_amd/csrc/pz_internal.h
--- a/paillier_halo2_amd/csrc/pz_internal.h
+++ b/paillier_halo2_amd/csrc/pz_internal.h
@@ -83,6 +83,18 @@
     int device = 0;
 };
 
+struct pz_copy_groups {
+    int device = 0;
+    size_t n = 0, n_cols = 0, n_groups = 0, n_cells = 0, bytes = 0;
+    uint32_t g_min = 0;
+    unsigned char* d_mask = nullptr;
+    uint32_t* d_reps = nullptr;
+    void* d_points = nullptr;
+    uint32_t* d_col_off = nullptr;
+    const void* bases_table = nullptr;
+    std::vector<uint32_t> col_off;
+};
+
 static inline int pz_hip_fail(pz_ctx* ctx, hipError_t e, const char* what) {
     if (ctx) snprintf(ctx->hip_err, sizeof ctx->hip_err, "%s: %s", what, hipGetErrorString(e));
     return e == hipErrorOutOfMemory ? PZ_ERR_OOM : PZ_ERR_HIP;
diff --git a/paillier_halo2_amd/csrc/pz_msm.hip b/paillier_halo2_amd/csrc/pz_msm.hip
--- a/paillier_halo2_amd/csrc/pz_msm.hip
+++ b/paillier_halo2_amd/csrc/pz_msm.hip
@@ -63,6 +63,10 @@
     return lt;
 }
 
+__device__ __forceinline__ bool row_masked(const unsigned char* __restrict__ mask, size_t mask_stride, size_t col, size_t i) {
+    return mask != nullptr && ((mask[col * mask_stride + (i >> 3)] >> (i & 7)) & 1u);
+}
+
 __device__ __forceinline__ int next_digit(const u32 s[8], unsigned w, unsigned c, unsigned& carry) {
     unsigned off = w * c;
     unsigned wi = off >> 5, sh = off & 31;
@@ -126,7 +130,8 @@
 }
 
 __global__ __launch_bounds__(SORT_THREADS) void k_msm_hist(const Fr* __restrict__ scalars, size_t col_stride, MsmP p,
-                                                           u32* __restrict__ slice_hist, unsigned n_slices, size_t n_cols) {
+                                                           u32* __restrict__ slice_hist, unsigned n_slices, size_t n_cols,
+                                                           const unsigned char* __restrict__ mask, size_t mask_stride) {
     __shared__ u32 h[SORT_MAXB];
     size_t col;
     unsigned slice;
@@ -137,6 +142,7 @@
     for (unsigned t = 0; t < p.spt; ++t) {
         const size_t i = base + (size_t)t * SORT_THREADS + threadIdx.x;
         if (i >= p.n) break;
+        if (row_masked(mask, mask_stride, col, i)) continue;
         u32 s[8];
         (void)scalar_prepare(fp_load<FrTag>(scalars + col * col_stride + i), s);
         u32 any = 0;
@@ -316,7 +322,8 @@
 __global__ __launch_bounds__(COARSE_THREADS) void k_msm_scatter_coarse(const Fr* __restrict__ scalars, size_t col_stride, MsmP p,
                                                                        const u32* __restrict__ slice_hist, unsigned n_slices,
                                                                        const u32* __restrict__ offs, u32* __restrict__ staged,
-                                                                       size_t n_cols, ScatterSel sel) {
+                                                                       size_t n_cols, ScatterSel sel,
+                                                                       const unsigned char* __restrict__ mask, size_t mask_stride) {
     if (!scatter_dense(sel)) return;
     __shared__ u32 cb[SORT_COARSE_MAX];
     __shared__ u32 cnt[SORT_COARSE_MAX];
@@ -357,7 +364,8 @@
     const size_t base = (size_t)slice * SORT_THREADS * p.spt;
     const unsigned rounds = SORT_THREADS * p.spt / COARSE_THREADS;
     Fr nxt = fp_zero<FrTag>();
-    if (base + threadIdx.x < p.n) nxt = fp_load<FrTag>(scalars + col * col_stride + base + threadIdx.x);
+    if (base + threadIdx.x < p.n && !row_masked(mask, mask_stride, col, base + threadIdx.x))
+        nxt = fp_load<FrTag>(scalars + col * col_stride + base + threadIdx.x);
     for (unsigned rd = 0; rd < rounds; ++rd) {
         const size_t i = base + (size_t)rd * COARSE_THREADS + threadIdx.x;
         if (base + (size_t)rd * COARSE_THREADS >= p.n) break;
@@ -365,7 +373,7 @@
         u32 ev[16], rb[16];
 #pragma unroll
         for (unsigned w = 0; w < 16; ++w) rb[w] = 0xffffffffu;
-        if (i < p.n) {
+        if (i < p.n && !row_masked(mask, mask_stride, col, i)) {
             u32 s[8];
             const bool neg = scalar_prepare(cur_scalar, s);
             unsigned carry = 0;
@@ -419,7 +427,7 @@
         __syncthreads();
         {
             const size_t in_ = i + COARSE_THREADS;
-            if (rd + 1 < rounds && in_ < p.n) nxt = fp_load<FrTag>(scalars + col * col_stride + in_);
+            if (rd + 1 < rounds && in_ < p.n && !row_masked(mask, mask_stride, col, in_)) nxt = fp_load<FrTag>(scalars + col * col_stride + in_);
         }
         const unsigned total = s_total;
         for (unsigned sl = threadIdx.x; sl < total; sl += COARSE_THREADS) {
@@ -640,7 +648,7 @@
 __global__ __launch_bounds__(SORT_THREADS) void k_msm_scatter(const Fr* __restrict__ scalars, size_t col_stride, MsmP p,
                                                               const u32* __restrict__ slice_hist, unsigned n_slices,
                                                               const u32* __restrict__ offs, u32* __restrict__ entries, size_t n_cols,
-                                                              ScatterSel sel) {
+                                                              ScatterSel sel, const unsigned char* __restrict__ mask, size_t mask_stride) {
     if (scatter_dense(sel)) return;
     __shared__ u32 h[SORT_MAXB];
     size_t col;
@@ -668,6 +676,7 @@
     for (unsigned t = 0; t < p.spt; ++t) {
         const size_t i = base + (size_t)t * SORT_THREADS + threadIdx.x;
         if (i >= p.n) break;
+        if (row_masked(mask, mask_stride, col, i)) continue;
         u32 s[8];
         const bool neg = scalar_prepare(fp_load<FrTag>(scalars + col * col_stride + i), s);
         u32 any = 0;
@@ -1229,7 +1238,8 @@
 }
 
 static int msm_group(pz_ctx* ctx, const pz_bases* bases, const Fr* d_scalars, size_t nc, size_t n, size_t cs,
-                     unsigned win_lo, unsigned win_hi, unsigned chunk, G1Jac* d_out) {
+                     unsigned win_lo, unsigned win_hi, unsigned chunk, G1Jac* d_out, const unsigned char* mask = nullptr,
+                     size_t mask_stride = 0) {
     MsmP p;
     p.n = n;
     p.n_table = bases->n;
@@ -1286,7 +1296,8 @@
     PZCHK(pz_async_err_init(ctx));
     {
         pz_timer tsort(ctx, PZ_T_MSM_SORT);
-        hipLaunchKernelGGL(k_msm_hist, gs, dim3(SORT_THREADS), 0, st, d_scalars, cs, p, (u32*)hist, n_slices, nc);
+        hipLaunchKernelGGL(k_msm_hist, gs, dim3(SORT_THREADS), 0, st, d_scalars, cs, p, (u32*)hist, n_slices, nc, mask,
+                           mask_stride);
         if (split_items) {
             hipLaunchKernelGGL(k_msm_totals_few, dim3(nblk_few, (unsigned)nc), dim3(256), 0, st, (u32*)hist, n_slices, p, (u32*)totals,
                                blk_cnt, blk_itm, blk_bins);
@@ -1305,13 +1316,13 @@
         sel.err = ctx->async_err_d;
         if (two_pass) {
             hipLaunchKernelGGL(k_msm_scatter_coarse, gs, dim3(COARSE_THREADS), 0, st, d_scalars, cs, p, (const u32*)hist, n_slices,
-                               (const u32*)offs, (u32*)partials, nc, sel);
+                               (const u32*)offs, (u32*)partials, nc, sel, mask, mask_stride);
             hipLaunchKernelGGL(k_msm_scatter_fine, dim3(p.B >> SORT_FINE_LOG, (unsigned)nc), dim3(FINE_THREADS), 0, st, p, (const u32*)offs,
                                (const u32*)partials, (u32*)entries, sel);
         }
         if (scatter_mode != 2 || !two_pass)
             hipLaunchKernelGGL(k_msm_scatter, gs, dim3(SORT_THREADS), 0, st, d_scalars, cs, p, (const u32*)hist, n_slices,
-                               (const u32*)offs, (u32*)entries, nc, sel);
+                               (const u32*)offs, (u32*)entries, nc, sel, mask, mask_stride);
     }
     {
         pz_timer tacc(ctx, PZ_T_MSM_ACC);
@@ -1372,8 +1383,8 @@
     return PZ_OK;
 }
 
-extern "C" int pz_msm_g1_dev(pz_ctx* ctx, const pz_bases* bases, const uint64_t* d_scalars, size_t n_cols, size_t n,
-                             size_t col_stride, uint32_t win_lo, uint32_t win_hi, uint64_t* d_out_jac) {
+static int msm_cols_dev(pz_ctx* ctx, const pz_bases* bases, const uint64_t* d_scalars, size_t n_cols, size_t n, size_t col_stride,
+                        uint32_t win_lo, uint32_t win_hi, uint64_t* d_out_jac, const unsigned char* mask, size_t mask_stride) {
     if (!ctx || !bases || (n_cols && (!d_scalars || !d_out_jac))) return PZ_ERR_INVALID;
     if (n > bases->n || win_lo > win_hi || win_hi > bases->nwin) return PZ_ERR_INVALID;
     if (col_stride % 4 || (n_cols > 1 && col_stride < 4 * n)) return PZ_ERR_INVALID;
@@ -1414,7 +1425,8 @@
     if (group > 4096) group = 4096;
     for (size_t c0 = 0; c0 < n_cols;) {
         const size_t nc = n_cols - c0 < group ? n_cols - c0 : group;
-        const int rc = msm_group(ctx, bases, (const Fr*)d_scalars + c0 * cs, nc, n, cs, win_lo, win_hi, chunk, (G1Jac*)d_out_jac + c0);
+        const int rc = msm_group(ctx, bases, (const Fr*)d_scalars + c0 * cs, nc, n, cs, win_lo, win_hi, chunk, (G1Jac*)d_out_jac + c0,
+                                 mask ? mask + c0 * mask_stride : nullptr, mask_stride);
         if (rc == PZ_ERR_OOM && group > 1) {
             ctx->mem_avail = 0;
             (void)hipGetLastError();
@@ -1424,6 +1436,190 @@
         PZCHK(rc);
         c0 += nc;
     }
+    return PZ_OK;
+}
+
+extern "C" int pz_msm_g1_dev(pz_ctx* ctx, const pz_bases* bases, const uint64_t* d_scalars, size_t n_cols, size_t n,
+                             size_t col_stride, uint32_t win_lo, uint32_t win_hi, uint64_t* d_out_jac) {
+    return msm_cols_dev(ctx, bases, d_scalars, n_cols, n, col_stride, win_lo, win_hi, d_out_jac, nullptr, 0);
+}
+
+#define GRP_THREADS 256u
+#define GRP_TILE 512u
+#define GRP_PARTS 4u
+#define GRP_WINDOWS 64u
+
+__global__ __launch_bounds__(GRP_THREADS) void k_grp_prepare(const Fr* __restrict__ scalars, size_t col_stride, size_t n,
+                                                             const u32* __restrict__ col_off, size_t first_col,
+                                                             const u32* __restrict__ reps, uint4* __restrict__ prep,
+                                                             u32* __restrict__ parts) {
+    const size_t col = blockIdx.y;
+    const u32 base = col_off[first_col], lo = col_off[first_col + col], hi = col_off[first_col + col + 1];
+    const u32 g = lo + blockIdx.x * blockDim.x + threadIdx.x;
+    if (g >= hi) return;
+    const u32 rep = reps[g];
+    u32 s[8];
+#pragma unroll
+    for (int i = 0; i < 8; ++i) s[i] = 0;
+    bool neg = false;
+    if (rep < n) neg = scalar_prepare(fp_load<FrTag>(scalars + col * col_stride + rep), s);
+    u32 pm = 0;
+#pragma unroll
+    for (int i = 0; i < 4; ++i)
+        if (s[2 * i] | s[2 * i + 1]) pm |= 1u << i;
+    if (pm) atomicOr(&parts[col], pm);
+    if (neg) s[7] |= 0x80000000u;
+    prep[2 * (size_t)(g - base)] = make_uint4(s[0], s[1], s[2], s[3]);
+    prep[2 * (size_t)(g - base) + 1] = make_uint4(s[4], s[5], s[6], s[7]);
+}
+
+__global__ __launch_bounds__(GRP_THREADS) void k_grp_sum(const u32* __restrict__ col_off, size_t first_col, const G1Aff64* __restrict__ points,
+                                                         const u32* __restrict__ prep, const u32* __restrict__ parts,
+                                                         G1X29Raw* __restrict__ wsum) {
+    __shared__ __align__(16) unsigned char s_buf[GRP_THREADS * sizeof(G1X29Raw)];
+    __shared__ u32 s_cnt[GRP_THREADS], s_start[GRP_THREADS], s_cur[GRP_THREADS];
+    static_assert(GRP_TILE * 16u * 4u <= GRP_THREADS * sizeof(G1X29Raw), "the list shares the reduction's storage");
+    u32* s_ids = reinterpret_cast<u32*>(s_buf);
+    G1X29Raw* s_pt = reinterpret_cast<G1X29Raw*>(s_buf);
+    const size_t col = blockIdx.x;
+    const u32 pmask = parts[col];
+    if (pmask == 0) return;
+    const u32 base = col_off[first_col], lo = col_off[first_col + col] - base, hi = col_off[first_col + col + 1] - base;
+    const unsigned t = threadIdx.x, bk = t & 15u;
+    for (unsigned part = 0; part < GRP_PARTS; ++part) {
+        if (!((pmask >> part) & 1u)) continue;
+        const u32 top_keep = part == 3 ? 0x7fffffffu : 0xffffffffu;
+        G1X29 acc = x29_inf();
+        for (u32 t0 = lo; t0 < hi; t0 += GRP_TILE) {
+            const u32 t1 = hi - t0 < GRP_TILE ? hi : t0 + GRP_TILE;
+            s_cnt[t] = 0;
+            __syncthreads();
+            for (u32 g = t0 + t; g < t1; g += GRP_THREADS) {
+                const u32 w0 = prep[8 * (size_t)g + 2 * part], w1 = prep[8 * (size_t)g + 2 * part + 1] & top_keep;
+#pragma unroll
+                for (unsigned k = 0; k < 16; ++k) {
+                    const u32 nib = ((k < 8 ? w0 : w1) >> (4u * (k & 7u))) & 15u;
+                    if (nib) atomicAdd(&s_cnt[16u * k + nib], 1u);
+                }
+            }
+            __syncthreads();
+            if (t < 64) {
+                const u32 c0 = s_cnt[4 * t], c1 = s_cnt[4 * t + 1], c2 = s_cnt[4 * t + 2], c3 = s_cnt[4 * t + 3];
+                const u32 sum = c0 + c1 + c2 + c3;
+                u32 incl = sum;
+#pragma unroll
+                for (int off = 1; off < 64; off <<= 1) {
+                    const u32 v = __shfl_up(incl, off, 64);
+                    if ((int)t >= off) incl += v;
+                }
+                const u32 excl = incl - sum;
+                s_start[4 * t] = excl;
+                s_start[4 * t + 1] = excl + c0;
+                s_start[4 * t + 2] = excl + c0 + c1;
+                s_start[4 * t + 3] = excl + c0 + c1 + c2;
+            }
+            __syncthreads();
+            s_cur[t] = s_start[t];
+            __syncthreads();
+            for (u32 g = t0 + t; g < t1; g += GRP_THREADS) {
+                const u32 w0 = prep[8 * (size_t)g + 2 * part], w1 = prep[8 * (size_t)g + 2 * part + 1] & top_keep;
+                const u32 id = g | (prep[8 * (size_t)g + 7] & 0x80000000u);
+#pragma unroll
+                for (unsigned k = 0; k < 16; ++k) {
+                    const u32 nib = ((k < 8 ? w0 : w1) >> (4u * (k & 7u))) & 15u;
+                    if (nib) s_ids[atomicAdd(&s_cur[16u * k + nib], 1u)] = id;
+                }
+            }
+            __syncthreads();
+            const u32 e0 = s_start[t], e1 = e0 + s_cnt[t];
+            for (u32 e = e0; e < e1; ++e) {
+                const u32 id = s_ids[e];
+                G1A29 q = a29_load64(points + base + (id & 0x7fffffffu));
+                if ((id & 0x80000000u) && !a29_is_inf(q)) q.y = a29_neg_y(q.y);
+                x29_add_affine(acc, q);
+            }
+            __syncthreads();
+        }
+        x29_store_raw(&s_pt[t], acc);
+        for (unsigned off = 1; off < 16; off <<= 1) {
+            __syncthreads();
+            G1X29 o = x29_inf();
+            if (bk + off < 16) o = x29_load_raw(&s_pt[t + off]);
+            __syncthreads();
+            x29_add(acc, o);
+            x29_store_raw(&s_pt[t], acc);
+        }
+        __syncthreads();
+        if (bk == 0) x29_store_raw(&s_pt[t], x29_inf());
+        for (unsigned off = 8; off > 0; off >>= 1) {
+            __syncthreads();
+            if (bk < off) {
+                G1X29 a = x29_load_raw(&s_pt[t]);
+                const G1X29 o = x29_load_raw(&s_pt[t + off]);
+                x29_add(a, o);
+                x29_store_raw(&s_pt[t], a);
+            }
+        }
+        if (bk == 0) wsum[col * GRP_WINDOWS + 16u * part + (t >> 4)] = s_pt[t];
+        __syncthreads();
+    }
+}
+
+__global__ __launch_bounds__(64) void k_grp_finish(const G1X29Raw* __restrict__ wsum, const u32* __restrict__ parts, size_t n_cols,
+                                                   G1Jac* __restrict__ out) {
+    const size_t col = (size_t)blockIdx.x * blockDim.x + threadIdx.x;
+    if (col >= n_cols) return;
+    const u32 pmask = parts[col];
+    if (pmask == 0) return;
+    G1X29 acc = x29_inf();
+    for (int w = (int)GRP_WINDOWS - 1; w >= 0; --w) {
+        if (!x29_is_inf(acc)) {
+            for (int d = 0; d < 4; ++d) acc = x29_dbl(acc);
+        }
+        if ((pmask >> ((unsigned)w >> 4)) & 1u) {
+            const G1X29 o = x29_load_raw(&wsum[col * GRP_WINDOWS + (unsigned)w]);
+            x29_add(acc, o);
+        }
+    }
+    G1X29 r = x29_load_jac(out + col);
+    x29_add(r, acc);
+    x29_store_jac(out + col, r);
+}
+
+extern "C" int pz_msm_g1_groups_dev(pz_ctx* ctx, const pz_bases* bases, const pz_copy_groups* groups, size_t first_col,
+                                    const uint64_t* d_scalars, size_t n_cols, size_t n, size_t col_stride, uint64_t* d_out_jac) {
+    if (!ctx || !bases || !groups) return PZ_ERR_INVALID;
+    if (n != groups->n || first_col > groups->n_cols || n_cols > groups->n_cols - first_col) return PZ_ERR_INVALID;
+    if (groups->device != ctx->device || groups->bases_table != bases->d_table) return PZ_ERR_INVALID;
+    const size_t ms = groups->n / 8;
+    PZ_ENTER(ctx);
+    PZCHK(msm_cols_dev(ctx, bases, d_scalars, n_cols, n, col_stride, 0, bases->nwin, d_out_jac, groups->d_mask + first_col * ms, ms));
+    if (n_cols == 0) return PZ_OK;
+    const size_t g0 = groups->col_off[first_col], g1 = groups->col_off[first_col + n_cols];
+    if (g1 == g0) return PZ_OK;
+    size_t g_max = 0;
+    for (size_t c = 0; c < n_cols; ++c) {
+        const size_t cnt = groups->col_off[first_col + c + 1] - groups->col_off[first_col + c];
+        if (cnt > g_max) g_max = cnt;
+    }
+    void *prep, *parts, *wsum;
+    PZCHK(pz_ws_get(ctx, WS_HIST, (g1 - g0) * 32, &prep));
+    PZCHK(pz_ws_get(ctx, WS_TOTALS, n_cols * 4, &parts));
+    PZCHK(pz_ws_get(ctx, WS_NODES_A, n_cols * (size_t)GRP_WINDOWS * sizeof(G1X29Raw), &wsum));
+    hipStream_t st = ctx->stream;
+    HIPCHK(ctx, hipMemsetAsync(parts, 0, n_cols * 4, st));
+    const size_t cs = col_stride / 4;
+    for (size_t c0 = 0; c0 < n_cols; c0 += 32768) {
+        const size_t nc = n_cols - c0 < 32768 ? n_cols - c0 : 32768;
+        hipLaunchKernelGGL(k_grp_prepare, dim3(pz_div_up(g_max, GRP_THREADS), (unsigned)nc), dim3(GRP_THREADS), 0, st,
+                           (const Fr*)d_scalars + c0 * cs, cs, n, (const u32*)groups->d_col_off, first_col + c0,
+                           (const u32*)groups->d_reps, (uint4*)prep + 2 * (groups->col_off[first_col + c0] - g0), (u32*)parts + c0);
+    }
+    hipLaunchKernelGGL(k_grp_sum, dim3((unsigned)n_cols), dim3(GRP_THREADS), 0, st, (const u32*)groups->d_col_off, first_col,
+                       (const G1Aff64*)groups->d_points, (const u32*)prep, (const u32*)parts, (G1X29Raw*)wsum);
+    hipLaunchKernelGGL(k_grp_finish, dim3(pz_div_up(n_cols, 64)), dim3(64), 0, st, (const G1X29Raw*)wsum, (const u32*)parts, n_cols,
+                       (G1Jac*)d_out_jac);
+    HIPCHK(ctx, hipGetLastError());
     return PZ_OK;
 }
 
diff --git a/paillier_halo2_amd/csrc/pz_prover.cpp b/paillier_halo2_amd/csrc/pz_prover.cpp
--- a/paillier_halo2_amd/csrc/pz_prover.cpp
+++ b/paillier_halo2_amd/csrc/pz_prover.cpp
@@ -57,6 +57,7 @@
 }
 
 namespace {
+pzp::CopyGroupOptions g_copy_groups;
 int pk_create(pz_ctx* ctx, const pz_bases* bases_lagrange, const pz_bases* bases_monomial, uint32_t k, uint32_t lookup_bits,
               uint32_t blinding_factors, size_t max_rows, size_t n_adv, size_t n_lk, const uint8_t* selectors, const uint64_t* constants,
               size_t n_constants, const uint32_t* map_col, const uint32_t* map_row, size_t tile, size_t ext_resident_cols, bool on_device,
@@ -88,7 +89,7 @@
             st.map_col.assign(map_col, map_col + m * n);
             st.map_row.assign(map_row, map_row + m * n);
         }
-        pk->key = pzp::keygen(pk->mem, std::move(st), bases_lagrange, bases_monomial, ext_resident_cols);
+        pk->key = pzp::keygen(pk->mem, std::move(st), bases_lagrange, bases_monomial, ext_resident_cols, g_copy_groups);
         pk->key->st.d_selectors = nullptr; pk->key->st.d_map_col = pk->key->st.d_map_row = nullptr;
         pk->ws = pzp::make_workspace(pk->mem, *pk->key, tile);
         PZP_CK(pz_sync(ctx));
@@ -132,6 +133,23 @@
                                     const uint32_t* d_map_row, size_t tile, size_t ext_resident_cols, pz_pk** out) {
     return pk_create(ctx, bases_lagrange, bases_monomial, k, lookup_bits, blinding_factors, max_rows, n_adv, n_lk, d_selectors, constants,
                      n_constants, d_map_col, d_map_row, tile, ext_resident_cols, true, n_instance, n_public, out);
+}
+
+extern "C" int pz_pk_copy_groups_default(int enabled, uint32_t g_min, size_t min_saved) {
+    if (enabled < -1 || enabled > 1 || g_min < 2 || g_min > 1024) return PZ_ERR_INVALID;
+    g_copy_groups.enabled = enabled;
+    g_copy_groups.g_min = g_min;
+    g_copy_groups.min_saved = min_saved;
+    return PZ_OK;
+}
+
+extern "C" int pz_pk_copy_groups(const pz_pk* pk, size_t* n_groups, size_t* n_cells, size_t* bytes) {
+    if (!pk || !pk->key) return PZ_ERR_INVALID;
+    if (n_groups) *n_groups = 0;
+    if (n_cells) *n_cells = 0;
+    if (bytes) *bytes = 0;
+    if (!pk->key->groups) return PZ_OK;
+    return pz_copy_groups_info(pk->key->groups, nullptr, n_groups, n_cells, bytes);
 }
 
 extern "C" int pz_pk_info(const pz_pk* pk, size_t* n_fixed, size_t* n_perm_cols, size_t* n_sets, size_t* blinding_words, size_t* evals_words_out) {
diff --git a/paillier_halo2_amd/engine.py b/paillier_halo2_amd/engine.py
--- a/paillier_halo2_amd/engine.py
+++ b/paillier_halo2_amd/engine.py
@@ -39,6 +39,55 @@
             self.handle = None
 
 
+class CopyGroups:
+
+    def __init__(self, engine: "Engine", handle: VP):
+        self.engine = engine
+        self.handle = handle
+        v = [C.c_size_t() for _ in range(4)]
+        engine._chk(_lib.lib().pz_copy_groups_info(handle, *[C.byref(x) for x in v]), "pz_copy_groups_info")
+        self.n_cols, self.n_groups, self.n_cells, self.bytes = (x.value for x in v)
+
+    def column(self, col: int, n: int) -> Tuple[np.ndarray, np.ndarray]:
+        cnt = C.c_size_t()
+        L = _lib.lib()
+        self.engine._chk(L.pz_copy_groups_column(self.engine.ctx, self.handle, col, None, None, 0, C.byref(cnt)), "pz_copy_groups_column")
+        mask = np.zeros(n // 8, dtype=np.uint8)
+        reps = np.zeros(max(1, cnt.value), dtype=np.uint32)
+        self.engine._chk(L.pz_copy_groups_column(self.engine.ctx, self.handle, col, _ptr(mask), _ptr(reps), reps.shape[0], C.byref(cnt)),
+                         "pz_copy_groups_column")
+        return mask, np.sort(reps[:cnt.value])
+
+    def free(self):
+        if self.handle is not None:
+            _lib.lib().pz_copy_groups_free(self.engine.ctx, self.handle)
+            self.handle = None
+
+    def __del__(self):
+        try:
+            self.free()
+        except Exception:
+            pass
+
+
+def copy_groups_plan(map_col, map_row, k: int, n_cols: int, g_min: int, min_saved: int = 0):
+    mc = np.ascontiguousarray(map_col, dtype=np.uint32)
+    mr = np.ascontiguousarray(map_row, dtype=np.uint32)
+    m, n = mc.shape
+    assert mr.shape == (m, n) and n == 1 << k
+    mask = np.zeros((n_cols, n // 8), dtype=np.uint8)
+    reps = np.zeros(max(1, n_cols * n // max(2, g_min)), dtype=np.uint32)
+    counts = (C.c_size_t * n_cols)()
+    rc = _lib.lib().pz_copy_groups_plan(_ptr(mc), _ptr(mr), m, k, n_cols, g_min, min_saved, _ptr(mask), _ptr(reps), reps.shape[0], counts)
+    if rc != 0:
+        raise PzError(rc, "pz_copy_groups_plan", "")
+    out, pos = [], 0
+    for c in range(n_cols):
+        out.append(reps[pos:pos + counts[c]].copy())
+        pos += counts[c]
+    return mask, out
+
+
 class VkHandle:
 
     def __init__(self, engine: "Engine", handle: VP):
@@ -240,6 +289,18 @@
             win_hi = bases.n_windows
         self._chk(self.L.pz_msm_g1_dev(self.ctx, bases.handle, VP(d_scalars), n_cols, n, col_stride_u64, win_lo,
                                        win_hi, VP(d_out)), "pz_msm_g1_dev")
+
+    def copy_groups_dev(self, bases: Bases, d_map_col: int, d_map_row: int, m: int, k: int, n_cols: int, g_min: int = 4,
+                        min_saved: int = 0) -> CopyGroups:
+        h = VP()
+        self._chk(self.L.pz_copy_groups_create_dev(self.ctx, bases.handle, VP(d_map_col), VP(d_map_row), m, k, n_cols, g_min, min_saved,
+                                                   C.byref(h)), "pz_copy_groups_create_dev")
+        return CopyGroups(self, h)
+
+    def msm_groups_dev(self, bases: Bases, groups: CopyGroups, first_col: int, d_scalars: int, n_cols: int, n: int, col_stride_u64: int,
+                       d_out: int):
+        self._chk(self.L.pz_msm_g1_groups_dev(self.ctx, bases.handle, groups.handle, first_col, VP(d_scalars), n_cols, n, col_stride_u64,
+                                              VP(d_out)), "pz_msm_g1_groups_dev")
 
     @staticmethod
     def msm_multi(engines: Sequence["Engine"], bases: Sequence[Bases], d_scalars: Sequence[int], n_per_ctx: Sequence[int],
diff --git a/paillier_halo2_amd/host/create_proof.hpp b/paillier_halo2_amd/host/create_proof.hpp
--- a/paillier_halo2_amd/host/create_proof.hpp
+++ b/paillier_halo2_amd/host/create_proof.hpp
@@ -124,7 +124,23 @@
     size_t res_fixed = 0, res_sigma = 0;
     bool streamed = false;
     std::vector<uint64_t> fixed_commit, sigma_commit;
+    pz_copy_groups* groups = nullptr;
     explicit ProvingKey(Structure&& s) : st(std::move(s)), dom(st.k, st.blinding_factors) {}
+    ProvingKey(const ProvingKey&) = delete;
+    ProvingKey& operator=(const ProvingKey&) = delete;
+    ~ProvingKey() {
+        if (groups) pz_copy_groups_free(nullptr, groups);
+    }
+};
+
+inline bool copy_groups_enabled() {
+    const char* e = getenv("PZ_COPY_GROUPS");
+    return !(e && e[0] == '0' && e[1] == 0);
+}
+struct CopyGroupOptions {
+    int enabled = -1;
+    uint32_t g_min = 4;
+    size_t min_saved = 4096;
 };
 
 inline void key_digest(const ProvingKey& pk, uint8_t out[pzh::KEY_DIGEST_BYTES]) {
@@ -153,7 +169,8 @@
     }
 };
 
-inline ProvingKey* keygen(Ctx& cx, Structure&& st_in, const pz_bases* bl, const pz_bases* bm, size_t ext_resident_cols = EXT_ALL) {
+inline ProvingKey* keygen(Ctx& cx, Structure&& st_in, const pz_bases* bl, const pz_bases* bm, size_t ext_resident_cols = EXT_ALL,
+                          const CopyGroupOptions& cg = CopyGroupOptions()) {
     std::unique_ptr<ProvingKey> pk(new ProvingKey(std::move(st_in)));
     const Structure& st = pk->st;
     Domain& d = pk->dom;
@@ -201,6 +218,8 @@
         const Fr delta = pzh::delta();
         PZP_CK(pz_permutation_sigma_dev(cx.c, dmc, dmr, m, st.k, d.omega.v, delta.v, sigma, 4 * n));
         PZP_CK(pz_sync(cx.c));
+        if (cg.enabled < 0 ? copy_groups_enabled() : cg.enabled != 0)
+            PZP_CK(pz_copy_groups_create_dev(cx.c, bl, dmc, dmr, m, st.k, A + st.n_lk, cg.g_min, cg.min_saved, &pk->groups));
     }
     {
         Structure& s_ = pk->st;
@@ -416,7 +435,8 @@
             PZP_CK(pz_dev_memset(cx.c, d_cols + (W + 1) * n * 4, 0, n * 32));
             PZP_CK(pz_upload(cx.c, d_cols + (W + 1) * n * 4, instances.data(), instances.size() * 8));
         }
-        commit(pk.bl, d_cols, W, w.out12);
+        if (pk.groups && copy_groups_enabled()) PZP_CK(pz_msm_g1_groups_dev(cx.c, pk.bl, pk.groups, 0, d_cols, W, n, 4 * n, w.out12));
+        else commit(pk.bl, d_cols, W, w.out12);
         if (after_launch) after_launch();
         affine(w.out12, W, out_affine);
         done(0);
diff --git a/paillier_halo2_amd/prover.py b/paillier_halo2_amd/prover.py
--- a/paillier_halo2_amd/prover.py
+++ b/paillier_halo2_amd/prover.py
@@ -1,5 +1,6 @@
 from __future__ import annotations
 
+import os
 from dataclasses import dataclass, field
 from typing import Dict, List, Optional, Sequence, Tuple
 
@@ -124,10 +125,19 @@
         return [mk(1, g, w4 * w4 % FR), mk(0, g * w4 % FR, pow(w4, 4, FR))]
 
 
+COPY_GROUP_MIN = 4
+COPY_GROUP_MIN_SAVED = 4096
+
+
+def copy_groups_enabled() -> bool:
+    return os.environ.get("PZ_COPY_GROUPS", "1") != "0"
+
+
 class ProvingKey:
 
     def __init__(self, eng: Engine, st: CircuitStructure, bases_lagrange: Bases, bases_monomial: Bases, cosets: int = 3,
-                 ext_resident_cols: Optional[int] = None):
+                 ext_resident_cols: Optional[int] = None, copy_groups: Optional[bool] = None, copy_group_min: int = COPY_GROUP_MIN,
+                 copy_group_min_saved: int = COPY_GROUP_MIN_SAVED):
         torch = _torch()
         self.eng, self.st = eng, st
         self.dom = d = Domain(st.k, st.blinding_factors, cosets)
@@ -156,6 +166,10 @@
         d_mc, d_mr = as_dev(st.map_col), as_dev(st.map_row)
         eng.permutation_sigma_dev(d_mc.data_ptr(), d_mr.data_ptr(), m, st.k, M(d.omega), M(DELTA), sigma.data_ptr(), 4 * n)
         eng.sync()
+        self.copy_groups = None
+        if copy_groups_enabled() if copy_groups is None else copy_groups:
+            self.copy_groups = eng.copy_groups_dev(bases_lagrange, d_mc.data_ptr(), d_mr.data_ptr(), m, st.k, A + st.n_lk, copy_group_min,
+                                                   copy_group_min_saved)
         del d_mc, d_mr
         self.sigma_lagrange = _zeros_cap(m, n, 4).copy_(sigma)
         self.fixed_commit = _zeros(F, 12)
@@ -232,8 +246,8 @@
 
 
 def keygen(eng: Engine, st: CircuitStructure, bases_lagrange: Bases, bases_monomial: Bases, cosets: int = 3,
-           ext_resident_cols: Optional[int] = None) -> ProvingKey:
-    return ProvingKey(eng, st, bases_lagrange, bases_monomial, cosets, ext_resident_cols)
+           ext_resident_cols: Optional[int] = None, copy_groups: Optional[bool] = None) -> ProvingKey:
+    return ProvingKey(eng, st, bases_lagrange, bases_monomial, cosets, ext_resident_cols, copy_groups)
 
 
 @dataclass
@@ -440,7 +454,12 @@
         cols[W + 1, :n_pub] = torch.from_numpy(inst_m.view(np.int64)).to(cols.device)
     if "advice" in hooks:
         hooks["advice"](cols)
-    c_adv = commit(bl, cols, W, 4 * n)
+    grp = getattr(pk, "copy_groups", None)
+    if grp is not None and "advice" not in hooks and eng2 is None and copy_groups_enabled():
+        c_adv = _zeros(W, 12)
+        eng.msm_groups_dev(bl, grp, 0, cols.data_ptr(), W, n, 4 * n, c_adv.data_ptr())
+    else:
+        c_adv = commit(bl, cols, W, 4 * n)
     if "after_advice_launch" in hooks:
         hooks["after_advice_launch"]()
     (a_adv,) = tr.absorb_points(eng, c_adv)
diff --git a/paillier_halo2_amd/prover_native.py b/paillier_halo2_amd/prover_native.py
--- a/paillier_halo2_amd/prover_native.py
+++ b/paillier_halo2_amd/prover_native.py
@@ -24,7 +24,7 @@
 class NativeKey:
 
     def __init__(self, eng: Engine, st: CircuitStructure, bases_lagrange: Bases, bases_monomial: Bases, tile: int = 64,
-                 ext_resident_cols: Optional[int] = None):
+                 ext_resident_cols: Optional[int] = None, copy_groups: Optional[bool] = None, copy_group_min_saved: int = 4096):
         self.eng, self.st = eng, st
         n = 1 << st.k
         consts_w = np.zeros((len(st.constants), 4), dtype=np.uint64)
@@ -33,6 +33,25 @@
         h = VP()
         R = (1 << 64) - 1 if ext_resident_cols is None else int(ext_resident_cols)
         on_dev = hasattr(st.selectors, "is_cuda") and st.selectors.is_cuda
+        try:
+            eng._chk(eng.L.pz_pk_copy_groups_default(-1 if copy_groups is None else int(bool(copy_groups)), 4, int(copy_group_min_saved)),
+                     "pz_pk_copy_groups_default")
+            self._create(eng, st, bases_lagrange, bases_monomial, tile, R, on_dev, consts_w, h, n)
+        finally:
+            eng.L.pz_pk_copy_groups_default(-1, 4, 4096)
+        self.handle = h
+        out = [C.c_size_t() for _ in range(5)]
+        eng._chk(eng.L.pz_pk_info(h, *[C.byref(x) for x in out]), "pz_pk_info")
+        self.n_fixed, self.m, self.n_sets, self.blinding_words, self.evals_words = (int(x.value) for x in out)
+        assert self.m == st.m and self.n_sets == -(-st.m // CHUNK)
+
+    def copy_groups(self):
+        v = [C.c_size_t() for _ in range(3)]
+        self.eng._chk(self.eng.L.pz_pk_copy_groups(self.handle, *[C.byref(x) for x in v]), "pz_pk_copy_groups")
+        return tuple(int(x.value) for x in v)
+
+    @staticmethod
+    def _create(eng, st, bases_lagrange, bases_monomial, tile, R, on_dev, consts_w, h, n):
         if on_dev:
             import torch
 
@@ -50,11 +69,6 @@
             eng._chk(eng.L.pz_pk_create_pub(eng.ctx, bases_lagrange.handle, bases_monomial.handle, st.k, st.lookup_bits, st.blinding_factors,
                                             st.max_rows, st.n_adv, st.n_lk, st.n_instance, st.n_public, _p(sel), _p(consts_w), len(st.constants),
                                             _p(mc), _p(mr), tile, R, C.byref(h)), "pz_pk_create_pub")
-        self.handle = h
-        out = [C.c_size_t() for _ in range(5)]
-        eng._chk(eng.L.pz_pk_info(h, *[C.byref(x) for x in out]), "pz_pk_info")
-        self.n_fixed, self.m, self.n_sets, self.blinding_words, self.evals_words = (int(x.value) for x in out)
-        assert self.m == st.m and self.n_sets == -(-st.m // CHUNK)
 
     @classmethod
     def from_device(cls, eng: Engine, ns: "NativeStructure", bases_lagrange: Bases, bases_monomial: Bases, tile: int = 64,
diff --git a/rust/pz-sys/src/lib.rs b/rust/pz-sys/src/lib.rs
--- a/rust/pz-sys/src/lib.rs
+++ b/rust/pz-sys/src/lib.rs
@@ -3,6 +3,7 @@
 
 #[repr(C)] pub struct pz_ctx     { _p: [u8; 0] }
 #[repr(C)] pub struct pz_bases   { _p: [u8; 0] }
+#[repr(C)] pub struct pz_copy_groups { _p: [u8; 0] }
 #[repr(C)] pub struct pz_shplonk { _p: [u8; 0] }
 #[repr(C)] pub struct pz_pk      { _p: [u8; 0] }
 #[repr(C)] pub struct pz_structure { _p: [u8; 0] }
@@ -71,6 +72,19 @@
     pub fn pz_fr_from_mask_dev(ctx: *mut pz_ctx, d_mask: *const u8, n: usize, d_out: *mut u64) -> c_int;
     pub fn pz_g1_commit_mask_dev(ctx: *mut pz_ctx, bases: *const pz_bases, d_mask: *const u8, n_cols: usize, n: usize,
                                  mask_stride: usize, d_out_jac: *mut u64) -> c_int;
+    pub fn pz_copy_groups_create_dev(ctx: *mut pz_ctx, bases_lagrange: *const pz_bases, d_map_col: *const u32, d_map_row: *const u32,
+                                     m: usize, k: u32, n_cols: usize, g_min: u32, min_saved: usize, out: *mut *mut pz_copy_groups) -> c_int;
+    pub fn pz_copy_groups_free(ctx: *mut pz_ctx, groups: *mut pz_copy_groups) -> c_int;
+    pub fn pz_copy_groups_info(groups: *const pz_copy_groups, n_cols: *mut usize, n_groups: *mut usize, n_cells: *mut usize,
+                               bytes: *mut usize) -> c_int;
+    pub fn pz_copy_groups_column(ctx: *mut pz_ctx, groups: *const pz_copy_groups, col: usize, mask_out: *mut u8, reps_out: *mut u32,
+                                 reps_cap: usize, n_groups: *mut usize) -> c_int;
+    pub fn pz_copy_groups_plan(map_col: *const u32, map_row: *const u32, m: usize, k: u32, n_cols: usize, g_min: u32, min_saved: usize,
+                               mask_out: *mut u8, reps_out: *mut u32, reps_cap: usize, col_counts: *mut usize) -> c_int;
+    pub fn pz_msm_g1_groups_dev(ctx: *mut pz_ctx, bases: *const pz_bases, groups: *const pz_copy_groups, first_col: usize,
+                                d_scalars: *const u64, n_cols: usize, n: usize, col_stride: usize, d_out_jac: *mut u64) -> c_int;
+    pub fn pz_pk_copy_groups_default(enabled: c_int, g_min: u32, min_saved: usize) -> c_int;
+    pub fn pz_pk_copy_groups(pk: *const pz_pk, n_groups: *mut usize, n_cells: *mut usize, bytes: *mut usize) -> c_int;
 
     pub fn pz_mul_mod(ctx: *mut pz_ctx, limbs: u32, a: *const u64, b: *const u64, modulus: *const u64,
                       q: *mut u64, r: *mut u64) -> c_int;
```

Measured after the change: 1.509, median of 6. +3.5%, better.
